# jiahuei/sparse-image-captioning

Hardware: AMD Instinct MI355X
Metric: captions/sec (higher is better)
Workload: dtype bf16; 1 GPU; configs[1]: ORT dense, 256 images x 5 captions, teacher-forcing XE fwd+bwd+clip+Adam; images_per_gpu=256, regions=36, captions_per_image=5, parallelism=single

## Files before the change

include/ortk.h:

```cpp
#ifndef ORTK_H
#define ORTK_H

#include <stddef.h>
#include <stdint.h>

#ifdef __cplusplus
extern "C" {
#endif

#define ORTK_VERSION 4
#define ORTK_EINVAL (-1)
#define ORTK_ENOSPC (-2)
#define ORTK_ENOSYS (-3)
#define ORTK_EEXCHANGE (-4)

typedef void* ortk_stream;

int ortk_version(void);
int ortk_device_ok(void);

struct ortk_sparse_plan;
typedef struct ortk_config {
    int32_t d_model, d_ff, n_layers, n_heads;
    int32_t vocab, feat, seq_len;
    int32_t pad_id, bos_id, eos_id, unk_id;
    int32_t box_trig;
    int32_t precision;
    float   drop_src, drop;
    int32_t share_enc[16], share_dec[16];
    int32_t share_att_enc, share_att_dec;
    int32_t no_box;
    const struct ortk_sparse_plan* sparse_fwd;
    const struct ortk_sparse_plan* sparse_bwd;
} ortk_config;

int64_t ortk_arena_numel(const ortk_config* cfg);
int64_t ortk_arena_numel_with_buffers(const ortk_config* cfg);
int32_t ortk_arena_entries(const ortk_config* cfg);
int ortk_arena_entry(const ortk_config* cfg, int32_t index, char* name_buf, int64_t* offset,
                     int64_t* numel, int32_t* ndim, int64_t* shape, int32_t* kind);

uint32_t ortk_dropout_site_seed(uint64_t seed, int32_t stack, int32_t layer, int32_t k);

typedef struct ortk_batch {
    const float*   att_feats;
    const float*   boxes;
    const float*   att_masks;
    const int64_t* seqs;
    int64_t        seq_stride;
    const float*   tok_weight;
    int32_t B, S, R, T;
    const int32_t* cap_off;
    const int32_t* row_pos;
    int32_t        Mc;
    int32_t        no_pad_keys;
} ortk_batch;

int ortk_valid_position_tables(const int64_t* counts, int32_t R, int32_t T, int32_t* cap_off, int32_t* row_pos, ortk_stream stream);
size_t ortk_train_workspace_bytes(const ortk_config* cfg, int32_t B, int32_t S, int32_t R, int32_t T);
int ortk_valid_positions_ok(const ortk_config* cfg, int32_t B, int32_t S, int32_t R, int32_t T);

int ortk_forward(const ortk_config* cfg, const float* params, const ortk_batch* batch, void* ws, size_t ws_bytes,
                 float* logp_out, int64_t ldv, int32_t train, uint64_t seed, ortk_stream stream);
int ortk_forward_phase(const ortk_config* cfg, const float* params, const ortk_batch* batch, void* ws, size_t ws_bytes,
                       float* logp_out, int64_t ldv, int32_t train, uint64_t seed, int32_t phase, ortk_stream stream);
void* ortk_train_workspace_memory(const ortk_config* cfg, int32_t B, int32_t S, int32_t R, int32_t T, void* ws, int32_t* dtype);

int ortk_loss(const ortk_config* cfg, const ortk_batch* batch, void* ws, size_t ws_bytes,
              const float* norm_dev, float* loss_dev, ortk_stream stream);

int ortk_loss_external(const ortk_config* cfg, const ortk_batch* batch, void* ws, size_t ws_bytes,
                       const float* logp, const float* dlogp, int64_t ldv, ortk_stream stream);

int ortk_backward(const ortk_config* cfg, const float* params, float* grads, const ortk_batch* batch,
                  void* ws, size_t ws_bytes, int32_t train, uint64_t seed, ortk_stream stream);
int ortk_backward_phase(const ortk_config* cfg, const float* params, float* grads, const ortk_batch* batch,
                        void* ws, size_t ws_bytes, int32_t train, uint64_t seed, int32_t phase, ortk_stream stream);
int64_t ortk_arena_decoder_offset(const ortk_config* cfg);

#define ORTK_SP_ELL32 0
#define ORTK_SP_ELL16 1
#define ORTK_SP_GU16  2
typedef struct ortk_sparse_block {
    int64_t src_offset;
    int64_t ld;
    int64_t stream_offset;
    int64_t capacity;
    int32_t N, K;
    int32_t chunk0;
    int32_t row0;
} ortk_sparse_block;

typedef struct ortk_sparse_plan {
    const ortk_sparse_block* blocks_host; const ortk_sparse_block* blocks_dev;
    int32_t nblocks, format;
    void* stream;
    int32_t* chunk_ptr;
    int32_t* chunk_len;
    int32_t* perm;
    int32_t* count_scratch;
    int32_t* overflow;
    int64_t total_rows;
} ortk_sparse_plan;

int ortk_sparse_build(const ortk_sparse_plan* plan, const void* dense, int32_t dtype, ortk_stream stream);

typedef struct ortk_spmm_args {
    const void* X; void* Y;
    int64_t ldx, ldy; int64_t M;
    int32_t x_dtype, y_dtype;
    const float* bias; const float* rowscale; const float* resid; int64_t ldr;
    const void* gate; int64_t ldg; int32_t gate_dtype; float gate_scale;
    int32_t relu; float drop_p; uint32_t drop_seed;
    const int32_t* drop_rows;
} ortk_spmm_args;
int ortk_spmm(const ortk_sparse_plan* plan, int32_t block, const ortk_spmm_args* a, ortk_stream stream);

typedef struct ortk_chain_unit { int64_t offset, ld; } ortk_chain_unit;
typedef struct ortk_chain_args {
    const void* w16; const ortk_chain_unit* units_dev; int32_t n_units;
    void* packed; size_t packed_bytes;
    int64_t M;
    const float* x_in;
    const void* a_in; const float* bias_r; float* x_mid; uint32_t seed_r;
    const float *g1, *b1; void* y1; float* st1;
    int32_t n1; const float* bias_s1; void* out1; int64_t ld1;
    int32_t NC; const float *bias_h, *bias_o; void* h; float* x_out; uint32_t seed_h, seed_o;
    const float *g2, *b2; void* y2; float* st2;
    int32_t n2; const float* bias_s2; void* out2; int64_t ld2;
    float drop_p, eps;
    int32_t* progress;
    const int32_t* drop_rows;
} ortk_chain_args;
size_t ortk_chain_packed_bytes(int32_t n_units);
int ortk_row_chain(const ortk_chain_args* a, ortk_stream stream);

typedef struct ortk_bchain_args {
    const void* w16t; const ortk_chain_unit* units_dev; int32_t n_units;
    void* packed; size_t packed_bytes;
    int64_t M;
    int32_t nin; const void* ain; int64_t ld_ain; const void* dz0;
    const float *xa, *sta, *ga, *dresa; float *dxa, *daa, *dba; void* dza; uint32_t seed_a; int32_t mask_a;
    int32_t NC; const void* hgate; void* gh; float gate_scale;
    const float *xb, *stb, *gb, *dresb; float *dxb, *dab, *dbb; void* dzb; uint32_t seed_b; int32_t mask_b;
    int32_t n2; void* out2;
    float drop_p, eps;
    const int32_t* drop_rows;
} ortk_bchain_args;
int ortk_row_bchain(const ortk_bchain_args* a, ortk_stream stream);
// ... 97 lines not shown
    int64_t rows;
    int32_t flags;
    void* ws; size_t ws_bytes;
} ortk_wgrad_group_args;
int ortk_wgrad_group(const ortk_wgrad_group_args* a, ortk_stream stream);
size_t ortk_wgrad_group_workspace_bytes(const ortk_wgrad_group_args* a);
int ortk_prof_enable(int32_t on);
int ortk_prof_collect(int32_t key, int64_t* launches, double* total_ms, double* total_flops);
int ortk_prof_collect_bytes(int32_t key, double* total_bytes);
int ortk_prof_collect_units(int32_t key, double* total_workgroups);

int ortk_layernorm_fwd(const float* x, const float* a, const float* b, void* y, int32_t y_dtype, float* stats,
                       int64_t rows, int32_t d, float eps, ortk_stream stream);
int ortk_layernorm_bwd(const float* dy, const float* x, const float* a, const float* stats, const float* dres,
                       float* dx, float* da, float* db, int64_t rows, int32_t d, float eps, ortk_stream stream);
int ortk_layernorm_bwd_drop(const float* dy, const float* x, const float* a, const float* stats, const float* dres,
                            float* dx, float* da, float* db, int64_t rows, int32_t d, float eps, void* dz, int32_t dz_dtype,
                            float drop_p, uint32_t drop_seed, ortk_stream stream);
int ortk_layernorm_bwd_drop_rows(const float* dy, const float* x, const float* a, const float* stats, const float* dres,
                                 float* dx, float* da, float* db, int64_t rows, int32_t d, float eps, void* dz, int32_t dz_dtype,
                                 float drop_p, uint32_t drop_seed, const int32_t* drop_rows, ortk_stream stream);
int ortk_layernorm_bwd_dt(const void* dy, int32_t dy_dtype, const float* x, const float* a, const float* stats, const float* dres,
                          float* dx, float* da, float* db, int64_t rows, int32_t d, float eps, void* dz, int32_t dz_dtype,
                          float drop_p, uint32_t drop_seed, const int32_t* drop_rows, ortk_stream stream);

int ortk_box_logbias_fwd(const float* boxes, const float* const* wg, const float* const* bg, const float* dim_mat,
                         float* out, int32_t L, int32_t B, int32_t S, int32_t H, ortk_stream stream);
int ortk_box_logbias_bwd(const float* boxes, const float* const* wg, const float* const* bg, const float* dim_mat,
                         const float* dscore, float* const* dwg, float* const* dbg,
                         int32_t L, int32_t B, int32_t S, int32_t H, ortk_stream stream);
int ortk_box_embedding(const float* boxes, const float* dim_mat, float* out, int32_t B, int32_t S, ortk_stream stream);

typedef struct ortk_attn_args {
    const float* q; const float* k; const float* v; void* o;
    int64_t ldq, ldk, ldv, ldo;
    const float* kmask; const float* bias; const int32_t* kv_index;
    int64_t kv_group_stride;
    float* p;
    int32_t nkv, H, Lq, Lk, dk, causal_period;
    float drop_p; uint32_t drop_seed;
    const float* d_o; void* dq; void* d_k; void* dv; float* dscore;
    int64_t lddo, lddq, lddk, lddv;
    int32_t o_dtype, dqkv_dtype;
    int32_t kv_dtype;
    const float* k_new; const float* v_new; int64_t ld_new;
    int32_t bwd_part;
    int32_t precision;
    int32_t qkv_dtype;
    const int32_t* q_off; int32_t q_off_stride; int32_t kv_ragged;
    int32_t drop_tf_T, drop_tf_t, drop_tf_lk;
    const int32_t* drop_rows;
} ortk_attn_args;
int ortk_attention_fwd(const ortk_attn_args* a, ortk_stream stream);
int ortk_attention_bwd(const ortk_attn_args* a, ortk_stream stream);

int ortk_embed_fwd(const int64_t* seq, int64_t seq_stride, const float* lut, const float* pe, float* out, float* keymask,
                   int64_t R, int32_t T, int32_t t0, int32_t d, int32_t pad_id, float drop_p, uint32_t seed, ortk_stream stream);
int ortk_embed_bwd(const int64_t* seq, int64_t seq_stride, const float* dout, float* dlut,
                   int64_t R, int32_t T, int32_t d, float drop_p, uint32_t seed, ortk_stream stream);

int ortk_log_softmax(float* x, int64_t rows, int32_t V, int64_t ld, float scale, ortk_stream stream);
int64_t ortk_xent_scratch_floats(int64_t rows);
int ortk_xent_fwd_bwd(const float* logits, const int64_t* targets, int64_t target_stride, int32_t T, const float* weight,
                      const float* norm_dev, float* loss_dev, float* row_loss, int64_t rows, int32_t V, int64_t ld,
                      void* dlogits, int32_t dl_dtype, int64_t ld_dl, ortk_stream stream);
int ortk_log_softmax_bwd(const float* logp, const float* dlogp, int64_t ld_in, void* dlogits, int32_t dl_dtype,
                         int64_t ld_out, int64_t rows, int32_t V, ortk_stream stream);

int ortk_colsum(const void* x, int32_t x_dtype, int64_t ld, float* out, int64_t M, int32_t N, ortk_stream stream);
int ortk_gate_apply(const float* x, const float* gate, void* y, int32_t y_dtype, int64_t n, float scale, ortk_stream stream);
int ortk_dropout_apply(const float* x, void* y, int32_t y_dtype, int64_t n, float p, uint32_t seed, ortk_stream stream);
int ortk_dropout_apply_rows(const float* x, void* y, int32_t y_dtype, int64_t rows, int32_t d, float p, uint32_t seed,
                            const int32_t* drop_rows, ortk_stream stream);
int ortk_cast_bf16(const float* x, void* y, int64_t n, ortk_stream stream);
int ortk_fill(float* x, int64_t n, float value, ortk_stream stream);
int ortk_axpy_cols(const void* x, void* y, int32_t dtype, int64_t ld, int64_t rows, int32_t cols, ortk_stream stream);
int64_t ortk_sum_scratch_floats(int64_t n);
int ortk_sum(const float* x, int64_t n, float* scratch, float* out_dev, ortk_stream stream);

int ortk_adam_clip(float* p, const float* g, float* m, float* v, int64_t n, float lr, float beta1, float beta2,
                   float eps, float clip, float bc1, float bc2, ortk_stream stream);
int ortk_adam_clip_zero(float* p, float* g, float* m, float* v, int64_t n, float lr, float beta1, float beta2,
                        float eps, float clip, float bc1, float bc2, ortk_stream stream);

int ortk_mask_apply(const float* w, const float* m, float* w_eff, int64_t n, int32_t mode, uint32_t seed, ortk_stream stream);
int ortk_mask_bwd(const float* dw_eff, const float* w, const float* m, float* dw, float* dm, int64_t n, int32_t mode,
                  uint32_t seed, const float* extra_coef_dev, ortk_stream stream);
typedef struct ortk_masked_adam_args {
    float *w, *g, *mw, *vw;
    float *ml, *mm, *mv;
    const float* draws;
    const float* active;
    const float* extra_coef;
    int64_t n, index0; int32_t mode; uint32_t seed;
    float lr_w, eps_w, lr_m, eps_m, beta1, beta2, clip, bc1, bc2;
} ortk_masked_adam_args;
int ortk_masked_adam_step(const ortk_masked_adam_args* a, ortk_stream stream);
int ortk_mask_apply_draws(const float* w, const float* m, const float* draws, float* w_eff, int64_t n, ortk_stream stream);
int ortk_mask_bwd_draws(const float* dw_eff, const float* w, const float* m, const float* draws, float* dw, float* dm, int64_t n,
                        const float* extra_coef_dev, ortk_stream stream);
int ortk_linear_block(const ortk_config* cfg, int32_t i, int64_t* offset, int32_t* N, int32_t* K);
int ortk_mask_count(const float* m, int64_t n, int32_t mode, float* count_dev, ortk_stream stream);

#ifdef __cplusplus
}
#endif
#endif
```

sparse-image-captioning_amd/_lib.py:

```python
import ctypes as C
import os

import torch

_HERE = os.path.dirname(os.path.abspath(__file__))
LIB_PATH = os.path.join(_HERE, "libortk.so")


class OrtkUnavailable(RuntimeError):
    pass


class OrtkError(RuntimeError):
    pass


class Config(C.Structure):
    _fields_ = [("d_model", C.c_int32), ("d_ff", C.c_int32), ("n_layers", C.c_int32), ("n_heads", C.c_int32),
                ("vocab", C.c_int32), ("feat", C.c_int32), ("seq_len", C.c_int32),
                ("pad_id", C.c_int32), ("bos_id", C.c_int32), ("eos_id", C.c_int32), ("unk_id", C.c_int32),
                ("box_trig", C.c_int32), ("precision", C.c_int32), ("drop_src", C.c_float), ("drop", C.c_float),
                ("share_enc", C.c_int32 * 16), ("share_dec", C.c_int32 * 16),
                ("share_att_enc", C.c_int32), ("share_att_dec", C.c_int32), ("no_box", C.c_int32),
                ("sparse_fwd", C.c_void_p), ("sparse_bwd", C.c_void_p)]


class Batch(C.Structure):
    _fields_ = [("att_feats", C.c_void_p), ("boxes", C.c_void_p), ("att_masks", C.c_void_p), ("seqs", C.c_void_p),
                ("seq_stride", C.c_int64), ("tok_weight", C.c_void_p),
                ("B", C.c_int32), ("S", C.c_int32), ("R", C.c_int32), ("T", C.c_int32),
                ("cap_off", C.c_void_p), ("row_pos", C.c_void_p), ("Mc", C.c_int32), ("no_pad_keys", C.c_int32)]


SP_ELL32, SP_ELL16, SP_GU16 = 0, 1, 2


class EllBlock(C.Structure):
    _fields_ = [("src_offset", C.c_int64), ("ld", C.c_int64), ("stream_offset", C.c_int64), ("capacity", C.c_int64),
                ("N", C.c_int32), ("K", C.c_int32), ("chunk0", C.c_int32), ("row0", C.c_int32)]


class EllPlanStruct(C.Structure):
    _fields_ = [("blocks_host", C.POINTER(EllBlock)), ("blocks_dev", C.c_void_p), ("nblocks", C.c_int32), ("format", C.c_int32),
                ("stream", C.c_void_p), ("chunk_ptr", C.c_void_p), ("chunk_len", C.c_void_p), ("perm", C.c_void_p),
                ("count_scratch", C.c_void_p), ("overflow", C.c_void_p), ("total_rows", C.c_int64)]


class SpmmArgs(C.Structure):
    _fields_ = [("X", C.c_void_p), ("Y", C.c_void_p), ("ldx", C.c_int64), ("ldy", C.c_int64), ("M", C.c_int64),
                ("x_dtype", C.c_int32), ("y_dtype", C.c_int32),
                ("bias", C.c_void_p), ("rowscale", C.c_void_p), ("resid", C.c_void_p), ("ldr", C.c_int64),
                ("gate", C.c_void_p), ("ldg", C.c_int64), ("gate_dtype", C.c_int32), ("gate_scale", C.c_float),
                ("relu", C.c_int32), ("drop_p", C.c_float), ("drop_seed", C.c_uint32), ("drop_rows", C.c_void_p)]


class ChainUnit(C.Structure):
    _fields_ = [("offset", C.c_int64), ("ld", C.c_int64)]


class ChainArgs(C.Structure):
    _fields_ = [("w16", C.c_void_p), ("units_dev", C.c_void_p), ("n_units", C.c_int32), ("packed", C.c_void_p), ("packed_bytes", C.c_size_t),
                ("M", C.c_int64), ("x_in", C.c_void_p),
                ("a_in", C.c_void_p), ("bias_r", C.c_void_p), ("x_mid", C.c_void_p), ("seed_r", C.c_uint32),
                ("g1", C.c_void_p), ("b1", C.c_void_p), ("y1", C.c_void_p), ("st1", C.c_void_p),
                ("n1", C.c_int32), ("bias_s1", C.c_void_p), ("out1", C.c_void_p), ("ld1", C.c_int64),
                ("NC", C.c_int32), ("bias_h", C.c_void_p), ("bias_o", C.c_void_p), ("h", C.c_void_p), ("x_out", C.c_void_p),
                ("seed_h", C.c_uint32), ("seed_o", C.c_uint32),
                ("g2", C.c_void_p), ("b2", C.c_void_p), ("y2", C.c_void_p), ("st2", C.c_void_p),
                ("n2", C.c_int32), ("bias_s2", C.c_void_p), ("out2", C.c_void_p), ("ld2", C.c_int64),
                ("drop_p", C.c_float), ("eps", C.c_float), ("progress", C.c_void_p), ("drop_rows", C.c_void_p)]


class BChainArgs(C.Structure):
    _fields_ = [("w16t", C.c_void_p), ("units_dev", C.c_void_p), ("n_units", C.c_int32), ("packed", C.c_void_p), ("packed_bytes", C.c_size_t),
                ("M", C.c_int64),
                ("nin", C.c_int32), ("ain", C.c_void_p), ("ld_ain", C.c_int64), ("dz0", C.c_void_p),
                ("xa", C.c_void_p), ("sta", C.c_void_p), ("ga", C.c_void_p), ("dresa", C.c_void_p), ("dxa", C.c_void_p), ("daa", C.c_void_p),
                ("dba", C.c_void_p), ("dza", C.c_void_p), ("seed_a", C.c_uint32), ("mask_a", C.c_int32),
                ("NC", C.c_int32), ("hgate", C.c_void_p), ("gh", C.c_void_p), ("gate_scale", C.c_float),
                ("xb", C.c_void_p), ("stb", C.c_void_p), ("gb", C.c_void_p), ("dresb", C.c_void_p), ("dxb", C.c_void_p), ("dab", C.c_void_p),
                ("dbb", C.c_void_p), ("dzb", C.c_void_p), ("seed_b", C.c_uint32), ("mask_b", C.c_int32),
                ("n2", C.c_int32), ("out2", C.c_void_p), ("drop_p", C.c_float), ("eps", C.c_float), ("drop_rows", C.c_void_p)]


class MaskedAdamArgs(C.Structure):
    _fields_ = [("w", C.c_void_p), ("g", C.c_void_p), ("mw", C.c_void_p), ("vw", C.c_void_p),
                ("ml", C.c_void_p), ("mm", C.c_void_p), ("mv", C.c_void_p),
                ("draws", C.c_void_p), ("active", C.c_void_p), ("extra_coef", C.c_void_p),
                ("n", C.c_int64), ("index0", C.c_int64), ("mode", C.c_int32), ("seed", C.c_uint32),
                ("lr_w", C.c_float), ("eps_w", C.c_float), ("lr_m", C.c_float), ("eps_m", C.c_float),
                ("beta1", C.c_float), ("beta2", C.c_float), ("clip", C.c_float), ("bc1", C.c_float), ("bc2", C.c_float)]


class Tuning(C.Structure):
    _fields_ = [("gemm_t64", C.c_int32), ("attn_impl", C.c_int32), ("attn16_min_lq", C.c_int32),
                ("side_stream", C.c_int32), ("row_chain", C.c_int32), ("chain_wide", C.c_int32), ("spmm_alias", C.c_int32), ("f32_split", C.c_int32), ("wgrad_wgs", C.c_int32),
                ("wgrad_group", C.c_int32), ("wgrad_group_splitk", C.c_int32), ("wgrad_group_wgs", C.c_int32), ("wgrad_group_tail", C.c_int32), ("feats_bf16", C.c_int32), ("ln_fuse", C.c_int32), ("samp_epilogue", C.c_int32), ("gemm_epilogue", C.c_int32)]


DEC_UNFUSED, DEC_STACK, DEC_SPARSE_STREAM, DEC_STACK_RB20, DEC_STACK_SPLIT, DEC_SPLIT_SMALL, DEC_SPARSE_GATHER = 1, 2, 4, 8, 16, 32, 64


class DecodeOpts(C.Structure):
    _fields_ = [("beam_size", C.c_int32), ("num_random_sample", C.c_int32), ("temperature", C.c_float),
                ("decoding_constraint", C.c_int32), ("length_penalty", C.c_int32), ("length_alpha", C.c_double),
                ("seed", C.c_uint64), ("sparse", C.POINTER(EllPlanStruct)), ("exec_flags", C.c_int32), ("with_greedy", C.c_int32), ("sample_row_offset", C.c_int64),
                ("train", C.c_int32), ("drop_seed", C.c_uint64), ("memory", C.c_void_p)]


class GemmArgs(C.Structure):
    _fields_ = [("A", C.c_void_p), ("B", C.c_void_p), ("C", C.c_void_p),
                ("lda", C.c_int64), ("ldb", C.c_int64), ("ldc", C.c_int64),
                ("M", C.c_int32), ("N", C.c_int32), ("K", C.c_int32), ("transA", C.c_int32), ("transB", C.c_int32),
                ("bias", C.c_void_p), ("rowscale", C.c_void_p), ("resid", C.c_void_p), ("ldr", C.c_int64),
                ("gate", C.c_void_p), ("ldg", C.c_int64), ("gate_scale", C.c_float),
                ("relu", C.c_int32), ("drop_p", C.c_float), ("drop_seed", C.c_uint32),
                ("accumulate", C.c_int32), ("splitk", C.c_int32), ("precision", C.c_int32),
                ("a_dtype", C.c_int32), ("b_dtype", C.c_int32), ("c_dtype", C.c_int32), ("gate_dtype", C.c_int32),
                ("colsum", C.c_void_p), ("drop_row_stride", C.c_int32), ("drop_row_off", C.c_int32),
                ("ln_mode", C.c_int32), ("ln_y_dtype", C.c_int32),
                ("ln_a", C.c_void_p), ("ln_b", C.c_void_p), ("ln_y", C.c_void_p), ("ln_stats", C.c_void_p), ("ln_eps", C.c_float),
                ("ln_x", C.c_void_p), ("ln_dres", C.c_void_p), ("ln_da", C.c_void_p), ("ln_db", C.c_void_p),
                ("tile_stats", C.c_void_p), ("stat_ncols", C.c_int32), ("drop_rows", C.c_void_p),
                ("tile_samp", C.c_void_p), ("samp_seq", C.c_void_p), ("samp_seed", C.c_uint64), ("samp_row_offset", C.c_int64),
                ("samp_L", C.c_int32), ("samp_t", C.c_int32), ("samp_greedy_stride", C.c_int32), ("samp_sample", C.c_int32),
                ("samp_fast", C.c_int32), ("samp_no_store", C.c_int32), ("samp_inv_temperature", C.c_float)]


class WgradItem(C.Structure):
    _fields_ = [("dY", C.c_void_p), ("lddy", C.c_int64), ("X", C.c_void_p), ("ldx", C.c_int64),
                ("dW", C.c_void_p), ("lddw", C.c_int64), ("db", C.c_void_p), ("Nout", C.c_int32), ("Kin", C.c_int32)]


WGRAD_MAX = 8


class WgradGroupArgs(C.Structure):
    _fields_ = [("item", WgradItem * WGRAD_MAX), ("n", C.c_int32), ("splitk", C.c_int32), ("rows", C.c_int64), ("flags", C.c_int32),
                ("ws", C.c_void_p), ("ws_bytes", C.c_size_t)]


class AttnArgs(C.Structure):
    _fields_ = [("q", C.c_void_p), ("k", C.c_void_p), ("v", C.c_void_p), ("o", C.c_void_p),
                ("ldq", C.c_int64), ("ldk", C.c_int64), ("ldv", C.c_int64), ("ldo", C.c_int64),
                ("kmask", C.c_void_p), ("bias", C.c_void_p), ("kv_index", C.c_void_p), ("kv_group_stride", C.c_int64),
                ("p", C.c_void_p),
                ("nkv", C.c_int32), ("H", C.c_int32), ("Lq", C.c_int32), ("Lk", C.c_int32), ("dk", C.c_int32),
                ("causal_period", C.c_int32), ("drop_p", C.c_float), ("drop_seed", C.c_uint32),
                ("d_o", C.c_void_p), ("dq", C.c_void_p), ("d_k", C.c_void_p), ("dv", C.c_void_p), ("dscore", C.c_void_p),
                ("lddo", C.c_int64), ("lddq", C.c_int64), ("lddk", C.c_int64), ("lddv", C.c_int64),
                ("o_dtype", C.c_int32), ("dqkv_dtype", C.c_int32), ("kv_dtype", C.c_int32),
                ("k_new", C.c_void_p), ("v_new", C.c_void_p), ("ld_new", C.c_int64), ("bwd_part", C.c_int32),
                ("precision", C.c_int32), ("qkv_dtype", C.c_int32),
                ("q_off", C.c_void_p), ("q_off_stride", C.c_int32), ("kv_ragged", C.c_int32),
                ("drop_tf_T", C.c_int32), ("drop_tf_t", C.c_int32), ("drop_tf_lk", C.c_int32), ("drop_rows", C.c_void_p)]


_P, _I32, _I64, _F, _U32, _U64, _SZ = C.c_void_p, C.c_int32, C.c_int64, C.c_float, C.c_uint32, C.c_uint64, C.c_size_t
_CFG = C.POINTER(Config)

SIGNATURES = {
    "ortk_version": (_I32, []),
    "ortk_device_ok": (_I32, []),
    "ortk_arena_numel": (_I64, [_CFG]),
    "ortk_arena_numel_with_buffers": (_I64, [_CFG]),
    "ortk_arena_entries": (_I32, [_CFG]),
    "ortk_arena_entry": (_I32, [_CFG, _I32, C.c_char_p, C.POINTER(_I64), C.POINTER(_I64), C.POINTER(_I32),
                               C.POINTER(_I64), C.POINTER(_I32)]),
    "ortk_train_workspace_bytes": (_SZ, [_CFG, _I32, _I32, _I32, _I32]),
    "ortk_valid_positions_ok": (_I32, [_CFG, _I32, _I32, _I32, _I32]),
    "ortk_forward": (_I32, [_CFG, _P, C.POINTER(Batch), _P, _SZ, _P, _I64, _I32, _U64, _P]),
    "ortk_forward_phase": (_I32, [_CFG, _P, C.POINTER(Batch), _P, _SZ, _P, _I64, _I32, _U64, _I32, _P]),
    "ortk_train_workspace_memory": (_P, [_CFG, _I32, _I32, _I32, _I32, _P, C.POINTER(C.c_int32)]),
    "ortk_loss": (_I32, [_CFG, C.POINTER(Batch), _P, _SZ, _P, _P, _P]),
    "ortk_loss_external": (_I32, [_CFG, C.POINTER(Batch), _P, _SZ, _P, _P, _I64, _P]),
    "ortk_backward": (_I32, [_CFG, _P, _P, C.POINTER(Batch), _P, _SZ, _I32, _U64, _P]),
    "ortk_backward_phase": (_I32, [_CFG, _P, _P, C.POINTER(Batch), _P, _SZ, _I32, _U64, _I32, _P]),
    "ortk_arena_decoder_offset": (_I64, [_CFG]),
    "ortk_decode_workspace_bytes": (_SZ, [_CFG, _I32, _I32, C.POINTER(DecodeOpts)]),
    "ortk_decode": (_I32, [_CFG, _P, _P, _P, _P, _I32, _I32, C.POINTER(DecodeOpts), _P, _SZ, _P, _P, _P, _P]),
    "ortk_decode_status": (_I32, [_P, _P]),
    "ortk_encode": (_I32, [_CFG, _P, _P, _P, _P, _I32, _I32, _P, _SZ, _P, _P]),
    "ortk_chain_packed_bytes": (_SZ, [_I32]),
    "ortk_row_chain": (_I32, [C.POINTER(ChainArgs), _P]),
    "ortk_row_bchain": (_I32, [C.POINTER(BChainArgs), _P]),
    "ortk_get_tuning": (None, [C.POINTER(Tuning)]),
    "ortk_set_tuning": (_I32, [C.POINTER(Tuning)]),
    "ortk_gemm": (_I32, [C.POINTER(GemmArgs), _P]),
    "ortk_wgrad_group": (_I32, [C.POINTER(WgradGroupArgs), _P]),
    "ortk_wgrad_group_workspace_bytes": (_SZ, [C.POINTER(WgradGroupArgs)]),
    "ortk_prof_enable": (_I32, [_I32]),
    "ortk_prof_collect": (_I32, [_I32, C.POINTER(_I64), C.POINTER(C.c_double), C.POINTER(C.c_double)]),
    "ortk_prof_collect_bytes": (_I32, [_I32, C.POINTER(C.c_double)]),
    "ortk_prof_collect_units": (_I32, [_I32, C.POINTER(C.c_double)]),
    "ortk_layernorm_fwd": (_I32, [_P, _P, _P, _P, _I32, _P, _I64, _I32, _F, _P]),
    "ortk_layernorm_bwd": (_I32, [_P, _P, _P, _P, _P, _P, _P, _P, _I64, _I32, _F, _P]),
    "ortk_layernorm_bwd_drop": (_I32, [_P, _P, _P, _P, _P, _P, _P, _P, _I64, _I32, _F, _P, _I32, _F, C.c_uint32, _P]),
    "ortk_layernorm_bwd_drop_rows": (_I32, [_P, _P, _P, _P, _P, _P, _P, _P, _I64, _I32, _F, _P, _I32, _F, C.c_uint32, _P, _P]),
    "ortk_layernorm_bwd_dt": (_I32, [_P, _I32, _P, _P, _P, _P, _P, _P, _P, _I64, _I32, _F, _P, _I32, _F, C.c_uint32, _P, _P]),
    "ortk_box_logbias_fwd": (_I32, [_P, C.POINTER(_P), C.POINTER(_P), C.POINTER(_F), _P, _I32, _I32, _I32, _I32, _P]),
    "ortk_box_logbias_bwd": (_I32, [_P, C.POINTER(_P), C.POINTER(_P), C.POINTER(_F), _P, C.POINTER(_P), C.POINTER(_P),
                                   _I32, _I32, _I32, _I32, _P]),
    "ortk_box_embedding": (_I32, [_P, C.POINTER(_F), _P, _I32, _I32, _P]),
    "ortk_attention_fwd": (_I32, [C.POINTER(AttnArgs), _P]),
    "ortk_attention_bwd": (_I32, [C.POINTER(AttnArgs), _P]),
    "ortk_valid_position_tables": (_I32, [_P, _I32, _I32, _P, _P, _P]),
    "ortk_embed_fwd": (_I32, [_P, _I64, _P, _P, _P, _P, _I64, _I32, _I32, _I32, _I32, _F, _U32, _P]),
    "ortk_embed_bwd": (_I32, [_P, _I64, _P, _P, _I64, _I32, _I32, _F, _U32, _P]),
    "ortk_log_softmax": (_I32, [_P, _I64, _I32, _I64, _F, _P]),
    "ortk_xent_scratch_floats": (_I64, [_I64]),
    "ortk_xent_fwd_bwd": (_I32, [_P, _P, _I64, _I32, _P, _P, _P, _P, _I64, _I32, _I64, _P, _I32, _I64, _P]),
    "ortk_log_softmax_bwd": (_I32, [_P, _P, _I64, _P, _I32, _I64, _I64, _I32, _P]),
    "ortk_colsum": (_I32, [_P, _I32, _I64, _P, _I64, _I32, _P]),
    "ortk_gate_apply": (_I32, [_P, _P, _P, _I32, _I64, _F, _P]),
    "ortk_dropout_apply": (_I32, [_P, _P, _I32, _I64, _F, _U32, _P]),
    "ortk_dropout_apply_rows": (_I32, [_P, _P, _I32, _I64, _I32, _F, _U32, _P, _P]),
    "ortk_dropout_site_seed": (_U32, [_U64, _I32, _I32, _I32]),
    "ortk_cast_bf16": (_I32, [_P, _P, _I64, _P]),
    "ortk_fill": (_I32, [_P, _I64, _F, _P]),
    "ortk_sum_scratch_floats": (_I64, [_I64]),
    "ortk_sum": (_I32, [_P, _I64, _P, _P, _P]),
    "ortk_adam_clip": (_I32, [_P, _P, _P, _P, _I64, _F, _F, _F, _F, _F, _F, _F, _P]),
    "ortk_adam_clip_zero": (_I32, [_P, _P, _P, _P, _I64, _F, _F, _F, _F, _F, _F, _F, _P]),
    "ortk_mask_apply": (_I32, [_P, _P, _P, _I64, _I32, _U32, _P]),
    "ortk_mask_bwd": (_I32, [_P, _P, _P, _P, _P, _I64, _I32, _U32, _P, _P]),
    "ortk_masked_adam_step": (_I32, [C.POINTER(MaskedAdamArgs), _P]),
    "ortk_mask_count": (_I32, [_P, _I64, _I32, _P, _P]),
    "ortk_mask_apply_draws": (_I32, [_P, _P, _P, _P, _I64, _P]),
    "ortk_mask_bwd_draws": (_I32, [_P, _P, _P, _P, _P, _P, _I64, _P, _P]),
    "ortk_decode_step_workspace_bytes": (_SZ, [_CFG, _I32]),
    "ortk_project_memory": (_I32, [_CFG, _P, _P, _I64, _P, _SZ, _P, _P]),
    "ortk_decode_step": (_I32, [_CFG, _P, _P, _I32, _I32, _I32, _I32, _P, _P, _P, _P, _I32, _P, _SZ, _P, _I64, _P]),
    "ortk_axpy_cols": (_I32, [_P, _P, _I32, _I64, _I64, _I32, _P]),
    "ortk_linear_block": (_I32, [_CFG, _I32, C.POINTER(C.c_int64), C.POINTER(C.c_int32), C.POINTER(C.c_int32)]),
    "ortk_sparse_build": (_I32, [C.POINTER(EllPlanStruct), _P, _I32, _P]),
    "ortk_spmm": (_I32, [C.POINTER(EllPlanStruct), _I32, C.POINTER(SpmmArgs), _P]),
}

_lib = None
ABI_VERSION = 4


def lib():
    global _lib
    if _lib is None:
        if not os.path.exists(LIB_PATH):
            raise OrtkUnavailable(
                f"{LIB_PATH} is missing: build it with `python -c 'import __graft_entry__ as g; g.build()'` "
                "(or `make -C sparse-image-captioning_amd/csrc`).  There is no CPU / PyTorch fallback.")
        h = C.CDLL(LIB_PATH)
        h.ortk_version.restype = C.c_int32
        if h.ortk_version() != ABI_VERSION:
            raise OrtkUnavailable(
                f"{LIB_PATH} is ABI version {h.ortk_version()}, these bindings were written for version {ABI_VERSION} (include/ortk.h: "
                "ORTK_VERSION): a stale build.  Rebuild it with `make -C sparse-image-captioning_amd/csrc`.")
        for name, (res, args) in SIGNATURES.items():
            fn = getattr(h, name)
            fn.restype = res
            fn.argtypes = args
        _lib = h
    return _lib


def set_tuning(**kw):
    t = Tuning()
    lib().ortk_get_tuning(C.byref(t))
    old = {f: getattr(t, f) for f, _ in Tuning._fields_}
    for k, v in kw.items():
        assert k in old, k
        setattr(t, k, int(v))
    check(lib().ortk_set_tuning(C.byref(t)), "ortk_set_tuning")
    return old


def require_gpu():
    if not torch.cuda.is_available():
        raise OrtkUnavailable("no HIP device visible: the ORT hot path runs only on MI355X (gfx950); no CPU fallback")
    if not lib().ortk_device_ok():
        raise OrtkUnavailable("the visible device is not gfx950; libortk.so carries gfx950 code objects only")


def stream_ptr():
    return C.c_void_p(torch.cuda.current_stream().cuda_stream)


def ptr(t):
    if t is None:
        return None
    assert t.is_cuda, "libortk takes device pointers only"
    return C.c_void_p(t.data_ptr())


def check(code, what):
    if code != 0:
        names = {-1: "ORTK_EINVAL (bad argument / unsupported shape)", -2: "ORTK_ENOSPC (workspace too small)",
                 -3: "ORTK_ENOSYS (option not implemented)",
                 -4: "ORTK_EEXCHANGE (column-split decode: an exchange group never met — the launch was not fully resident; "
                     "outputs are poisoned; set model.exclusive_gpu = False when the GPU is shared)"}
        raise OrtkError(f"{what} failed: {names.get(code, 'hipError ' + str(code))}")


def f32c(t):
    assert t.is_cuda
    if t.dtype != torch.float32:
        t = t.float()
    return t.contiguous()
```

sparse-image-captioning_amd/csrc/ortk_chain.hip:

```cpp
#include "ortk_internal.h"
#include <mutex>

namespace ortk {
namespace {

typedef __attribute__((ext_vector_type(2))) __bf16 bf16x2;

constexpr int CD = 512;
constexpr int CMT = 3;
constexpr int CRB = 16 * CMT;
constexpr int CSPD = 4;
constexpr int CFRAG = 64;
constexpr int CKSTEP = 4 * CFRAG;
constexpr int CUNIT = 16 * CKSTEP;
constexpr int CIMG = CRB * CD * 2;
constexpr int CKEY_BYTES = 512;
__device__ __forceinline__ void c_fill_keys(uint32_t* skey, const int32_t* __restrict__ drop_rows, int r0, int nrow, int tid) {
    if (tid < CKEY_BYTES / 4) {
        const int g = r0 + (tid < nrow ? tid : 0);
        skey[tid] = drop_rows ? (uint32_t)drop_rows[g] : (uint32_t)g;
    }
    __syncthreads();
}

// ... 729 lines not shown
        ln_bwd(acc, a.xa, a.sta, a.ga, a.dresa, a.dxa, a.daa, a.dba, a.dza, a.seed_a, a.mask_a != 0);
    } else {
        load_img(A0, a.dz0, CD, 0);
        __syncthreads();
    }
    if (a.NC > 0) {
        CH_FRESH_LANE();
        f32x4 acc2[CMT][4];
        c_zero(acc2);
        const int64_t ffn = (int64_t)a.NC * CD;
        for (int c = 0; c < a.NC; ++c) {
            char* Hc = (c & 1) ? H1 : H0;
            f32x4 acc[CMT][4];
            c_zero(acc);
            c_unit(acc, A0, wp, ring, lane);
#pragma unroll
            for (int mt = 0; mt < CMT; ++mt) {
                const int row = 16 * mt + (lane & 15);
                const bool live = row < nrow;
                const int64_t g = r0 + (live ? row : 0);
#pragma unroll
                for (int nt = 0; nt < 4; ++nt) {
                    const int col = 64 * wave + 16 * nt + 4 * (lane >> 4);
                    const uint2 hv = *reinterpret_cast<const uint2*>(a.hgate + g * ffn + c * CD + col);
                    const bool k0 = (hv.x & 0x7FFFu) != 0 && !(hv.x & 0x8000u), k1 = (hv.x & 0x7FFF0000u) != 0 && !(hv.x & 0x80000000u);
                    const bool k2 = (hv.y & 0x7FFFu) != 0 && !(hv.y & 0x8000u), k3 = (hv.y & 0x7FFF0000u) != 0 && !(hv.y & 0x80000000u);
                    const float v0 = k0 ? acc[mt][nt][0] * a.gate_scale : 0.f, v1 = k1 ? acc[mt][nt][1] * a.gate_scale : 0.f;
                    const float v2 = k2 ? acc[mt][nt][2] * a.gate_scale : 0.f, v3 = k3 ? acc[mt][nt][3] * a.gate_scale : 0.f;
                    const uint2 pk = make_uint2(c_pack2(v0, v1), c_pack2(v2, v3));
                    *reinterpret_cast<uint2*>(Hc + c_off(row, col >> 3) + ((col >> 2) & 1) * 8) = pk;
                    if (live) *reinterpret_cast<uint2*>(a.gh + g * ffn + c * CD + col) = pk;
                }
            }
            __syncthreads();
            c_unit(acc2, Hc, wp, ring, lane);
        }
        __syncthreads();
        ln_bwd(acc2, a.xb, a.stb, a.gb, a.dresb, a.dxb, a.dab, a.dbb, a.dzb, a.seed_b, a.mask_b != 0);
    }
    if (a.n2 > 0) {
        CH_FRESH_LANE();
        f32x4 acc[CMT][4];
        c_zero(acc);
        c_unit(acc, A0, wp, ring, lane);
#pragma unroll
        for (int mt = 0; mt < CMT; ++mt) {
            const int row = 16 * mt + (lane & 15);
            if (row < nrow) {
#pragma unroll
                for (int nt = 0; nt < 4; ++nt) {
                    const int col = 64 * wave + 16 * nt + 4 * (lane >> 4);
                    *reinterpret_cast<uint2*>(a.out2 + (int64_t)(r0 + row) * CD + col) =
                        make_uint2(c_pack2(acc[mt][nt][0], acc[mt][nt][1]), c_pack2(acc[mt][nt][2], acc[mt][nt][3]));
                }
            }
        }
    }
#undef CH_FRESH_LANE
}

struct PackUnit { int64_t offset, ld; };
__device__ __forceinline__ int64_t pack_src(int form, int w, int q, int64_t ld) {
    const int lane = q & 63;
    int nt, ks, col0;
    col0 = 64 * w;
    if (form != 2) { nt = (q >> 6) & 3; ks = q >> 8; }
    else { const int j = (q >> 6) & 3, g = q >> 8; ks = 2 * (g & 7) + (j >> 1); nt = 2 * (g >> 3) + (j & 1); }
    return (int64_t)(col0 + 16 * nt + (lane & 15)) * ld + 32 * ks + 8 * (lane >> 4);
}
__global__ __launch_bounds__(256) void chain_pack_kernel(const __bf16* __restrict__ w16, uint4* __restrict__ out, const PackUnit* __restrict__ units,
                                                         int n_units, int wide, int n_r, int n1, int NC) {
    const int64_t usz = CUNIT;
    const int64_t per_wave = (int64_t)(n_units + 1) * usz, total = 8 * per_wave;
    for (int64_t i = (int64_t)blockIdx.x * 256 + threadIdx.x; i < total; i += (int64_t)gridDim.x * 256) {
        const int w = (int)(i / per_wave);
        const int64_t rest = i - (int64_t)w * per_wave;
        const int u = (int)(rest / usz), q = (int)(rest % usz);
        if (u >= n_units) { out[i] = make_uint4(0, 0, 0, 0); continue; }
        const PackUnit pu = units[u];
        out[i] = *reinterpret_cast<const uint4*>(w16 + pu.offset + pack_src(chain_unit_form(wide != 0, u, n_r, n1, NC), w, q, pu.ld));
    }
}

__global__ __launch_bounds__(256) void chain_pack_all_kernel(const __bf16* __restrict__ w16, uint4* __restrict__ out, ChainPackTable t, int64_t total) {
    for (int64_t i = (int64_t)blockIdx.x * 256 + threadIdx.x; i < total; i += (int64_t)gridDim.x * 256) {
        int c = 0;
        int64_t rest = i;
        for (; c < t.n_chains; ++c) {
            const int64_t sz = (int64_t)8 * (t.first[c + 1] - t.first[c] + 1) * CUNIT;
            if (rest < sz) break;
            rest -= sz;
        }
        const int n = t.first[c + 1] - t.first[c];
        const int64_t usz = CUNIT;
        const int64_t per_wave = (int64_t)(n + 1) * usz;
        const int w = (int)(rest / per_wave);
        const int64_t r2 = rest - (int64_t)w * per_wave;
        const int u = (int)(r2 / usz), q = (int)(r2 % usz);
        uint4 v = make_uint4(0, 0, 0, 0);
        if (u < n) {
            const auto pu = t.u[t.first[c] + u];
            v = *reinterpret_cast<const uint4*>(w16 + (int64_t)pu.offset + pack_src(t.form[t.first[c] + u], w, q, pu.ld));
        }
        out[t.base[c] + rest] = v;
    }
}

constexpr size_t CHAIN_LDS = (size_t)3 * CIMG + 2 * CRB * 8 * sizeof(float) + CKEY_BYTES;

}

size_t chain_packed_bytes(int n_units) { return (size_t)8 * (n_units + 1) * CUNIT * sizeof(uint4); }

int chain_rows_per_block(int64_t M, int slots) {
    const int64_t blocks48 = ortk_cdiv(M, CRB), rounds = ortk_cdiv(blocks48, slots);
    const int64_t rb = ortk_cdiv(M, rounds * slots);
    return (int)std::min<int64_t>(CRB, std::max<int64_t>(rb, 1));
}

bool chain_wide(int64_t M) {
    if (!tuning().chain_wide) return false;
    if (tuning().chain_wide == 2) return ortk_cdiv(ortk_cdiv(M, (int64_t)WRB), 256) < ortk_cdiv(ortk_cdiv(M, (int64_t)CRB), 256);
    return ortk_cdiv(ortk_cdiv(M, (int64_t)WRB), 256) == 1 && ortk_cdiv(ortk_cdiv(M, (int64_t)CRB), 256) == 2;
}

int chain_pack(const void* w16, const ortk_chain_unit* units_dev, int n_units, void* packed, hipStream_t s, bool wide, int n_r, int n1, int NC) {
    if (!w16 || !units_dev || n_units < 1 || !packed) return ORTK_EINVAL;
    static_assert(sizeof(PackUnit) == sizeof(ortk_chain_unit), "unit descriptor");
    static_assert(WUNIT == CUNIT, "both streams take the same bytes per unit and wave");
    hipLaunchKernelGGL(chain_pack_kernel, dim3(1024), dim3(256), 0, s, reinterpret_cast<const __bf16*>(w16), reinterpret_cast<uint4*>(packed),
                       reinterpret_cast<const PackUnit*>(units_dev), n_units, wide ? 1 : 0, n_r, n1, NC);
    ORTK_CHECK_LAUNCH();
    return 0;
}

int chain_pack_all(const void* w16, void* packed, const ChainPackTable& t, hipStream_t s) {
    if (!w16 || !packed || t.n_chains < 1 || t.n_chains > CH_MAX_CHAINS) return ORTK_EINVAL;
    int64_t total = 0;
    for (int c = 0; c < t.n_chains; ++c) {
        if (t.base[c] != total || t.first[c + 1] <= t.first[c] || t.first[c + 1] > CH_MAX_UNITS) return ORTK_EINVAL;
        total += (int64_t)8 * (t.first[c + 1] - t.first[c] + 1) * CUNIT;
    }
    hipLaunchKernelGGL(chain_pack_all_kernel, dim3(2048), dim3(256), 0, s, reinterpret_cast<const __bf16*>(w16), reinterpret_cast<uint4*>(packed), t, total);
    ORTK_CHECK_LAUNCH();
    return 0;
}

int chain_run(const ortk_chain_args* p, const void* packed, hipStream_t s) {
    if (!p || !packed || !p->x_in || p->M < 1 || p->M > (int64_t)1 << 22) return ORTK_EINVAL;
    if (p->n1 < 0 || p->n1 > 3 || p->n2 < 0 || p->n2 > 3 || p->NC < 0 || p->NC > 8) return ORTK_EINVAL;
    if ((p->n1 > 0 && !p->g1) || (p->n2 > 0 && !p->g2)) return ORTK_EINVAL;
    if (p->a_in && (!p->bias_r || !p->x_mid)) return ORTK_EINVAL;
    if (p->n1 > 0 && (!p->bias_s1 || !p->out1 || p->ld1 < p->n1 * CD || p->ld1 % 4)) return ORTK_EINVAL;
    if (p->n2 > 0 && (!p->bias_s2 || !p->out2 || p->ld2 < p->n2 * CD || p->ld2 % 4)) return ORTK_EINVAL;
    if (p->NC > 0 && (!p->g1 || !p->bias_h || !p->bias_o || !p->x_out)) return ORTK_EINVAL;
    if (p->drop_p < 0.f || p->drop_p >= 1.f) return ORTK_EINVAL;
    const int n_units = (p->a_in ? 1 : 0) + p->n1 + 2 * p->NC + p->n2;
    if (n_units < 1 || n_units != p->n_units) return ORTK_EINVAL;
    if ((int64_t)p->M * std::max(p->NC, 1) * CD >= ((int64_t)1 << 32)) return ORTK_EINVAL;
    static std::mutex mu;
    static bool done[64] = {};
    int dev = 0;
    if (hipGetDevice(&dev) != hipSuccess || dev < 0 || dev >= 64) return ORTK_EINVAL;
    {
        std::lock_guard<std::mutex> g(mu);
        if (!done[dev]) {
            hipError_t e = hipFuncSetAttribute(reinterpret_cast<const void*>(row_chain_kernel), hipFuncAttributeMaxDynamicSharedMemorySize, (int)CHAIN_LDS);
            if (e == hipSuccess) e = hipFuncSetAttribute(reinterpret_cast<const void*>(row_chain_wide_kernel), hipFuncAttributeMaxDynamicSharedMemorySize, (int)WIDE_LDS);
            if (e != hipSuccess) return (int)e;
            done[dev] = true;
        }
    }
    const bool wide = !p->progress && chain_wide(p->M);
    ChainArgs a;
    a.wpk = reinterpret_cast<const uint4*>(packed); a.n_units = n_units;
    a.progress = p->progress; a.npf = p->progress ? 8 : 0; a.slots = 256 - a.npf;
    if (p->progress && hipMemsetAsync(p->progress, 0, 16 * sizeof(int32_t), s) != hipSuccess) return ORTK_EINVAL;
    a.M = (int)p->M; a.rb = chain_rows_per_block(p->M, a.slots);
    if (wide) a.rb = (int)std::min<int64_t>(WRB, ortk_cdiv(p->M, ortk_cdiv(ortk_cdiv(p->M, (int64_t)WRB), 256) * 256));
    a.x_in = p->x_in;
    a.a_in = reinterpret_cast<const __bf16*>(p->a_in); a.bias_r = p->bias_r; a.x_mid = p->x_mid; a.seed_r = p->seed_r;
    a.g1 = p->g1; a.b1 = p->b1; a.y1 = reinterpret_cast<__bf16*>(p->y1); a.st1 = p->st1;
    a.n1 = p->n1; a.bias_s1 = p->bias_s1; a.out1 = reinterpret_cast<__bf16*>(p->out1); a.ld1 = (int)p->ld1;
    a.NC = p->NC; a.bias_h = p->bias_h; a.bias_o = p->bias_o; a.h = reinterpret_cast<__bf16*>(p->h); a.x_out = p->x_out;
    a.seed_h = p->seed_h; a.seed_o = p->seed_o;
    a.g2 = p->g2; a.b2 = p->b2; a.y2 = reinterpret_cast<__bf16*>(p->y2); a.st2 = p->st2;
    a.n2 = p->n2; a.bias_s2 = p->bias_s2; a.out2 = reinterpret_cast<__bf16*>(p->out2); a.ld2 = (int)p->ld2;
    a.drop_p = p->drop_p; a.eps = p->eps; a.drop_rows = p->drop_rows;
    const unsigned grid = (unsigned)(ortk_cdiv(p->M, a.rb) + a.npf);
    ProfMark pm;
    if (ortk_prof_active()) {
        const double rowb = 2048.0 + (p->a_in ? 1024 + 2048 : 0) + (p->g1 ? (p->y1 ? 1024 : 0) + 8 : 0) + p->n1 * 1024.0 +
                            (p->NC ? (p->h ? p->NC * 1024.0 : 0.0) + 2048 + 2048 : 0) + (p->g2 ? (p->y2 ? 1024 : 0) + 8 : 0) + p->n2 * 1024.0;
        (void)prof_begin(PROF_KEY_CHAIN, 2.0 * p->M * n_units * CD * CD, (double)n_units * CD * CD * 2 + rowb * p->M, s, pm);
    } else pm.live = false;
    if (wide) hipLaunchKernelGGL(row_chain_wide_kernel, dim3(grid), dim3(512), WIDE_LDS, s, a);
    else hipLaunchKernelGGL(row_chain_kernel, dim3(grid), dim3(512), CHAIN_LDS, s, a);
    prof_end(pm, s);
    ORTK_CHECK_LAUNCH();
    return 0;
}

int bchain_run(const ortk_bchain_args* p, const void* packed, hipStream_t s) {
    if (!p || !packed || p->M < 1 || p->M > (int64_t)1 << 22) return ORTK_EINVAL;
    if ((p->nin != 0 && p->nin != 1 && p->nin != 3) || p->NC < 0 || p->NC > 8 || p->n2 < 0 || p->n2 > 1) return ORTK_EINVAL;
    if (p->nin > 0 && (!p->ain || p->ld_ain < p->nin * CD || p->ld_ain % 8 || !p->xa || !p->sta || !p->ga || !p->dxa || !p->daa || !p->dba)) return ORTK_EINVAL;
    if (p->nin == 0 && !p->dz0) return ORTK_EINVAL;
    if (p->NC > 0 && (!p->hgate || !p->gh || !p->xb || !p->stb || !p->gb || !p->dxb || !p->dab || !p->dbb)) return ORTK_EINVAL;
    if (p->n2 > 0 && !p->out2) return ORTK_EINVAL;
    if ((p->NC > 0 || p->n2 > 0) && p->nin > 0 && !p->mask_a) return ORTK_EINVAL;
    if (p->n2 > 0 && p->NC > 0 && !p->mask_b) return ORTK_EINVAL;
    if (p->drop_p < 0.f || p->drop_p >= 1.f) return ORTK_EINVAL;
    const int n_units = p->nin + 2 * p->NC + p->n2;
    if (n_units < 1 || n_units != p->n_units) return ORTK_EINVAL;
    if ((int64_t)p->M * CD >= ((int64_t)1 << 32)) return ORTK_EINVAL;
    static std::mutex mu;
    static bool done[64] = {};
    int dev = 0;
    if (hipGetDevice(&dev) != hipSuccess || dev < 0 || dev >= 64) return ORTK_EINVAL;
    {
        std::lock_guard<std::mutex> g(mu);
        if (!done[dev]) {
            const hipError_t e = hipFuncSetAttribute(reinterpret_cast<const void*>(row_bchain_kernel), hipFuncAttributeMaxDynamicSharedMemorySize, (int)CHAIN_LDS);
            if (e != hipSuccess) return (int)e;
            done[dev] = true;
        }
// ... 38 lines not shown
```

sparse-image-captioning_amd/csrc/ortk_embed_loss.hip:

```cpp
#include "ortk_internal.h"

namespace {

__global__ __launch_bounds__(128) void embed_fwd_kernel(const int64_t* __restrict__ seq, int64_t seq_stride,
                                                        const float* __restrict__ lut, const float* __restrict__ pe,
                                                        float* __restrict__ out, float* __restrict__ keymask, int T, int t0,
                                                        int d, int pad_id, float scale, float drop_p, uint32_t seed,
                                                        const int32_t* __restrict__ row_pos, int drop_rs, int drop_r0, int eval_stride) {
    const int64_t row = blockIdx.x;
    const int64_t prow = row_pos ? (int64_t)row_pos[row] : row;
    const int64_t r = prow / T;
    const int t = (int)(prow - r * T);
    const int64_t tok = seq[r * seq_stride + t];
    if (keymask && threadIdx.x == 0) keymask[row] = tok != pad_id ? 1.f : 0.f;
    const float* e = lut + tok * d;
    const float* p = pe + (int64_t)(t0 + t) * d;
    const float inv_keep = drop_p > 0.f ? 1.f / (1.f - drop_p) : 1.f;
    int64_t drow = prow;
    bool drop = drop_p > 0.f;
    if (eval_stride > 0) { const int64_t q = row / eval_stride, k = row - q * eval_stride; drop = drop && k != 0; drow = q * (eval_stride - 1) + k - 1; }
    for (int c = threadIdx.x; c < d; c += 128) {
        float v = e[c] * scale + p[c];
        if (drop) v = ortk_keep(seed, (uint64_t)(drow * drop_rs + drop_r0) * d + c, drop_p) ? v * inv_keep : 0.f;
        out[row * d + c] = v;
// ... 100 lines not shown
    if (FAST) {
#pragma unroll
        for (int u = 0; u < NPT; ++u) { z[u] = tid + 256 * u < V ? __expf(z[u] - mx) : 0.f; s += z[u]; }
    } else {
#pragma unroll
        for (int u = 0; u < NPT; ++u) if (tid + 256 * u < V) s += expf(z[u] - mx);
    }
    s = block_sum(s, sh);
    const float lse = logf(s);
    if (tid == 0) row_loss[r] = w != 0.f ? -((row[tgt] - mx) - lse) * w : 0.f;
    __syncthreads();
    const float ws_ = FAST ? w / s : 0.f;
#pragma unroll
    for (int u = 0; u < NPT; ++u) {
        const int c = tid + 256 * u;
        if (c < (int)ld_dl) {
            float g = 0.f;
            if (FAST) { if (c < V && w != 0.f) g = z[u] * ws_ - (c == tgt ? w : 0.f); }
            else if (c < V && w != 0.f) g = (expf((z[u] - mx) - lse) - (c == tgt ? 1.f : 0.f)) * w;
            st_elem(dlogits, r * ld_dl + c, dl_dt, g);
        }
    }
}

__global__ __launch_bounds__(256) void log_softmax_bwd_kernel(const float* __restrict__ logp, const float* __restrict__ dlogp,
                                                              int64_t ld_in, void* __restrict__ dlogits, int dl_dt, int64_t ld_out, int V) {
    __shared__ float sh[4];
    const int64_t r = blockIdx.x;
    const float* lp = logp + r * ld_in;
    const float* dl = dlogp + r * ld_in;
    float s = 0.f;
    for (int c = threadIdx.x; c < V; c += 256) s += dl[c];
    s = block_sum(s, sh);
    for (int c = threadIdx.x; c < (int)ld_out; c += 256) st_elem(dlogits, r * ld_out + c, dl_dt, c < V ? dl[c] - expf(lp[c]) * s : 0.f);
}

constexpr int CS_ROWS = 256;
__global__ __launch_bounds__(256) void colsum_kernel(const void* __restrict__ x, int x_dt, int64_t ld, float* __restrict__ out,
                                                     int64_t M, int N) {
    __shared__ float sh[4][64];
    const int lane = threadIdx.x & 63, wave = threadIdx.x >> 6;
    const int c = blockIdx.x * 64 + lane;
    const int64_t r0 = (int64_t)blockIdx.y * CS_ROWS;
    float acc = 0.f;
    if (c < N)
        for (int64_t r = r0 + wave; r < min(M, r0 + CS_ROWS); r += 4) acc += ld_elem(x, r * ld + c, x_dt);
    sh[wave][lane] = acc;
    __syncthreads();
    if (wave == 0 && c < N) atomicAdd(&out[c], sh[0][lane] + sh[1][lane] + sh[2][lane] + sh[3][lane]);
}

__global__ __launch_bounds__(256) void dropout_apply_kernel(const float* __restrict__ x, void* __restrict__ y, int y_dt, int64_t n,
                                                            float p, uint32_t seed) {
    const float inv_keep = 1.f / (1.f - p);
    for (int64_t i = (int64_t)blockIdx.x * 256 + threadIdx.x; i < n; i += (int64_t)gridDim.x * 256)
        st_elem(y, i, y_dt, (p > 0.f && !ortk_keep(seed, (uint64_t)i, p)) ? 0.f : x[i] * inv_keep);
}

__global__ __launch_bounds__(256) void dropout_apply_rows_kernel(const float* __restrict__ x, void* __restrict__ y, int y_dt, int64_t rows, int d,
                                                                 float p, uint32_t seed, const int32_t* __restrict__ drop_rows) {
    const float inv_keep = 1.f / (1.f - p);
    const int64_t n = rows * d;
    for (int64_t i = (int64_t)blockIdx.x * 256 + threadIdx.x; i < n; i += (int64_t)gridDim.x * 256) {
        const int64_t r = i / d; const int c = (int)(i - r * d);
        st_elem(y, i, y_dt, (p > 0.f && !ortk_keep(seed, (uint64_t)drop_rows[r] * (uint64_t)d + (uint64_t)c, p)) ? 0.f : x[i] * inv_keep);
    }
}

__global__ __launch_bounds__(256) void gate_apply_kernel(const float* __restrict__ x, const float* __restrict__ gate,
                                                         void* __restrict__ y, int y_dt, int64_t n, float scale) {
    for (int64_t i = (int64_t)blockIdx.x * 256 + threadIdx.x; i < n; i += (int64_t)gridDim.x * 256)
        st_elem(y, i, y_dt, gate[i] > 0.f ? x[i] * scale : 0.f);
}

__global__ __launch_bounds__(256) void cast_bf16_kernel(const float* __restrict__ x, __bf16* __restrict__ y, int64_t n) {
    const int64_t n4 = n >> 2;
    for (int64_t i = (int64_t)blockIdx.x * 256 + threadIdx.x; i < n4; i += (int64_t)gridDim.x * 256) {
        const float4 v = reinterpret_cast<const float4*>(x)[i];
        reinterpret_cast<bf16x4*>(y)[i] = (bf16x4){(__bf16)v.x, (__bf16)v.y, (__bf16)v.z, (__bf16)v.w};
    }
    for (int64_t i = (n4 << 2) + (int64_t)blockIdx.x * 256 + threadIdx.x; i < n; i += (int64_t)gridDim.x * 256) y[i] = (__bf16)x[i];
}

__global__ __launch_bounds__(256) void cast_bf16_t_kernel(const float* __restrict__ x, __bf16* __restrict__ yt, ortk::WBlockTable tab) {
    __shared__ float tile[64][65];
    int bi = 0;
    {
        int lo = 0, hi = tab.n - 1;
        while (lo < hi) { const int mid = (lo + hi + 1) >> 1; if (tab.b[mid].tile0 <= (int)blockIdx.x) lo = mid; else hi = mid - 1; }
        bi = lo;
    }
    const ortk::WBlock wb = tab.b[bi];
    const int tk = (wb.K + 63) >> 6;
    const int t = (int)blockIdx.x - wb.tile0, n0 = (t / tk) * 64, k0 = (t % tk) * 64;
    const float* src = x + wb.off;
    __bf16* dst = yt + wb.off;
    const int tid = threadIdx.x;
    const bool vec = (wb.K & 3) == 0 && (wb.off & 3) == 0;
#pragma unroll
    for (int i = 0; i < 4; ++i) {
        const int r = (tid >> 4) + 16 * i, c = (tid & 15) * 4;
        const int n = n0 + r, k = k0 + c;
        float4 v = make_float4(0.f, 0.f, 0.f, 0.f);
        if (n < wb.N) {
            if (vec && k + 3 < wb.K) v = *reinterpret_cast<const float4*>(src + (int64_t)n * wb.K + k);
            else { float* q = &v.x; for (int e = 0; e < 4; ++e) if (k + e < wb.K) q[e] = src[(int64_t)n * wb.K + k + e]; }
        }
        tile[r][c] = v.x; tile[r][c + 1] = v.y; tile[r][c + 2] = v.z; tile[r][c + 3] = v.w;
    }
    __syncthreads();
    const bool vec_o = (wb.N & 7) == 0 && (wb.off & 7) == 0;
#pragma unroll
    for (int i = 0; i < 2; ++i) {
        const int kr = (tid >> 3) + 32 * i, c = (tid & 7) * 8;
        const int k = k0 + kr, n = n0 + c;
        if (k >= wb.K) continue;
        if (vec_o && n + 7 < wb.N) {
            bf16x8 o;
#pragma unroll
            for (int e = 0; e < 8; ++e) o[e] = (__bf16)tile[c + e][kr];
            *reinterpret_cast<bf16x8*>(dst + (int64_t)k * wb.N + n) = o;
        } else {
            for (int e = 0; e < 8; ++e) if (n + e < wb.N) dst[(int64_t)k * wb.N + n + e] = (__bf16)tile[c + e][kr];
        }
    }
}

__global__ __launch_bounds__(256) void add_cols_kernel(const void* __restrict__ x, void* __restrict__ y, int dt, int64_t ld, int64_t rows, int cols) {
    const int64_t n = rows * cols;
    for (int64_t i = (int64_t)blockIdx.x * 256 + threadIdx.x; i < n; i += (int64_t)gridDim.x * 256) {
        const int64_t r = i / cols; const int c = (int)(i - r * cols);
        st_elem(y, r * ld + c, dt, ld_elem(y, r * ld + c, dt) + ld_elem(x, r * ld + c, dt));
    }
}

__global__ __launch_bounds__(256) void fill_kernel(float* __restrict__ x, int64_t n, float v) {
    for (int64_t i = (int64_t)blockIdx.x * 256 + threadIdx.x; i < n; i += (int64_t)gridDim.x * 256) x[i] = v;
}

constexpr int SUM_THREADS = 1024;
constexpr int64_t SUM_CHUNK = 64 * 1024;
__device__ __forceinline__ float fixed_order_block_sum(const float* __restrict__ x, int64_t n, float* sh) {
    float s = 0.f;
    for (int64_t i = threadIdx.x; i < n; i += SUM_THREADS) s += x[i];
    sh[threadIdx.x] = s;
    __syncthreads();
#pragma unroll
    for (int k = SUM_THREADS / 2; k >= 1; k >>= 1) {
        if ((int)threadIdx.x < k) sh[threadIdx.x] += sh[threadIdx.x + k];
        __syncthreads();
    }
    return sh[0];
}
__global__ __launch_bounds__(SUM_THREADS) void sum_fixed_kernel(const float* __restrict__ x, int64_t n, float* __restrict__ out) {
    __shared__ float sh[SUM_THREADS];
    const int64_t i0 = (int64_t)blockIdx.x * SUM_CHUNK;
    const float s = fixed_order_block_sum(x + i0, n - i0 < SUM_CHUNK ? n - i0 : SUM_CHUNK, sh);
    if (threadIdx.x == 0) out[blockIdx.x] = s;
}

__global__ __launch_bounds__(1024) void valid_rows_scan_kernel(const int64_t* __restrict__ n, int R, int32_t* __restrict__ cap_off) {
    __shared__ int part[1024];
    const int tid = threadIdx.x;
    const int per = (R + 1023) / 1024, r0 = tid * per, r1 = min(R, r0 + per);
    int s = 0;
    for (int r = r0; r < r1; ++r) s += (int)n[r];
    part[tid] = s;
    __syncthreads();
    for (int k = 1; k < 1024; k <<= 1) {
        const int v = tid >= k ? part[tid - k] : 0;
        __syncthreads();
        part[tid] += v;
        __syncthreads();
    }
    int acc = tid ? part[tid - 1] : 0;
    if (tid == 0) cap_off[0] = 0;
    for (int r = r0; r < r1; ++r) { acc += (int)n[r]; cap_off[r + 1] = acc; }
}
__global__ __launch_bounds__(256) void valid_rows_fill_kernel(const int32_t* __restrict__ cap_off, int R, int T, int32_t* __restrict__ row_pos) {
    const int r = blockIdx.x * 4 + (threadIdx.x >> 6), lane = threadIdx.x & 63;
    if (r >= R) return;
    const int o = cap_off[r], cnt = cap_off[r + 1] - o;
    for (int t = lane; t < cnt; t += 64) row_pos[o + t] = r * T + t;
}

inline unsigned ew_grid(int64_t n) { return (unsigned)std::min<int64_t>(ortk_cdiv(n, 256), 2048); }

}

namespace ortk {
int embed_fwd_rows(const int64_t* seq, int64_t seq_stride, const float* lut, const float* pe, float* out, float* keymask, int64_t nrows,
// ... 61 lines not shown
              int64_t ld_dl, hipStream_t s) {
    if (!logits || !targets || !weight || !norm_dev || !loss_dev || !row_loss || !dlogits || rows < 0 || V < 1 || ld < V || ld_dl < V || T < 1)
        return ORTK_EINVAL;
    if (dl_dtype != ORTK_F32 && dl_dtype != ORTK_BF16) return ORTK_EINVAL;
    if (rows == 0) return ortk_fill(loss_dev, 1, 0.f, (ortk_stream)s);
    if (V <= 256 * 40 && ld_dl <= 256 * 40 && V > 256 * 8 && dl_dtype == ORTK_BF16)
        hipLaunchKernelGGL((xent_reg_kernel<40, true>), dim3((unsigned)rows), dim3(256), 0, s, logits, targets, target_stride, T,
                           weight, norm_dev, row_loss, V, ld, dlogits, (int)dl_dtype, ld_dl, row_pos);
    else if (V <= 256 * 40 && ld_dl <= 256 * 40 && V > 256 * 8)
        hipLaunchKernelGGL((xent_reg_kernel<40, false>), dim3((unsigned)rows), dim3(256), 0, s, logits, targets, target_stride, T,
                           weight, norm_dev, row_loss, V, ld, dlogits, (int)dl_dtype, ld_dl, row_pos);
    else
        hipLaunchKernelGGL(xent_kernel, dim3((unsigned)rows), dim3(256), 0, s, logits, targets, target_stride, T, weight,
                           norm_dev, row_loss, V, ld, dlogits, (int)dl_dtype, ld_dl, row_pos);
    ORTK_CHECK_LAUNCH();
    return sum_fixed(row_loss, rows, row_loss + rows, loss_dev, s);
}
}

extern "C" int64_t ortk_xent_scratch_floats(int64_t rows) { return ortk::xent_scratch_floats(rows); }
extern "C" int ortk_xent_fwd_bwd(const float* logits, const int64_t* targets, int64_t target_stride, int32_t T, const float* weight,
                                 const float* norm_dev, float* loss_dev, float* row_loss, int64_t rows, int32_t V, int64_t ld, void* dlogits,
                                 int32_t dl_dtype, int64_t ld_dl, ortk_stream stream) {
    return ortk::xent_rows(logits, targets, target_stride, T, weight, norm_dev, loss_dev, row_loss, rows, nullptr, V, ld, dlogits, dl_dtype,
                           ld_dl, ortk_s(stream));
}

extern "C" int ortk_log_softmax_bwd(const float* logp, const float* dlogp, int64_t ld_in, void* dlogits, int32_t dl_dtype,
                                    int64_t ld_out, int64_t rows, int32_t V, ortk_stream stream) {
    if (!logp || !dlogp || !dlogits || rows < 0 || V < 1 || ld_in < V || ld_out < V) return ORTK_EINVAL;
    if (dl_dtype != ORTK_F32 && dl_dtype != ORTK_BF16) return ORTK_EINVAL;
    if (rows == 0) return 0;
    hipLaunchKernelGGL(log_softmax_bwd_kernel, dim3((unsigned)rows), dim3(256), 0, ortk_s(stream), logp, dlogp, ld_in, dlogits,
                       (int)dl_dtype, ld_out, V);
    ORTK_CHECK_LAUNCH();
    return 0;
}

extern "C" int ortk_colsum(const void* x, int32_t x_dtype, int64_t ld, float* out, int64_t M, int32_t N, ortk_stream stream) {
    if (!x || !out || M < 0 || N < 0 || (x_dtype != ORTK_F32 && x_dtype != ORTK_BF16)) return ORTK_EINVAL;
    if (M == 0 || N == 0) return 0;
    hipLaunchKernelGGL(colsum_kernel, dim3((unsigned)ortk_cdiv(N, 64), (unsigned)ortk_cdiv(M, CS_ROWS)), dim3(256), 0,
                       ortk_s(stream), x, (int)x_dtype, ld, out, M, N);
    ORTK_CHECK_LAUNCH();
    return 0;
}

extern "C" int ortk_dropout_apply(const float* x, void* y, int32_t y_dtype, int64_t n, float p, uint32_t seed, ortk_stream stream) {
    if (!x || !y || n < 0 || p < 0.f || p >= 1.f || (y_dtype != ORTK_F32 && y_dtype != ORTK_BF16)) return ORTK_EINVAL;
    if (n == 0) return 0;
    hipLaunchKernelGGL(dropout_apply_kernel, dim3(ew_grid(n)), dim3(256), 0, ortk_s(stream), x, y, (int)y_dtype, n, p, seed);
    ORTK_CHECK_LAUNCH();
    return 0;
}

extern "C" int ortk_dropout_apply_rows(const float* x, void* y, int32_t y_dtype, int64_t rows, int32_t d, float p, uint32_t seed,
                                       const int32_t* drop_rows, ortk_stream stream) {
    if (rows < 0 || d < 1) return ORTK_EINVAL;
    if (!drop_rows) return ortk_dropout_apply(x, y, y_dtype, rows * d, p, seed, stream);
    if (!x || !y || p < 0.f || p >= 1.f || (y_dtype != ORTK_F32 && y_dtype != ORTK_BF16)) return ORTK_EINVAL;
    if (rows == 0) return 0;
    hipLaunchKernelGGL(dropout_apply_rows_kernel, dim3(ew_grid(rows * d)), dim3(256), 0, ortk_s(stream), x, y, (int)y_dtype, rows, (int)d, p, seed, drop_rows);
    ORTK_CHECK_LAUNCH();
    return 0;
}

extern "C" int ortk_gate_apply(const float* x, const float* gate, void* y, int32_t y_dtype, int64_t n, float scale, ortk_stream stream) {
    if (!x || !gate || !y || n < 0 || (y_dtype != ORTK_F32 && y_dtype != ORTK_BF16)) return ORTK_EINVAL;
    if (n == 0) return 0;
    hipLaunchKernelGGL(gate_apply_kernel, dim3(ew_grid(n)), dim3(256), 0, ortk_s(stream), x, gate, y, (int)y_dtype, n, scale);
    ORTK_CHECK_LAUNCH();
    return 0;
}

extern "C" int ortk_cast_bf16(const float* x, void* y, int64_t n, ortk_stream stream) {
    if (!x || !y || n < 0 || (reinterpret_cast<uintptr_t>(x) & 15) || (reinterpret_cast<uintptr_t>(y) & 7)) return ORTK_EINVAL;
    if (n == 0) return 0;
    hipLaunchKernelGGL(cast_bf16_kernel, dim3(ew_grid(n / 4 + 1)), dim3(256), 0, ortk_s(stream), x, reinterpret_cast<__bf16*>(y), n);
    ORTK_CHECK_LAUNCH();
    return 0;
}

namespace ortk {
int cast_bf16_transposed(const float* x, void* yt, const WBlockTable& t, hipStream_t s) {
    if (!x || !yt || t.n < 0 || t.n > MAX_WBLOCKS) return ORTK_EINVAL;
    if (t.n == 0 || t.tiles == 0) return 0;
    hipLaunchKernelGGL(cast_bf16_t_kernel, dim3((unsigned)t.tiles), dim3(256), 0, s, x, reinterpret_cast<__bf16*>(yt), t);
    ORTK_CHECK_LAUNCH();
    return 0;
}
}

extern "C" int ortk_axpy_cols(const void* x, void* y, int32_t dtype, int64_t ld, int64_t rows, int32_t cols, ortk_stream stream) {
    if (!x || !y || rows < 0 || cols < 0 || ld < cols || (dtype != ORTK_F32 && dtype != ORTK_BF16)) return ORTK_EINVAL;
    if (rows == 0 || cols == 0) return 0;
    hipLaunchKernelGGL(add_cols_kernel, dim3(ew_grid(rows * cols)), dim3(256), 0, ortk_s(stream), x, y, (int)dtype, ld, rows, cols);
    ORTK_CHECK_LAUNCH();
    return 0;
}

extern "C" int ortk_valid_position_tables(const int64_t* counts, int32_t R, int32_t T, int32_t* cap_off, int32_t* row_pos, ortk_stream stream) {
    if (!counts || !cap_off || !row_pos || R < 1 || R > 1024 * 64 || T < 1) return ORTK_EINVAL;
    hipLaunchKernelGGL(valid_rows_scan_kernel, dim3(1), dim3(1024), 0, ortk_s(stream), counts, (int)R, cap_off);
    ORTK_CHECK_LAUNCH();
    hipLaunchKernelGGL(valid_rows_fill_kernel, dim3((unsigned)ortk_cdiv(R, 4)), dim3(256), 0, ortk_s(stream), cap_off, (int)R, (int)T, row_pos);
    ORTK_CHECK_LAUNCH();
    return 0;
}

extern "C" int ortk_fill(float* x, int64_t n, float value, ortk_stream stream) {
    if (!x || n < 0) return ORTK_EINVAL;
    if (n == 0) return 0;
    hipLaunchKernelGGL(fill_kernel, dim3(ew_grid(n)), dim3(256), 0, ortk_s(stream), x, n, value);
    ORTK_CHECK_LAUNCH();
    return 0;
}

extern "C" int64_t ortk_sum_scratch_floats(int64_t n) { return n < 0 ? -1 : ortk::sum_partials(n); }
extern "C" int ortk_sum(const float* x, int64_t n, float* scratch, float* out_dev, ortk_stream stream) {
    return ortk::sum_fixed(x, n, scratch, out_dev, ortk_s(stream));
}
```

sparse-image-captioning_amd/csrc/ortk_internal.h:

```cpp
#pragma once
#include "ortk_common.h"

namespace ortk {

const ortk_tuning& tuning();
int lds_attr(const void* fn, size_t bytes);

bool ortk_prof_active();
bool ortk_prof_serial();
constexpr int PROF_KEY_DECSTACK = 16;
constexpr int PROF_KEY_CHAIN = 17;
constexpr int PROF_KEY_WGRAD_GROUP = 18;
struct ProfMark { hipEvent_t a, b; int key; double flops, bytes; bool live; int slot = -1; double per_count = 0.0; double units = 0.0 ; };
bool prof_begin(int key, double flops, double bytes, hipStream_t s, ProfMark& m);
void prof_end(const ProfMark& m, hipStream_t s);
unsigned long long* prof_slot(int* index);

int kv_append(const float* qkv, void* cache_k, void* cache_v, int32_t kv_dtype, int64_t rows, int32_t d, int32_t row_mult, int32_t tmax,
              int32_t t, hipStream_t s);

bool attn16_shape_ok(int Lq, int Lk, int dk);
bool attn16_ok(const ortk_attn_args* a, bool bwd);
int attn16_fwd(const ortk_attn_args* a, hipStream_t s);
int attn16_bwd(const ortk_attn_args* a, hipStream_t s);

struct WBlock { int32_t off, N, K, tile0; };
constexpr int MAX_WBLOCKS = 200;
struct WBlockTable { int32_t n, tiles; WBlock b[MAX_WBLOCKS]; };
int cast_bf16_transposed(const float* x, void* yt, const WBlockTable& t, hipStream_t s);

struct BeamState {
    int32_t B, b, L, V, eos;
    int64_t ldv;
    int32_t* seq[2];
    float* tok_lp[2];
    float* cum;
    int64_t* it;
    int32_t* kvidx[2];
    int32_t* done_seq;
    float* done_lp;
    double* done_p;
    int32_t* done_len;
    int32_t* done_cnt;
    int32_t decoding_constraint, length_penalty;
    double length_alpha;
    int32_t tmax;
    const float* gstats; int32_t nblk;
    unsigned long long* uniq = nullptr;
};
int beam_step(const BeamState& st, const float* logp, int32_t t, hipStream_t s, bool fused = false, float scale = 1.f, bool fast_exp = false);
int beam_finalize(const BeamState& st, int64_t* seq_out, float* lp_out, float* score_out, hipStream_t s);

struct SampleState {
    int32_t rows, L, V, eos;
    int64_t ldv;
    int64_t* it;
    int64_t* seq;
    float* lp;
    int32_t* unfinished;
    int32_t* last_step;
    int32_t decoding_constraint, sample;
    float temperature;
    uint64_t seed;
    int32_t greedy_stride;
    int64_t row_offset;
};
int sample_init(const SampleState& st, int32_t bos, hipStream_t s);
int sample_step(const SampleState& st, const float* logp, int32_t t, hipStream_t s, bool fused = false, bool fast_exp = false);
int sample_combine(const SampleState& st, const float* gstats, const float* gsamp, int32_t nblk, int32_t t, hipStream_t s, bool fast_exp);
int sample_finalize(const SampleState& st, hipStream_t s);

constexpr int STACK_MAXL = 8;
struct StackLayer {
    const float *n0a, *n0b, *bqkv, *bo, *n1a, *n1b, *cqb, *cob, *n2a, *n2b, *b1, *b2;
    __bf16 *ck, *cv;
    const __bf16 *xk, *xv;
    const __bf16 *xkg, *xvg;
};
struct StackArgs {
    StackLayer layer[STACK_MAXL];
    const uint4* wpk;
    const uint2* sstream;
    int32_t gather;
    const int32_t* snst;
    const int64_t* sstart;
    const float* x_io;
    const int64_t* tok; const float* lut; const float* pe_t; float emb_scale;
    __bf16* y_out;
    const float *fa, *fb;
    const float* att_masks;
    const int32_t* kvidx;
    int64_t ldx;
    int32_t rows, per_img, S, T, t, L, NC;
    float eps;
    int32_t nblocks;
    int32_t* progress;
    int32_t uniq_slot;
    int32_t debug;
    int32_t rb;
    int32_t tp;
    const uint4* tp_wpk;
    char* tp_xbuf;
    int32_t* tp_flag;
    int32_t* tp_status;
    int32_t tp_groups;
    int32_t tp_launch;
    int64_t tp_xtile;
    float drop_p;
    int32_t greedy_stride;
    uint32_t drop_seed[STACK_MAXL][6];
};
constexpr int TP_FLAG_STRIDE = 128;
// ... 53 lines not shown
```

sparse-image-captioning_amd/csrc/ortk_model.hip:

```cpp
#include <string>
#include <vector>
#include <mutex>
#include <utility>
#include <cstring>
#include <cstdio>
#include <cstdlib>
#include "ortk_internal.h"

namespace ortk {

constexpr int MAXLAYERS = 16;

struct EncOff { int64_t wqkv, bqkv, wo, bo, wg, bg, w1, b1, w2, b2, n0a, n0b, n1a, n1b; };
struct DecOff { int64_t wqkv, bqkv, wo, bo, cqw, cqb, cow, cob, w1, b1, w2, b2, n0a, n0b, n1a, n1b, n2a, n2b; };
struct Offsets {
    int64_t att_w, att_b;
    EncOff enc[MAXLAYERS];
    int64_t enc_na, enc_nb;
    DecOff dec[MAXLAYERS];
    int64_t dec_na, dec_nb;
    int64_t ckv_w, ckv_b;
    int ckv_slot[MAXLAYERS];
    int ckv_slots;
    int64_t cw;
// ... 661 lines not shown
    const int d = cfg.d_model, ff = cfg.d_ff, H = cfg.n_heads, L = cfg.n_layers, dk = d / H, A = c.adt;
    const int64_t Me = (int64_t)B * S;
    const bool plain = cfg.no_box != 0;
    hipEvent_t box_done = nullptr;
    if (plain) {
    } else if (box_queued) {
        box_done = *box_queued;
    } else {
        TRY(queue_box_bias(c, o, boxes, logbias, B, S, &box_done));
    }
    if (feats16) {
        TRY(c.wait_ev(feats16_done));
        TRY(fwd_gemm(c, feats16, ORTK_BF16, cfg.feat, o.att_w, P + o.att_b, x0, ORTK_F32, d, Me, d, cfg.feat, true, c.p_src(), c.sub(OP_SRC),
                     nullptr, 0, plain ? nullptr : masks));
    } else {
        TRY(fwd_gemm(c, feats, ORTK_F32, cfg.feat, o.att_w, P + o.att_b, x0, ORTK_F32, d, Me, d, cfg.feat, true, c.p_src(), c.sub(OP_SRC),
                     nullptr, 0, plain ? nullptr : masks));
    }
    TRY(c.wait_ev(pack_done));
    const float* x = x0;
    const AttMode am = att_mode(cfg.share_att_enc);
    const bool chains = cs && cs->on && cs->e0 >= 0 && chain_pk && qdt == ORTK_BF16 && mem_dt == ORTK_BF16 && A == ORTK_BF16;
    if (chains) {
        ortk_chain_args ca; std::memset(&ca, 0, sizeof(ca));
        ca.n_units = cs->units(cs->e0); ca.M = Me; ca.x_in = x0;
        ca.g1 = P + o.enc[0].n0a; ca.b1 = P + o.enc[0].n0b; ca.y1 = keep ? bufs[0].y1 : nullptr; ca.st1 = keep ? bufs[0].st1 : nullptr;
        ca.n1 = 3; ca.bias_s1 = P + o.enc[0].bqkv; ca.out1 = bufs[0].qkv; ca.ld1 = 3 * d;
        ca.eps = 1e-6f;
        TRY(chain_run(&ca, cs->stream_of(chain_pk, cs->e0), c.s));
    }
    for (int l = 0; l < L; ++l) {
        const EncOff& e = o.enc[l]; const EncPtrs& b = bufs[l];
        if (chains) {
            ortk_attn_args a; std::memset(&a, 0, sizeof(a)); a.precision = c.prec; a.qkv_dtype = qdt;
            a.q = (const float*)b.qkv; a.k = (const float*)off_elems(b.qkv, am.k * d, qdt); a.v = (const float*)off_elems(b.qkv, am.v * d, qdt);
            a.ldq = a.ldk = a.ldv = 3 * d; a.o = b.o; a.o_dtype = A; a.ldo = d;
            a.kmask = masks; a.bias = plain ? nullptr : logbias + (int64_t)l * B * H * S * S; a.p = b.P;
            a.nkv = B; a.H = H; a.Lq = S; a.Lk = S; a.dk = dk; a.drop_p = c.p_drop(); a.drop_seed = c.sub(eop(l, 0));
            if (l == 0) TRY(c.wait_ev(box_done));
            TRY(ortk_attention_fwd(&a, (ortk_stream)c.s));
            ortk_chain_args ca; std::memset(&ca, 0, sizeof(ca));
            ca.n_units = cs->units(cs->eb[l]); ca.M = Me; ca.x_in = x;
            ca.a_in = b.o; ca.bias_r = P + e.bo; ca.x_mid = b.xm; ca.seed_r = c.sub(eop(l, 1));
            ca.g1 = P + e.n1a; ca.b1 = P + e.n1b; ca.y1 = keep ? b.y2 : nullptr; ca.st1 = keep ? b.st2 : nullptr;
            ca.NC = ff / 512; ca.bias_h = P + e.b1; ca.bias_o = P + e.b2; ca.h = keep ? b.h : nullptr; ca.x_out = b.xout;
            ca.seed_h = c.sub(eop(l, 2)); ca.seed_o = c.sub(eop(l, 3));
            if (l + 1 < L) {
                ca.g2 = P + o.enc[l + 1].n0a; ca.b2 = P + o.enc[l + 1].n0b; ca.y2 = keep ? bufs[l + 1].y1 : nullptr; ca.st2 = keep ? bufs[l + 1].st1 : nullptr;
                ca.n2 = 3; ca.bias_s2 = P + o.enc[l + 1].bqkv; ca.out2 = bufs[l + 1].qkv; ca.ld2 = 3 * d;
            } else {
                ca.g2 = P + o.enc_na; ca.b2 = P + o.enc_nb; ca.y2 = mem; ca.st2 = keep ? st_mem : nullptr;
            }
            ca.drop_p = c.p_drop(); ca.eps = 1e-6f;
            TRY(chain_run(&ca, cs->stream_of(chain_pk, cs->eb[l]), c.s));
            x = b.xout;
            continue;
        }
        TRY(ln_fwd(c, x, e.n0a, e.n0b, b.y1, A, b.st1, Me));
        TRY(fwd_gemm(c, b.y1, A, d, e.wqkv, P + e.bqkv, b.qkv, qdt, 3 * d, Me, am.n * d, d));
        ortk_attn_args a; std::memset(&a, 0, sizeof(a)); a.precision = c.prec; a.qkv_dtype = qdt;
        a.q = (const float*)b.qkv; a.k = (const float*)off_elems(b.qkv, am.k * d, qdt); a.v = (const float*)off_elems(b.qkv, am.v * d, qdt);
        a.ldq = a.ldk = a.ldv = 3 * d; a.o = b.o; a.o_dtype = A; a.ldo = d;
        a.kmask = masks; a.bias = plain ? nullptr : logbias + (int64_t)l * B * H * S * S; a.p = b.P;
        a.nkv = B; a.H = H; a.Lq = S; a.Lk = S; a.dk = dk; a.drop_p = c.p_drop(); a.drop_seed = c.sub(eop(l, 0));
        if (l == 0) TRY(c.wait_ev(box_done));
        TRY(ortk_attention_fwd(&a, (ortk_stream)c.s));
        TRY(fwd_gemm(c, b.o, A, d, e.wo, P + e.bo, b.xm, ORTK_F32, d, Me, d, d, false, c.p_drop(), c.sub(eop(l, 1)), x, d));
        TRY(ln_fwd(c, b.xm, e.n1a, e.n1b, b.y2, A, b.st2, Me));
        TRY(fwd_gemm(c, b.y2, A, d, e.w1, P + e.b1, b.h, A, ff, Me, ff, d, true, c.p_drop(), c.sub(eop(l, 2))));
        TRY(fwd_gemm(c, b.h, A, ff, e.w2, P + e.b2, b.xout, ORTK_F32, d, Me, d, ff, false, c.p_drop(), c.sub(eop(l, 3)), b.xm, d));
        x = b.xout;
    }
    if (!chains) TRY(ln_fwd(c, x, o.enc_na, o.enc_nb, mem, mem_dt, st_mem, Me));
    return 0;
}

static void enc_ptrs_from_ws(const TrainWS& w, int L, EncPtrs* out) {
    for (int l = 0; l < L; ++l) {
        const EncBuf& e = w.enc[l];
        out[l] = EncPtrs{e.y1, e.qkv, e.P, e.o, e.xm, e.y2, e.h, e.xout, e.st1, e.st2};
    }
}

static int make_w16t(const ortk_config* cfg, const Offsets& o, const float* params, void* w16t, ortk_stream stream);
static int make_w16(const ortk_config* cfg, const Offsets& o, const float* params, void* w16, ortk_stream stream) {
    if (!cfg->precision) return 0;
    return ortk_cast_bf16(params, w16, o.total, stream);
}

}

using namespace ortk;

extern "C" int ortk_version(void) { return ORTK_VERSION; }

extern "C" int ortk_device_ok(void) {
    int n = 0;
    if (hipGetDeviceCount(&n) != hipSuccess || n <= 0) return 0;
    hipDeviceProp_t prop;
    if (hipGetDeviceProperties(&prop, 0) != hipSuccess) return 0;
    return std::strstr(prop.gcnArchName, "gfx950") != nullptr ? 1 : 0;
}

extern "C" int64_t ortk_arena_numel(const ortk_config* cfg) {
    if (check_cfg(cfg)) return -1;
    Offsets o; build_layout(*cfg, o, nullptr);
    return o.total;
}
extern "C" int64_t ortk_arena_numel_with_buffers(const ortk_config* cfg) {
    if (check_cfg(cfg)) return -1;
    Offsets o; build_layout(*cfg, o, nullptr);
    return o.total_all;
}
extern "C" int32_t ortk_arena_entries(const ortk_config* cfg) {
    if (check_cfg(cfg)) return -1;
    Offsets o; std::vector<Entry> v; build_layout(*cfg, o, &v);
    return (int32_t)v.size();
}
extern "C" int ortk_arena_entry(const ortk_config* cfg, int32_t index, char* name_buf, int64_t* offset, int64_t* numel,
                                int32_t* ndim, int64_t* shape, int32_t* kind) {
    if (int e = check_cfg(cfg)) return e;
    Offsets o; std::vector<Entry> v; build_layout(*cfg, o, &v);
    if (index < 0 || index >= (int32_t)v.size() || !name_buf) return ORTK_EINVAL;
    const Entry& e = v[index];
    std::snprintf(name_buf, 128, "%s", e.name.c_str());
    if (offset) *offset = e.offset;
    if (numel) *numel = e.numel;
    if (ndim) *ndim = e.ndim;
    if (shape) for (int i = 0; i < 4; ++i) shape[i] = e.shape[i];
    if (kind) *kind = e.kind;
    return 0;
}

static int check_batch(const ortk_config* cfg, const ortk_batch* b, bool need_seq) {
    if (!b || !b->att_feats || (!b->boxes && !cfg->no_box) || !b->att_masks) return ORTK_EINVAL;
    if (b->B < 1 || b->S < 1 || b->S > 128) return ORTK_EINVAL;
    if (need_seq) {
        if (!b->seqs || b->R < 1 || b->T < 1 || b->R % b->B || b->seq_stride < b->T + 1) return ORTK_EINVAL;
        if (b->T > 64 || (int64_t)(b->R / b->B) * b->T > 4096) return ORTK_EINVAL;
        if (b->T > cfg->seq_len) return ORTK_EINVAL;
        if (b->cap_off || b->row_pos || b->Mc) {
            if (!b->cap_off || !b->row_pos || b->Mc < b->R || (int64_t)b->Mc > (int64_t)b->R * b->T || cfg->precision != 1) return ORTK_EINVAL;
        }
    }
    return 0;
}
static inline bool batch_compact(const ortk_batch* b) { return b->row_pos != nullptr; }

extern "C" int ortk_valid_positions_ok(const ortk_config* cfg, int32_t B, int32_t S, int32_t R, int32_t T) {
    if (check_cfg(cfg) || B < 1 || S < 1 || R < 1 || T < 1 || R % B) return 0;
    TrainWS w; carve_train(*cfg, B, S, R, T, nullptr, w);
    return cfg->precision == 1 && w.qdt_self && w.qdt_cross ? 1 : 0;
}

extern "C" size_t ortk_train_workspace_bytes(const ortk_config* cfg, int32_t B, int32_t S, int32_t R, int32_t T) {
    if (check_cfg(cfg) || B < 1 || S < 1 || R < 1 || T < 1) return 0;
    TrainWS w; carve_train(*cfg, B, S, R, T, nullptr, w);
    return w.bytes;
}

extern "C" int ortk_forward(const ortk_config* cfg, const float* params, const ortk_batch* bt, void* ws, size_t ws_bytes,
                            float* logp_out, int64_t ldv_out, int32_t train, uint64_t seed, ortk_stream stream) {
    return ortk_forward_phase(cfg, params, bt, ws, ws_bytes, logp_out, ldv_out, train, seed, 0, stream);
}

extern "C" void* ortk_train_workspace_memory(const ortk_config* cfg, int32_t B, int32_t S, int32_t R, int32_t T, void* ws, int32_t* dtype) {
    if (check_cfg(cfg) || B < 1 || S < 1 || R < 1 || T < 1 || !ws) return nullptr;
    TrainWS w; carve_train(*cfg, B, S, R, T, ws, w);
    if (dtype) *dtype = w.adt;
    return w.mem;
}

extern "C" int ortk_forward_phase(const ortk_config* cfg, const float* params, const ortk_batch* bt, void* ws, size_t ws_bytes,
                                  float* logp_out, int64_t ldv_out, int32_t train, uint64_t seed, int32_t phase, ortk_stream stream) {
    if (phase < 0 || phase > 2) return ORTK_EINVAL;
    if (int e = check_cfg(cfg)) return e;
    if (int e = check_batch(cfg, bt, phase != 1)) return e;
    if (phase == 1 && (bt->R < 1 || bt->T < 1 || bt->R % bt->B || bt->T > cfg->seq_len)) return ORTK_EINVAL;
    if (!params || !ws) return ORTK_EINVAL;
    Offsets o; build_layout(*cfg, o, nullptr);
    TrainWS w; carve_train(*cfg, bt->B, bt->S, bt->R, bt->T, ws, w);
    if (w.bytes > ws_bytes) return ORTK_ENOSPC;
    if (logp_out && (ldv_out < cfg->vocab)) return ORTK_EINVAL;
    Ctx c{cfg, ortk_s(stream), cfg->precision, seed, train != 0, params, w.w16, w.adt};
    c.side = (c.adt == ORTK_BF16 && !ortk_prof_serial()) ? side_for(c.s) : nullptr;
    c.use_side = c.side != nullptr;
    hipEvent_t box_done = nullptr;
    const bool box_early = c.use_side && !cfg->no_box && phase != 2;
    hipEvent_t feats16_done = nullptr;
    const bool f16 = c.use_side && w.feats16 && phase != 2 && (cfg->feat % 64) == 0 && tuning().feats_bf16;
    if (phase != 2) {
        if (f16) {
            TRY(ortk_cast_bf16(bt->att_feats, w.feats16, w.Me * cfg->feat, (ortk_stream)c.side->s));
            TRY(c.side_mark(&feats16_done));
        }
        if (box_early) TRY(queue_box_bias(c, o, bt->boxes, w.logbias, bt->B, bt->S, &box_done));
        TRY(make_w16(cfg, o, params, w.w16, stream));
        if (c.use_side) {
            if (!box_early) TRY(c.fork());
            TRY(make_w16t(cfg, o, params, w.w16t, (ortk_stream)c.side->s));
            TRY(c.side_mark(nullptr));
        } else {
            TRY(make_w16t(cfg, o, params, w.w16t, stream));
        }
    }
    c.ell_f = cfg->sparse_fwd;
    const float* P = params;
    const int d = cfg->d_model, ff = cfg->d_ff, H = cfg->n_heads, L = cfg->n_layers, dk = d / H, V = cfg->vocab, A = w.adt;
    const int B = bt->B, S = bt->S, R = bt->R, T = bt->T, spi = R / B;
    const bool compact = batch_compact(bt);
    if (compact && (logp_out || !w.qdt_self || !w.qdt_cross)) return ORTK_EINVAL;
    ChainSet cs; chain_layout(*cfg, o, true, true, cs, w.Me, batch_compact(bt) ? bt->Mc : w.Md);
    if (cs.on && (!w.chain_pk || plan_hits_chain(c.ell_f, cs))) cs.on = false;
    const bool dchains = cs.on && w.qdt_self == ORTK_BF16 && w.qdt_cross == ORTK_BF16 && A == ORTK_BF16;
    hipEvent_t fplan_done = nullptr;
    if (cfg->sparse_fwd && phase != 2) {
        const void* src = cfg->precision ? (const void*)w.w16 : (const void*)params;
        const int sdt = cfg->precision ? ORTK_BF16 : ORTK_F32;
        if (cs.on && c.use_side && Ctx::ell_block(c.ell_f, o.att_w, cfg->d_model, cfg->feat) < 0) {
            TRY(c.fork());
            TRY(ortk_sparse_build(cfg->sparse_fwd, src, sdt, (ortk_stream)c.side->s));
            TRY(c.side_mark(&fplan_done));
        } else {
            TRY(ortk_sparse_build(cfg->sparse_fwd, src, sdt, stream));
        }
    }
    const int64_t Me = w.Me, Md = compact ? bt->Mc : w.Md;
    const bool repack2 = phase == 2 && cs.on && chain_wide(w.Md) != chain_wide(Md);
    hipEvent_t pack_done = nullptr;
    if (cs.on && (phase != 2 || repack2)) {
        if (c.use_side && phase != 2 && tuning().feats_bf16) {
            hipEvent_t w16_ready = c.side->take();
            pack_done = c.side->take();
            if (hipEventRecord(w16_ready, c.s) != hipSuccess || hipStreamWaitEvent(c.side->s2, w16_ready, 0) != hipSuccess) return ORTK_EINVAL;
            TRY(chain_pack_all(w.w16, w.chain_pk, cs.t, c.side->s2));
            if (hipEventRecord(pack_done, c.side->s2) != hipSuccess) return ORTK_EINVAL;
        } else {
            TRY(chain_pack_all(w.w16, w.chain_pk, cs.t, c.s));
        }
    }
    EncPtrs ep[MAXLAYERS]; enc_ptrs_from_ws(w, L, ep);
    const AttMode am = att_mode(cfg->share_att_dec);
    const int64_t cw = o.cw, cv = o.cv;
    auto self_part = [&](const Ctx& cx, int l, const float* x) -> int {
        const DecOff& e = o.dec[l]; const DecBuf& b = w.dec[l];
        if (dchains) {
            if (l == 0) {
                ortk_chain_args ca; std::memset(&ca, 0, sizeof(ca));
                ca.n_units = cs.units(cs.d0); ca.M = Md; ca.x_in = x;
                ca.g1 = P + e.n0a; ca.b1 = P + e.n0b; ca.y1 = b.y1; ca.st1 = b.st1;
                ca.n1 = 3; ca.bias_s1 = P + e.bqkv; ca.out1 = b.qkv; ca.ld1 = 3 * d; ca.eps = 1e-6f;
                TRY(chain_run(&ca, cs.stream_of(w.chain_pk, cs.d0), cx.s));
            }
        } else {
            TRY(ln_fwd(cx, x, e.n0a, e.n0b, b.y1, A, b.st1, Md));
            TRY(fwd_gemm(cx, b.y1, A, d, e.wqkv, P + e.bqkv, b.qkv, w.qdt_self, 3 * d, Md, am.n * d, d));
        }
        ortk_attn_args a; std::memset(&a, 0, sizeof(a)); a.precision = cx.prec; a.qkv_dtype = w.qdt_self;
        a.q = (const float*)b.qkv; a.k = (const float*)off_elems(b.qkv, am.k * d, w.qdt_self); a.v = (const float*)off_elems(b.qkv, am.v * d, w.qdt_self);
        a.ldq = a.ldk = a.ldv = 3 * d; a.o = b.o1; a.o_dtype = A; a.ldo = d;
        a.kmask = w.keymask; a.p = b.Ps; a.nkv = R; a.H = H; a.Lq = T; a.Lk = T; a.dk = dk; a.causal_period = T;
        a.drop_p = cx.p_drop(); a.drop_seed = cx.sub(dop(l, 0));
        if (compact) { a.q_off = bt->cap_off; a.q_off_stride = 1; a.kv_ragged = 1; }
        TRY(ortk_attention_fwd(&a, (ortk_stream)cx.s));
        if (dchains) {
            ortk_chain_args ca; std::memset(&ca, 0, sizeof(ca));
            ca.n_units = cs.units(cs.db[l]); ca.M = Md; ca.x_in = x;
            ca.a_in = b.o1; ca.bias_r = P + e.bo; ca.x_mid = b.xm1; ca.seed_r = cx.sub(dop(l, 1));
            ca.g1 = P + e.n1a; ca.b1 = P + e.n1b; ca.y1 = b.y2; ca.st1 = b.st2;
            ca.n1 = 1; ca.bias_s1 = P + e.cqb; ca.out1 = b.qc; ca.ld1 = d;
            ca.drop_p = cx.p_drop(); ca.eps = 1e-6f; ca.drop_rows = cx.drop_rows;
            return chain_run(&ca, cs.stream_of(w.chain_pk, cs.db[l]), cx.s);
        }
        TRY(fwd_gemm(cx, b.o1, A, d, e.wo, P + e.bo, b.xm1, ORTK_F32, d, Md, d, d, false, cx.p_drop(), cx.sub(dop(l, 1)), x, d));
        TRY(ln_fwd(cx, b.xm1, e.n1a, e.n1b, b.y2, A, b.st2, Md));
        TRY(fwd_gemm(cx, b.y2, A, d, e.cqw, P + e.cqb, b.qc, w.qdt_cross, d, Md, d, d));
        return 0;
    };
    hipEvent_t prefix_done = nullptr;
    const bool prefix_side = c.use_side && phase == 0;
    if (prefix_side) {
        TRY(c.fork());
        if (pack_done && hipStreamWaitEvent(c.side->s, pack_done, 0) != hipSuccess) return ORTK_EINVAL;
    }
    if (phase != 2)
        TRY(encoder_forward(c, o, bt->att_feats, bt->boxes, bt->att_masks, B, S, w.x0, w.logbias, ep, w.mem, A, w.st_mem, w.qdt_enc,
                            box_early ? &box_done : nullptr, &cs, w.chain_pk, true, f16 ? w.feats16 : nullptr, feats16_done, pack_done));
    else TRY(c.wait_ev(pack_done));
    c.drop_rows = compact ? bt->row_pos : nullptr;
    if (phase == 1) {
        if (cfg->sparse_bwd) bwd_plan_forget(cfg->sparse_bwd);
        return c.join();
    }
    TRY(c.wait_ev(fplan_done));
    {
        const Ctx cx = prefix_side ? c.on_side() : c;
        TRY(embed_fwd_rows(bt->seqs, bt->seq_stride, P + o.lut, P + o.pe, w.dx0, w.keymask, Md, compact ? bt->row_pos : nullptr, T, 0, d,
                           bt->no_pad_keys ? -1 : cfg->pad_id, c.p_drop(), c.sub(OP_EMB), cx.s));
        if (prefix_side) { TRY(self_part(cx, 0, w.dx0)); TRY(c.side_mark(&prefix_done)); }
    }
    hipEvent_t bplan_done = nullptr;
    if (cfg->precision && cfg->sparse_bwd && w.w16t) {
        if (c.use_side) {
            TRY(ortk_sparse_build(cfg->sparse_bwd, w.w16t, ORTK_BF16, (ortk_stream)c.side->s));
            TRY(c.side_mark(&bplan_done));
        } else {
            TRY(ortk_sparse_build(cfg->sparse_bwd, w.w16t, ORTK_BF16, stream));
        }
        bwd_plan_built_by(cfg->sparse_bwd, ws, seed, train != 0);
    }
    const int U = o.ckv_slots;
    TRY(fwd_gemm(c, w.mem, A, d, o.ckv_w, P + o.ckv_b, w.ckv, w.qdt_cross, U * cw, Me, (int)(U * cw), d));
    const float* x = w.dx0;
    for (int l = 0; l < L; ++l) {
        const DecOff& e = o.dec[l]; const DecBuf& b = w.dec[l];
        if (l == 0 && prefix_side) TRY(c.wait_ev(prefix_done)); else TRY(self_part(c, l, x));
        ortk_attn_args a; std::memset(&a, 0, sizeof(a)); a.precision = c.prec;
// ... 379 lines not shown
    for (int l = L - 1; l >= 0; --l) {
        const EncOff& e = o.enc[l]; const EncBuf& b = w.enc[l];
        const float* xin = l == 0 ? w.x0 : w.enc[l - 1].xout;
        const void* dt; int dtt;
        void* const ghl = gh_of(l); void* const gql = gq_of(l);
        c.grp_on = grp_layers;
        TRY(drop_bwd(c, dx, gt_cur, Me * d, eop(l, 3), &dt, &dtt, true));
        TRY(wgrad_gemm(c, dt, dtt, d, b.h, A, ff, G + e.w2, G + e.b2, Me, d, ff));
        TRY(dgrad_gemm(c, dt, dtt, d, e.w2, ghl, A, ff, Me, d, ff, b.h, A, ff, inv_keep));
        TRY(wgrad_gemm(c, ghl, A, ff, b.y2, A, d, G + e.w1, G + e.b1, Me, ff, d));
        TRY(dgrad_ln_bwd(c, ghl, A, ff, e.w1, Me, ff, d, w.gy, b.xm, G, e.n1a, e.n1b, b.st2, dx, dx2, gt_new(), eop(l, 1)));
        TRY(drop_bwd(c, dx2, gt_cur, Me * d, eop(l, 1), &dt, &dtt, true));
        TRY(wgrad_gemm(c, dt, dtt, d, b.o, A, d, G + e.wo, G + e.bo, Me, d, d));
        if (l == 0 && tail_group) TRY(flush_wgrads(c));
        void* dOe = w.qdt_enc ? w.gdo : (void*)w.gy;
        TRY(dgrad_gemm(c, dt, dtt, d, e.wo, dOe, w.qdt_enc, d, Me, d, d));
        ortk_attn_args a; std::memset(&a, 0, sizeof(a)); a.precision = c.prec;
        a.qkv_dtype = w.qdt_enc; a.q = (const float*)b.qkv; a.k = (const float*)off_elems(b.qkv, ame.k * d, w.qdt_enc);
        a.v = (const float*)off_elems(b.qkv, ame.v * d, w.qdt_enc); a.ldq = a.ldk = a.ldv = 3 * d;
        a.p = b.P; a.nkv = B; a.H = H; a.Lq = S; a.Lk = S; a.dk = dk; a.drop_p = c.p_drop(); a.drop_seed = c.sub(eop(l, 0));
        a.d_o = (const float*)dOe; a.lddo = d; a.dqkv_dtype = A;
        a.dq = gql; a.d_k = off_elems(gql, ame.gk * d, A); a.dv = off_elems(gql, ame.gv * d, A); a.lddq = a.lddk = a.lddv = 3 * d;
        a.dscore = cfg->no_box ? nullptr : w.dscore + (int64_t)l * B * H * S * S;
        TRY(c.before_write(gql));
        TRY(ortk_attention_bwd(&a, stream));
        if (l == 1 && box_split) TRY(box_grad(1, L - 1));
        if (l == 0 && tail_group && !cfg->no_box) TRY(box_grad(0, box_split ? 1 : L));
        TRY(fold(ame, Me, gql));
        TRY(wgrad_gemm(c, gql, A, 3 * d, b.y1, A, d, G + e.wqkv, G + e.bqkv, Me, ame.n * d, d));
        if (l > 0 || !tail_group) TRY(flush_wgrads(c, l == 0));
        c.grp_on = false;
        TRY(dgrad_ln_bwd(c, gql, A, 3 * d, e.wqkv, Me, ame.n * d, d, w.gy, xin, G, e.n0a, e.n0b, b.st1, dx2, dx, gt_new(), l > 0 ? (int)eop(l - 1, 3) : -1));
    }
    if (!cfg->no_box && !tail_group) TRY(box_grad(0, box_split ? 1 : L));
    TRY(c.before_write(gt_new()));
    TRY(ortk_gate_apply(dx, w.x0, gt_cur, A, Me * d, c.p_src() > 0.f ? 1.f / (1.f - c.p_src()) : 1.f, stream));
    if (tail_group) {
        c.grp_on = true;
        TRY(wgrad_gemm(c, gt_cur, A, d, w.feats16, ORTK_BF16, cfg->feat, G + o.att_w, G + o.att_b, Me, d, cfg->feat));
        TRY(flush_wgrads(c, true));
        c.grp_on = false;
    } else {
        const bool us = c.use_side;
        c.use_side = false;
        TRY(wgrad_gemm(c, gt_cur, A, d, bt->att_feats, ORTK_F32, cfg->feat, G + o.att_w, G + o.att_b, Me, d, cfg->feat));
        c.use_side = us;
    }
    TRY(c.wait_ev(box_done_ev));
    return c.join();
}

static int encode_impl(const ortk_config*, const float*, const float*, const float*, const float*, int32_t, int32_t, void*,
                       size_t, float*, ortk_stream);

extern "C" int ortk_encode(const ortk_config* cfg, const float* params, const float* att_feats, const float* boxes,
                           const float* att_masks, int32_t B, int32_t S, void* ws, size_t ws_bytes, float* memory_out,
                           ortk_stream stream) {
    if (int e = check_cfg(cfg)) return e;
    if (!params || !att_feats || (!boxes && !cfg->no_box) || !att_masks || !ws || !memory_out || B < 1 || S < 1 || S > 128) return ORTK_EINVAL;
    return encode_impl(cfg, params, att_feats, boxes, att_masks, B, S, ws, ws_bytes, memory_out, stream);
}

namespace ortk {
struct Blk { int64_t off; int N, K; };
static std::vector<Blk> linear_blocks(const ortk_config* cfg, const Offsets& o) {
    const int d = cfg->d_model, ff = cfg->d_ff, L = cfg->n_layers;
    const int ne = att_mode(cfg->share_att_enc).n, nd = att_mode(cfg->share_att_dec).n;
    std::vector<Blk> v;
    v.push_back({o.att_w, d, cfg->feat});
    for (int l = 0; l < L; ++l) {
        const EncOff& e = o.enc[l];
        v.push_back({e.wqkv, ne * d, d}); v.push_back({e.wo, d, d}); v.push_back({e.w1, ff, d}); v.push_back({e.w2, d, ff});
    }
    for (int l = 0; l < L; ++l) {
        const DecOff& e = o.dec[l];
        v.push_back({e.wqkv, nd * d, d}); v.push_back({e.wo, d, d}); v.push_back({e.cow, d, d});
        if (cfg->share_att_dec != 2) v.push_back({e.cqw, d, d});
        v.push_back({e.w1, ff, d}); v.push_back({e.w2, d, ff});
    }
    v.push_back({o.ckv_w, (int)(o.ckv_slots * o.cw), d});
    v.push_back({o.gen_w, (int)ortk_align(cfg->vocab, 128), d});
    return v;
}
static int make_w16t(const ortk_config* cfg, const Offsets& o, const float* params, void* w16t, ortk_stream stream) {
    if (!cfg->precision || !w16t) return 0;
    const std::vector<Blk> v = linear_blocks(cfg, o);
    WBlockTable t; t.n = 0; t.tiles = 0;
    for (size_t i = 1; i < v.size(); ++i) {
        bool dup = false;
        for (int j = 0; j < t.n; ++j) dup |= t.b[j].off == (int32_t)v[i].off;
        if (dup) continue;
        if (t.n >= MAX_WBLOCKS || v[i].off > 0x7FFFFFFF) return ORTK_EINVAL;
        t.b[t.n] = WBlock{(int32_t)v[i].off, v[i].N, v[i].K, t.tiles};
        t.tiles += (int32_t)(ortk_cdiv(v[i].N, 64) * ortk_cdiv(v[i].K, 64));
        ++t.n;
    }
    return cast_bf16_transposed(params, w16t, t, ortk_s(stream));
}
}

extern "C" int ortk_linear_block(const ortk_config* cfg, int32_t i, int64_t* offset, int32_t* N, int32_t* K) {
    if (int e = check_cfg(cfg)) return e;
    Offsets o; build_layout(*cfg, o, nullptr);
    const std::vector<Blk> v = linear_blocks(cfg, o);
    if (i < 0) return (int)v.size();
    if (i >= (int)v.size() || !offset || !N || !K) return ORTK_EINVAL;
    *offset = v[i].off; *N = v[i].N; *K = v[i].K;
    return 0;
}

namespace ortk {
struct DecodeWS {
    int64_t ldv; int adt;
    void* w16;
    float *x0, *logbias; void* mem ; float* st; void* ckv ;
    EncPtrs enc;
    float *xa, *xb; void* y ; float* qkv; void* o ; void* q ; void* h ; float* logits;
    float* gstats = nullptr;
    float* gsamp = nullptr;
    int ckvdt, xq16;
    void *cache_k[MAXLAYERS], *cache_v[MAXLAYERS]; int kvdt;
    int64_t* it; int32_t *unfinished, *last_step;
    int32_t *bseq[2], *kvidx[2], *done_seq, *done_len, *done_cnt; float *blp[2], *cum, *done_lp; double* done_p;
    void* wpk = nullptr;
    int32_t* progress = nullptr;
    SStackBufs ss{};
    int tp = 0;
    void* tp_wpk = nullptr; char* tp_xbuf = nullptr; int32_t* tp_flag = nullptr;
    void* chain_pk = nullptr;
    int32_t* status = nullptr;
    void* ckv_g = nullptr;
    size_t bytes;
};

static bool stack_ok(const ortk_config& c, int64_t rows, int32_t flags) {
    if (flags & ORTK_DEC_UNFUSED) return false;
    const bool small_split = (flags & ORTK_DEC_SPLIT_SMALL) && !(flags & ORTK_DEC_SPARSE_STREAM) && stack_tp_degree(rows) >= 4;
    if (!(flags & (ORTK_DEC_STACK | ORTK_DEC_SPARSE_STREAM | ORTK_DEC_STACK_SPLIT)) && !small_split && rows < 1600) return false;
    return c.precision == 1 && c.d_model == 512 && c.n_heads == 8 && c.d_ff % 512 == 0 && c.d_ff / 512 <= 8 &&
           c.share_att_dec == 0 && c.n_layers <= STACK_MAXL && c.seq_len <= 64;
}

static int split_degree(bool dense_stack, int32_t flags, int64_t rows) {
    if (!dense_stack) return 0;
    const int G = stack_tp_degree(rows);
    if (flags & ORTK_DEC_STACK_SPLIT) return G;
    return ((flags & ORTK_DEC_SPLIT_SMALL) && !(flags & ORTK_DEC_STACK) && G >= 4) ? G : 0;
}
static void carve_decode(const ortk_config& c, int B, int S, int K, bool beam, void* base, DecodeWS& w, bool stack = false, bool sstream = false,
                         bool train = false, int tp = 0, bool greedy_rows = false) {
    const int64_t d = c.d_model, ff = c.d_ff, H = c.n_heads, L = c.n_layers, T = c.seq_len;
    w.kvdt = (c.precision && H == 8 && d == 512 && S > 8 && S <= 48 && T <= 32 && K <= 16) ? ORTK_BF16 : ORTK_F32;
    w.xq16 = (c.precision && w.kvdt == ORTK_F32 && S > 48 && attn16_shape_ok(K, S, (int)(d / H))) ? 1 : 0;
    w.ckvdt = w.xq16 ? ORTK_BF16 : w.kvdt;
    if (stack) { w.kvdt = w.ckvdt = ORTK_BF16; w.xq16 = 0; }
    if (train && !stack) { w.kvdt = w.ckvdt = ORTK_F32; w.xq16 = 0; }
    const size_t kves = ortk_esize(w.kvdt);
    const int64_t Me = (int64_t)B * S, rows = (int64_t)B * K;
    w.ldv = ortk_align(c.vocab, 128);
    w.adt = c.precision ? ORTK_BF16 : ORTK_F32;
    const size_t es = ortk_esize(w.adt);
    Bump b{reinterpret_cast<char*>(base), 0};
    auto act = [&](int64_t n) { return b.take_bytes((size_t)n * es); };
    Offsets o; build_layout(c, o, nullptr);
    w.status = b.take<int32_t>(64);
    w.w16 = c.precision ? b.take_bytes((size_t)o.total * 2) : nullptr;
    w.x0 = b.take<float>(Me * d); w.logbias = b.take<float>(L * B * H * S * S);
    w.enc.y1 = act(Me * d); w.enc.qkv = b.take<float>(Me * 3 * d); w.enc.P = nullptr; w.enc.o = act(Me * d);
    w.enc.xm = b.take<float>(Me * d); w.enc.y2 = act(Me * d); w.enc.h = act(Me * ff);
    w.enc.xout = w.x0; w.enc.st1 = b.take<float>(Me * 2); w.enc.st2 = w.enc.st1;
    w.mem = b.take_bytes((size_t)Me * d * 4); w.st = b.take<float>(std::max(Me, rows) * 2);
    w.ckv = b.take_bytes((size_t)(Me * L * 2 * d) * ortk_esize(w.ckvdt));
    if (train && stack && greedy_rows) w.ckv_g = b.take_bytes((size_t)(Me * L * 2 * d) * ortk_esize(w.ckvdt));
    w.xa = b.take<float>(rows * d); w.xb = b.take<float>(rows * d); w.y = act(rows * d);
    w.qkv = b.take<float>(rows * 3 * d); w.o = act(rows * d); w.q = b.take<float>(rows * d);
    w.h = act(rows * ff); w.logits = b.take<float>(rows * w.ldv);
    if (c.precision) w.gstats = b.take<float>(rows * (w.ldv / 64) * 2);
    if (!beam && c.precision) w.gsamp = b.take<float>(rows * (w.ldv / 64) * 4);
    for (int l = 0; l < L; ++l) { w.cache_k[l] = b.take_bytes((size_t)(rows * T * d) * kves); w.cache_v[l] = b.take_bytes((size_t)(rows * T * d) * kves); }
    w.it = b.take<int64_t>(rows);
// ... 404 lines not shown
```

sparse-image-captioning_amd/csrc/ortk_optim.hip:

```cpp
#include "ortk_common.h"

namespace {

template <bool ZERO>
__global__ __launch_bounds__(256) void adam_clip_kernel(float* __restrict__ p, float* __restrict__ g, float* __restrict__ m,
                                                        float* __restrict__ v, int64_t n, float step_size, float b1, float b2,
                                                        float eps, float clip, float sqrt_bc2) {
    const int64_t stride = (int64_t)gridDim.x * 256;
    const int64_t n4 = n >> 2;
    for (int64_t i = (int64_t)blockIdx.x * 256 + threadIdx.x; i < n4; i += stride) {
        float4 pp = reinterpret_cast<float4*>(p)[i], gg = reinterpret_cast<const float4*>(g)[i];
        float4 mm = reinterpret_cast<float4*>(m)[i], vv = reinterpret_cast<float4*>(v)[i];
        float* P = &pp.x; float* G = &gg.x; float* M = &mm.x; float* V = &vv.x;
#pragma unroll
        for (int u = 0; u < 4; ++u) {
            const float gc = fminf(fmaxf(G[u], -clip), clip);
            M[u] = M[u] + (gc - M[u]) * (1.f - b1);
            V[u] = V[u] * b2 + gc * gc * (1.f - b2);
            const float denom = sqrtf(V[u]) / sqrt_bc2 + eps;
            P[u] = P[u] - step_size * (M[u] / denom);
        }
        reinterpret_cast<float4*>(p)[i] = pp;
        reinterpret_cast<float4*>(m)[i] = mm;
        reinterpret_cast<float4*>(v)[i] = vv;
        if (ZERO) reinterpret_cast<float4*>(g)[i] = make_float4(0.f, 0.f, 0.f, 0.f);
    }
    for (int64_t i = (n4 << 2) + (int64_t)blockIdx.x * 256 + threadIdx.x; i < n; i += stride) {
        const float gc = fminf(fmaxf(g[i], -clip), clip);
        const float mi = m[i] + (gc - m[i]) * (1.f - b1);
        const float vi = v[i] * b2 + gc * gc * (1.f - b2);
        m[i] = mi; v[i] = vi;
        p[i] = p[i] - step_size * (mi / (sqrtf(vi) / sqrt_bc2 + eps));
        if (ZERO) g[i] = 0.f;
    }
}

__device__ __forceinline__ float sigmoidf_(float x) { return 1.f / (1.f + expf(-x)); }

__device__ __forceinline__ float mask_sample(float m, int mode, uint32_t seed, uint64_t i, const float* __restrict__ draws) {
    if (mode == 2) return m;
    const float pr = sigmoidf_(m);
    if (mode == 0) return rintf(pr);
    if (draws) return draws[i] < pr ? 1.f : 0.f;
    const uint32_t h = ortk_mix32((uint32_t)i * 0x9E3779B1u + (uint32_t)(i >> 32) * 0x85EBCA77u + seed);
    return ortk_u01(h) < pr ? 1.f : 0.f;
}

__global__ __launch_bounds__(256) void mask_apply_kernel(const float* __restrict__ w, const float* __restrict__ m,
                                                         float* __restrict__ we, int64_t n, int mode, uint32_t seed,
                                                         const float* __restrict__ draws) {
    for (int64_t i = (int64_t)blockIdx.x * 256 + threadIdx.x; i < n; i += (int64_t)gridDim.x * 256)
        we[i] = mask_sample(m[i], mode, seed, (uint64_t)i, draws) * w[i];
}

__global__ __launch_bounds__(256) void mask_bwd_kernel(const float* __restrict__ dwe, const float* __restrict__ w,
                                                       const float* __restrict__ m, float* __restrict__ dw, float* __restrict__ dm,
                                                       int64_t n, int mode, uint32_t seed,
                                                       const float* __restrict__ extra_coef, const float* __restrict__ draws, int64_t index0) {
    const float ec = extra_coef ? extra_coef[0] : 0.f;
    for (int64_t i = (int64_t)blockIdx.x * 256 + threadIdx.x; i < n; i += (int64_t)gridDim.x * 256) {
        const float g = dwe[i], mi = m[i];
        const float s = mask_sample(mi, mode, seed, (uint64_t)(index0 + i), draws ? draws - index0 : nullptr);
        if (dm) {
            float ds = g * w[i] + ec;
            if (mode != 2) { const float pr = sigmoidf_(mi); ds *= pr * (1.f - pr); }
            dm[i] += ds;
        }
        dw[i] = g * s;
    }
}

__global__ __launch_bounds__(256) void mask_count_kernel(const float* __restrict__ m, int64_t n, int mode, float* __restrict__ out) {
    __shared__ float sh[4];
    float c = 0.f;
    for (int64_t i = (int64_t)blockIdx.x * 256 + threadIdx.x; i < n; i += (int64_t)gridDim.x * 256)
        c += mode == 2 ? (m[i] != 0.f ? 1.f : 0.f) : rintf(sigmoidf_(m[i]));
    c = wave_sum(c);
    if ((threadIdx.x & 63) == 0) sh[threadIdx.x >> 6] = c;
    __syncthreads();
    if (threadIdx.x == 0) atomicAdd(out, sh[0] + sh[1] + sh[2] + sh[3]);
}

__device__ __forceinline__ void adam1(float& p, float g, float& m, float& v, float step_size, float b1, float b2, float eps, float clip, float sqrt_bc2) {
    const float gc = fminf(fmaxf(g, -clip), clip);
    m = m + (gc - m) * (1.f - b1);
    v = v * b2 + gc * gc * (1.f - b2);
    p = p - step_size * (m / (sqrtf(v) / sqrt_bc2 + eps));
}
__global__ __launch_bounds__(256) void masked_adam_kernel(ortk_masked_adam_args a, float step_w, float step_m, float sqrt_bc2) {
    const float ec = a.extra_coef ? a.extra_coef[0] : 0.f;
    const bool tm = a.mm != nullptr;
    const int64_t stride = (int64_t)gridDim.x * 256;
    auto one = [&](int64_t i, float g, float& w, float& ml, float& mw, float& vw, float& mm, float& mv, float act) {
        const float s = mask_sample(ml, a.mode, a.seed, (uint64_t)(a.index0 + i), a.draws);
        float ds = g * w + ec;
        if (a.mode != 2) { const float pr = sigmoidf_(ml); ds *= pr * (1.f - pr); }
        ds *= act;
        adam1(w, g * s, mw, vw, step_w, a.beta1, a.beta2, a.eps_w, a.clip, sqrt_bc2);
        if (tm) adam1(ml, ds, mm, mv, step_m, a.beta1, a.beta2, a.eps_m, a.clip, sqrt_bc2);
    };
    const int64_t n4 = a.n >> 2;
    for (int64_t i = (int64_t)blockIdx.x * 256 + threadIdx.x; i < n4; i += stride) {
        float4 g4 = reinterpret_cast<const float4*>(a.g)[i], w4 = reinterpret_cast<float4*>(a.w)[i], l4 = reinterpret_cast<float4*>(a.ml)[i];
        float4 mw4 = reinterpret_cast<float4*>(a.mw)[i], vw4 = reinterpret_cast<float4*>(a.vw)[i];
        float4 mm4 = make_float4(0.f, 0.f, 0.f, 0.f), mv4 = mm4, ac4 = make_float4(1.f, 1.f, 1.f, 1.f);
        if (tm) { mm4 = reinterpret_cast<float4*>(a.mm)[i]; mv4 = reinterpret_cast<float4*>(a.mv)[i]; }
        if (a.active) ac4 = reinterpret_cast<const float4*>(a.active)[i];
        float* G = &g4.x; float* W = &w4.x; float* Lg = &l4.x; float* MW = &mw4.x; float* VW = &vw4.x; float* MM = &mm4.x; float* MV = &mv4.x; float* AC = &ac4.x;
#pragma unroll
        for (int u = 0; u < 4; ++u) one(4 * i + u, G[u], W[u], Lg[u], MW[u], VW[u], MM[u], MV[u], AC[u]);
        reinterpret_cast<float4*>(a.w)[i] = w4; reinterpret_cast<float4*>(a.mw)[i] = mw4; reinterpret_cast<float4*>(a.vw)[i] = vw4;
        if (tm) { reinterpret_cast<float4*>(a.ml)[i] = l4; reinterpret_cast<float4*>(a.mm)[i] = mm4; reinterpret_cast<float4*>(a.mv)[i] = mv4; }
        reinterpret_cast<float4*>(a.g)[i] = make_float4(0.f, 0.f, 0.f, 0.f);
    }
    for (int64_t i = (n4 << 2) + (int64_t)blockIdx.x * 256 + threadIdx.x; i < a.n; i += stride) {
        float w = a.w[i], ml = a.ml[i], mw = a.mw[i], vw = a.vw[i], mm = tm ? a.mm[i] : 0.f, mv = tm ? a.mv[i] : 0.f;
        one(i, a.g[i], w, ml, mw, vw, mm, mv, a.active ? a.active[i] : 1.f);
        a.w[i] = w; a.mw[i] = mw; a.vw[i] = vw;
        if (tm) { a.ml[i] = ml; a.mm[i] = mm; a.mv[i] = mv; }
        a.g[i] = 0.f;
    }
}

inline unsigned ew_grid(int64_t n) { return (unsigned)std::min<int64_t>(ortk_cdiv(n, 256), 4096); }

}

extern "C" int ortk_masked_adam_step(const ortk_masked_adam_args* a, ortk_stream stream) {
    if (!a || !a->w || !a->g || !a->mw || !a->vw || !a->ml || a->n < 0 || a->index0 < 0 || a->mode < 0 || a->mode > 2) return ORTK_EINVAL;
    if ((a->mm == nullptr) != (a->mv == nullptr) || a->bc1 <= 0.f || a->bc2 <= 0.f) return ORTK_EINVAL;
    if (a->n == 0) return 0;
    auto al = [](const void* q) { return q == nullptr || (reinterpret_cast<uintptr_t>(q) & 15) == 0; };
    if (!(al(a->w) && al(a->g) && al(a->mw) && al(a->vw) && al(a->ml) && al(a->mm) && al(a->mv) && al(a->active))) return ORTK_EINVAL;
    ortk_masked_adam_args k = *a;
    if (k.draws) { k.draws -= k.index0; }
    hipLaunchKernelGGL(masked_adam_kernel, dim3(ew_grid(a->n / 4 + 1)), dim3(256), 0, ortk_s(stream), k, a->lr_w / a->bc1, a->lr_m / a->bc1,
                       (float)sqrt((double)a->bc2));
    ORTK_CHECK_LAUNCH();
    return 0;
}

static int adam_clip_launch(float* p, float* g, float* m, float* v, int64_t n, float lr, float beta1, float beta2, float eps, float clip,
                            float bc1, float bc2, bool zero, ortk_stream stream) {
    if (!p || !g || !m || !v || n < 0 || bc1 <= 0.f || bc2 <= 0.f) return ORTK_EINVAL;
    if (n == 0) return 0;
    auto al = [](const void* q) { return (reinterpret_cast<uintptr_t>(q) & 15) == 0; };
    if (!(al(p) && al(g) && al(m) && al(v))) return ORTK_EINVAL;
    const float step_size = lr / bc1;
    const float sqrt_bc2 = (float)sqrt((double)bc2);
    if (zero) hipLaunchKernelGGL(adam_clip_kernel<true>, dim3(ew_grid(n / 4 + 1)), dim3(256), 0, ortk_s(stream), p, g, m, v, n, step_size,
                                 beta1, beta2, eps, clip, sqrt_bc2);
    else      hipLaunchKernelGGL(adam_clip_kernel<false>, dim3(ew_grid(n / 4 + 1)), dim3(256), 0, ortk_s(stream), p, g, m, v, n, step_size,
                                 beta1, beta2, eps, clip, sqrt_bc2);
    ORTK_CHECK_LAUNCH();
    return 0;
}
extern "C" int ortk_adam_clip(float* p, const float* g, float* m, float* v, int64_t n, float lr, float beta1, float beta2,
                              float eps, float clip, float bc1, float bc2, ortk_stream stream) {
    return adam_clip_launch(p, const_cast<float*>(g), m, v, n, lr, beta1, beta2, eps, clip, bc1, bc2, false, stream);
}
extern "C" int ortk_adam_clip_zero(float* p, float* g, float* m, float* v, int64_t n, float lr, float beta1, float beta2,
                                   float eps, float clip, float bc1, float bc2, ortk_stream stream) {
    return adam_clip_launch(p, g, m, v, n, lr, beta1, beta2, eps, clip, bc1, bc2, true, stream);
}

extern "C" int ortk_mask_apply(const float* w, const float* m, float* w_eff, int64_t n, int32_t mode, uint32_t seed,
                               ortk_stream stream) {
    if (!w || !m || !w_eff || n < 0 || mode < 0 || mode > 2) return ORTK_EINVAL;
    if (n == 0) return 0;
    hipLaunchKernelGGL(mask_apply_kernel, dim3(ew_grid(n)), dim3(256), 0, ortk_s(stream), w, m, w_eff, n, mode, seed, (const float*)nullptr);
    ORTK_CHECK_LAUNCH();
    return 0;
}

extern "C" int ortk_mask_apply_draws(const float* w, const float* m, const float* draws, float* w_eff, int64_t n, ortk_stream stream) {
    if (!w || !m || !draws || !w_eff || n < 0) return ORTK_EINVAL;
    if (n == 0) return 0;
    hipLaunchKernelGGL(mask_apply_kernel, dim3(ew_grid(n)), dim3(256), 0, ortk_s(stream), w, m, w_eff, n, 1, 0u, draws);
    ORTK_CHECK_LAUNCH();
    return 0;
}

extern "C" int ortk_mask_bwd(const float* dw_eff, const float* w, const float* m, float* dw, float* dm, int64_t n, int32_t mode,
                             uint32_t seed, const float* extra_coef_dev, ortk_stream stream) {
    if (!dw_eff || !w || !m || !dw || n < 0 || mode < 0 || mode > 2) return ORTK_EINVAL;
    if (n == 0) return 0;
    hipLaunchKernelGGL(mask_bwd_kernel, dim3(ew_grid(n)), dim3(256), 0, ortk_s(stream), dw_eff, w, m, dw, dm, n, mode, seed, extra_coef_dev,
                       (const float*)nullptr, (int64_t)0);
    ORTK_CHECK_LAUNCH();
    return 0;
}

extern "C" int ortk_mask_bwd_draws(const float* dw_eff, const float* w, const float* m, const float* draws, float* dw, float* dm,
                                   int64_t n, const float* extra_coef_dev, ortk_stream stream) {
    if (!dw_eff || !w || !m || !draws || !dw || n < 0) return ORTK_EINVAL;
    if (n == 0) return 0;
    hipLaunchKernelGGL(mask_bwd_kernel, dim3(ew_grid(n)), dim3(256), 0, ortk_s(stream), dw_eff, w, m, dw, dm, n, 1, 0u, extra_coef_dev, draws, (int64_t)0);
    ORTK_CHECK_LAUNCH();
    return 0;
}

extern "C" int ortk_mask_count(const float* m, int64_t n, int32_t mode, float* count_dev, ortk_stream stream) {
    if (!m || !count_dev || n < 0 || mode < 0 || mode > 2) return ORTK_EINVAL;
    if (n == 0) return 0;
    hipLaunchKernelGGL(mask_count_kernel, dim3((unsigned)std::min<int64_t>(ortk_cdiv(n, 256), 1024)), dim3(256), 0,
                       ortk_s(stream), m, n, mode, count_dev);
    ORTK_CHECK_LAUNCH();
    return 0;
}
```

sparse-image-captioning_amd/models/relation_transformer.py:

```python
import ctypes as C
import os
import math
import weakref

import torch
import torch.nn as nn

from . import register_model
from .. import _lib as L
from ..data.collate import ObjectRelationCollate


class _Node(nn.Module):

    def forward(self, *a, **k):
        raise RuntimeError("structural node: compute happens in RelationTransformerModel")


def parse_share_layer(value, n_layers, what):
    if value is None or value == "" or value == ():
        return [0] * n_layers
    if isinstance(value, str):
        value = [int(v) for v in value.replace("(", "").replace(")", "").replace("[", "").replace("]", "").split(",") if v.strip()]
    if not isinstance(value, (tuple, list)):
# ... 33 lines not shown
    c.vocab, c.feat, c.seq_len = int(config.vocab_size), int(config.att_feat_size), int(config.max_seq_length)
    c.pad_id, c.bos_id, c.eos_id, c.unk_id = (int(config.pad_token_id), int(config.bos_token_id),
                                              int(config.eos_token_id), int(config.unk_token_id))
    c.box_trig = 0 if get("no_box_trigonometric_embedding", False) else 1
    c.precision = int(precision)
    c.drop_src = float(config.drop_prob_src if train_drop_src is None else train_drop_src)
    c.drop = float(drop)
    return c


def arena_entries(ccfg):
    lib = L.lib()
    n = lib.ortk_arena_entries(C.byref(ccfg))
    if n < 0:
        raise L.OrtkError("unsupported model geometry (see ortk_model.hip: check_cfg)")
    out = []
    name = C.create_string_buffer(128)
    off, numel, ndim, kind = C.c_int64(), C.c_int64(), C.c_int32(), C.c_int32()
    shape = (C.c_int64 * 4)()
    for i in range(n):
        L.check(lib.ortk_arena_entry(C.byref(ccfg), i, name, C.byref(off), C.byref(numel), C.byref(ndim), shape,
                                     C.byref(kind)), "ortk_arena_entry")
        out.append(dict(name=name.value.decode(), offset=off.value, numel=numel.value,
                        shape=tuple(shape[j] for j in range(ndim.value)), kind=kind.value))
    return out


class _ForwardFn(torch.autograd.Function):

    @staticmethod
    def forward(ctx, model, batch, train, seed, *params):
        logp, ws = model._run_forward(batch, train, seed, want_logp=True, cache_ws=False)
        ctx.model_ref = weakref.ref(model)
        ctx.batch, ctx.ws, ctx.train, ctx.seed = batch, ws, train, seed
        ctx.save_for_backward(logp)
        return logp

    @staticmethod
    def backward(ctx, dlogp):
        model = ctx.model_ref()
        (logp,) = ctx.saved_tensors
        grads = model._run_backward_external(ctx.batch, ctx.ws, logp, dlogp.contiguous(), ctx.train, ctx.seed)
        ctx.ws = None
        return (None, None, None, None) + tuple(grads)


class CaptionModelBase(nn.Module):

    def forward(self, *args, **kwargs):
        mode = kwargs.pop("mode", "forward")
        return getattr(self, "_" + mode)(*args, **kwargs)


@register_model("relation_transformer")
class RelationTransformerModel(CaptionModelBase):
    COLLATE_FN = ObjectRelationCollate
    DROPOUT = 0.1
    MASKED = False
    NO_BOX = False

    def __init__(self, config, precision=None):
        super().__init__()
        self.config = config
        self.d_model, self.dim_feedforward = config.d_model, config.dim_feedforward
        self.num_layers, self.num_heads = config.num_layers, config.num_heads
        self.drop_prob_src = config.drop_prob_src
        self.seq_length = config.max_seq_length
        self.att_feat_size, self.vocab_size = config.att_feat_size, config.vocab_size
        self.eos_idx, self.bos_idx = config.eos_token_id, config.bos_token_id
        self.unk_idx, self.pad_idx = config.unk_token_id, config.pad_token_id
        self.box_trigonometric_embedding = not (config.get("no_box_trigonometric_embedding", False) if hasattr(config, "get")
                                                else getattr(config, "no_box_trigonometric_embedding", False))
        assert self.num_layers > 0, "num_layers should be greater than 0"
        if precision is None:
            precision = config.get("ortk_precision", 0) if hasattr(config, "get") else 0
        self.precision = {"fp32": 0, "f32": 0, "bf16": 1}.get(precision, precision)
        self._ccfg = make_ccfg(config, self.precision, self.DROPOUT, no_box=self.NO_BOX)
        self._entries = arena_entries(self._ccfg)
        lib = L.lib()
        self._n_train = lib.ortk_arena_numel(C.byref(self._ccfg))
        self._n_all = lib.ortk_arena_numel_with_buffers(C.byref(self._ccfg))
        self._flat = torch.zeros(self._n_all)
        self._params = {}
        self._build_tree()
        self._bind()
        self.reset_parameters()
        self._ws_cache = {}
        self._vr_stage = {}
        self._seed_counter = 0
        self.done_beams = None

    def _extra_param_specs(self, entry):
        return []

    def _build_tree(self):
        for e in self._entries:
            parts = e["name"].split(".")
            node = self
            for p in parts[:-1]:
                if p not in node._modules:
                    node.add_module(p, _Node())
                node = node._modules[p]
            if e["kind"] == 2:
                node.register_buffer(parts[-1], torch.empty(0))
                self._params[e["name"]] = (node, parts[-1], None)
            else:
                par = nn.Parameter(torch.empty(0))
                node.register_parameter(parts[-1], par)
                self._params[e["name"]] = (node, parts[-1], par)
                for suffix, _ in self._extra_param_specs(e):
                    mp = nn.Parameter(torch.empty(0))
                    node.register_parameter(parts[-1] + suffix, mp)
                    self._params[e["name"] + suffix] = (node, parts[-1] + suffix, mp)

        for stack, share in (("encoder", self._ccfg.share_enc), ("decoder", self._ccfg.share_dec)):
            layers = self._modules["core" if self.NO_BOX else "model"]._modules[stack]._modules["layers"]
            for l in range(self.num_layers):
                if share[l] > 0:
                    layers.add_module(str(l), layers._modules[str(share[l] - 1)])

    def _arenas(self):
        return {"": "_flat"}

    def _bind(self):
        for e in self._entries:
            node, leaf, par = self._params[e["name"]]
            view = self._flat[e["offset"]:e["offset"] + e["numel"]].view(e["shape"])
            if par is None:
                node._buffers[leaf] = view
            else:
                par.data = view
                for suffix, attr in self._extra_param_specs(e):
                    arena = getattr(self, attr, None)
                    if arena is None:
                        continue
                    self._params[e["name"] + suffix][2].data = arena[e["offset"]:e["offset"] + e["numel"]].view(e["shape"])

    def _apply(self, fn, recurse=True):
        for attr in self._arenas().values():
            if getattr(self, attr, None) is None:
                continue
            t = fn(getattr(self, attr))
            if t.dtype != torch.float32:
                raise TypeError("the ORT arena is fp32; choose bf16 MFMA with precision='bf16', not .half()/.bfloat16()")
            setattr(self, attr, t)
        self._bind()
        self._ws_cache = {}
        self._vr_stage = {}
        self._plans = None
        self._ccfg.sparse_fwd = None
        self._ccfg.sparse_bwd = None
        for par in self.parameters():
            if par.grad is not None:
                par.grad = fn(par.grad)
        return self

    def named_weight_entries(self):
        return [e for e in self._entries if e["kind"] != 2]

    @torch.no_grad()
    def reset_parameters(self):
        for e in self._entries:
            node, leaf, par = self._params[e["name"]]
            name, shape = e["name"], e["shape"]
            t = node._buffers[leaf] if par is None else par.data
            if e["kind"] == 2:
                d = shape[-1]
                position = torch.arange(0, shape[1]).unsqueeze(1).float()
                div_term = torch.exp(torch.arange(0, d, 2).float() * -(math.log(10000.0) / d))
                t[0, :, 0::2] = torch.sin(position * div_term)
                t[0, :, 1::2] = torch.cos(position * div_term)
            elif name.endswith(".a_2"):
                t.fill_(1.0)
            elif name.endswith(".b_2"):
                t.zero_()
            elif len(shape) >= 2:
                if name.startswith(("model.", "core.")):
                    nn.init.xavier_uniform_(t)
                else:
                    nn.init.kaiming_uniform_(t, a=math.sqrt(5))
            else:
                wshape = self._shape_of(name[:-len("bias")] + "weight")
                bound = 1.0 / math.sqrt(wshape[1]) if wshape is not None and wshape[1] > 0 else 0.0
                t.uniform_(-bound, bound)

    def _shape_of(self, name):
        for e in self._entries:
            if e["name"] == name:
                return e["shape"]
        return None

    def load_state_dict(self, state_dict, strict=True, **kw):
        from ..utils.model_utils import densify_state_dict
        sd = {k: (v.float() if isinstance(v, torch.Tensor) and v.is_floating_point() and v.dtype != torch.float32 else v)
              for k, v in densify_state_dict(state_dict).items()}
        out = super().load_state_dict(sd, strict=strict, **kw)
        self._plans = None
        return out

    def _eff_params_ptr(self, train, seed):
        return L.ptr(self._flat)

    def _eff_params_tensor(self):
        return self._flat

    def enable_sparse_kernels(self, min_sparsity=0.9, train=False, fmt=None):
        self._sparse_min = min_sparsity
        self._sparse_fmt = {None: None, "ell16": L.SP_ELL16, "gu16": L.SP_GU16, "ell32": L.SP_ELL32}[fmt]
        self._sparse_train = bool(train) and min_sparsity is not None
        self._plans = None
        self._ccfg.sparse_fwd = None
        self._ccfg.sparse_bwd = None
        if min_sparsity is not None and self._flat.is_cuda:
            self._sparse_plans()

    def enable_sparse_stream(self, on=True):
        gather = on == "gather"
        if on == "auto":
            self._eff_params_ptr(False, 0)
            eff = self._eff_params_tensor()
            dec = [e for e in self._entries if ".decoder.layers." in e["name"] and len(e["shape"]) >= 2]
            nz = sum(int(torch.count_nonzero(eff[e["offset"]:e["offset"] + e["numel"]])) for e in dec)
            tot = sum(e["numel"] for e in dec)
            on, gather = nz <= 0.2 * tot, nz <= 0.015 * tot
        self._sparse_stream = bool(on)
        self._sparse_gather = bool(on) and gather
        return self._sparse_stream

    def _sparse_plans(self):
        if getattr(self, "_sparse_min", None) is None:
            return None, None
        if getattr(self, "_plans", None) is None:
            from ..sparse import make_plans
            L.require_gpu()
            self._eff_params_ptr(False, 0)
            eff = self._eff_params_tensor()
            pf, pb = make_plans(self._ccfg, eff, self._sparse_min, self.precision, backward=self._sparse_train,
                                fmt=getattr(self, "_sparse_fmt", None), density_of=self._train_density if self._sparse_train else None)
            if pf is not None:
                pf.build(eff[:self._n_train].bfloat16() if self.precision else eff)
                pf.check_overflow()
            self._plans = (pf, pb)
            if self._sparse_train:
                self._ccfg.sparse_fwd = C.cast(pf.ref(), C.c_void_p) if pf is not None else None
                self._ccfg.sparse_bwd = C.cast(pb.ref(), C.c_void_p) if pb is not None else None
        return self._plans

    def _train_density(self, offset, N, K):
        return 0.0

    def check_sparse_overflow(self):
        for pl in self._sparse_plans():
            if pl is not None:
                pl.check_overflow()

    def _next_seed(self):
        self._seed_counter += 1
        return (torch.initial_seed() * 1000003 + self._seed_counter) & 0xFFFFFFFFFFFFFFFF or 1

    def _workspace(self, key, nbytes, cache):
        if not cache:
            return torch.empty(int(nbytes), dtype=torch.uint8, device=self._flat.device)
        slot = (key[0], key[5] if key[0] == "decode" and len(key) > 5 else 0)
        ws = self._ws_cache.get(slot)
        if ws is None or ws.numel() < nbytes:
            ws = None
            self._ws_cache.pop(slot, None)
            ws = torch.empty(int(nbytes), dtype=torch.uint8, device=self._flat.device)
            self._ws_cache[slot] = ws
        return ws

    @staticmethod
    def clip_att(att_feats, att_masks, boxes, max_len=None):
        if att_masks is not None:
            if max_len is None:
                max_len = int(att_masks.long().sum(1).max())
            if max_len < att_masks.size(1):
                att_feats, att_masks = att_feats[:, :max_len], att_masks[:, :max_len]
                boxes = boxes[:, :max_len] if boxes is not None else boxes
# ... 356 lines not shown
```

sparse-image-captioning_amd/training.py:

```python
import ctypes as C
import math

import torch
import torch.distributed as dist

from . import _lib as L
from . import parallel
from .pruning import prune


def noam_rate(step, d_model, factor, warmup):
    return factor * (d_model ** (-0.5) * min(step ** (-0.5), step * warmup ** (-1.5)))


class NativeTrainer:
    def __init__(self, model, noamopt_factor=1.0, noamopt_warmup=20000, grad_clip=0.1, betas=(0.9, 0.98), eps=1e-9,
                 prune_supermask_lr=100.0, mask_eps=1e-2, sparsity_target=None, sparsity_weight=None, max_train_step=1,
                 overlap_allreduce=None, keep_grads=False, allreduce_dtype=None):
        L.require_gpu()
        self.model = model
        self.dev = model._flat.device
        assert self.dev.type == "cuda", "move the model to the GPU first"
        self.factor, self.warmup, self.clip, self.betas, self.eps = noamopt_factor, noamopt_warmup, grad_clip, betas, eps
        n = model._n_train
        self.grads = torch.zeros(n, device=self.dev)
        self.m = torch.zeros(n, device=self.dev)
        self.v = torch.zeros(n, device=self.dev)
        self.step_count = 0
        self.loss_dev = torch.zeros(1, device=self.dev)
        self.norm_dev = torch.zeros(1, device=self.dev)
        self._sum_scratch = None
        self.masked = getattr(model, "MASKED", False)
        if self.masked:
            self.train_masks = model._supermask
            self.mask_lr, self.mask_eps = prune_supermask_lr, mask_eps
            if self.train_masks:
                self.dm = torch.zeros(n, device=self.dev)
                self.mm = torch.zeros(n, device=self.dev)
                self.mv = torch.zeros(n, device=self.dev)
                self.mask_active = None
                if model.mask_freeze_scope is not None:
                    act = torch.zeros(n, device=self.dev)
                    names = {k for k, _ in model.active_pruning_masks()}
                    for e in model.named_weight_entries():
                        if e["kind"] == 1 and (e["name"] + "_pruning_mask") in names:
                            act[e["offset"]:e["offset"] + e["numel"]] = 1.0
                    self.mask_active = act
            self.sparsity_target = sparsity_target
            self.sparsity_weight = sparsity_weight if (sparsity_weight is not None and sparsity_weight >= 0) else (
                max(5.0, 1.5 / (1.0 - sparsity_target)) if sparsity_target is not None else 0.0)
            self.max_train_step = max_train_step
        assert allreduce_dtype in (None, "fp32", "bf16"), allreduce_dtype
        self.allreduce_dtype = "bf16" if allreduce_dtype == "bf16" else None
        self.world = parallel.world()
        self.overlap = (self.world > 1 if overlap_allreduce is None else bool(overlap_allreduce)) and not self.masked
        self.valid_positions = True
        self._dec_off = int(L.lib().ortk_arena_decoder_offset(C.byref(model._ccfg)))
        self._pending = None
        self.early_adam = (self.world == 1 and not self.masked and not self.overlap and self._dec_off % 4 == 0
                           and 0 < self._dec_off < self.grads.numel())
        self.fused_masked_tail = True
        self._opt_stream = None
        self._grads_clean = False
        self.keep_grads = bool(keep_grads)
        self.overflow_check_every = 50
        self.check_rollout_status = False

    def _batch(self, data, tok_weight, rollouts=False):
        m = self.model
        feats, boxes, masks = m._prepare(data["att_feats"], data.get("boxes"), data.get("att_masks"), data.get("att_max_len"))
        return m._make_batch(feats, boxes, masks, data["seqs"], tok_weight, m.valid_position_tables(data) if self.valid_positions else None,
                             rollouts=rollouts)

    def encode_for_update(self, data, rows, train=False, seed=0, positions=None):
        m, lib = self.model, L.lib()
        feats, boxes, masks = m._prepare(data["att_feats"], data.get("boxes"), data.get("att_masks"), data.get("att_max_len"))
        b = m._make_batch(feats, boxes, masks, None, None, None)
        b.R, b.T = int(rows), int(m.seq_length if positions is None else positions)
        m._sparse_plans()
        nbytes = lib.ortk_train_workspace_bytes(C.byref(m._ccfg), b.B, b.S, b.R, b.T)
        ws = m._workspace(("train", b.B, b.S, b.R, b.T), nbytes, True)
        pptr = m._eff_params_ptr(train, seed)
        L.check(lib.ortk_forward_phase(C.byref(m._ccfg), pptr, C.byref(b), L.ptr(ws), ws.numel(), None, 0, int(train), seed, 1,
                                       L.stream_ptr()), "ortk_forward_phase(1)")
        dt = C.c_int32(0)
        mem = lib.ortk_train_workspace_memory(C.byref(m._ccfg), b.B, b.S, b.R, b.T, L.ptr(ws), C.byref(dt))
        if not mem:
            raise L.OrtkError("ortk_train_workspace_memory")
        self._enc_keep = (feats, boxes, masks, ws)
        self._enc_geom = (b.B, b.S, b.R, b.T, bool(train), int(seed))
        return int(mem)

    def _fwd_bwd(self, batch, norm, train=True, seed=None, after_decoder_half=None, encoded=False):
        m, lib = self.model, L.lib()
        if seed is None:
            seed = m._next_seed() if train else 0
        m._sparse_plans()
        if encoded:
            geom = (batch.B, batch.S, batch.R, batch.T, bool(train), int(seed))
            if getattr(self, "_enc_geom", None) != geom:
                raise ValueError(f"encoded=True: encode_for_update() prepared {getattr(self, '_enc_geom', None)}, the update asks for "
                                 f"{geom} (images, regions, caption rows, positions, train, seed)")
            self._enc_geom = None
        nbytes = lib.ortk_train_workspace_bytes(C.byref(m._ccfg), batch.B, batch.S, batch.R, batch.T)
        ws = m._workspace(("train", batch.B, batch.S, batch.R, batch.T), nbytes, True)
        pptr = m._eff_params_ptr(train, seed)
        L.check(lib.ortk_forward_phase(C.byref(m._ccfg), pptr, C.byref(batch), L.ptr(ws), ws.numel(), None, 0, int(train), seed,
                                       2 if encoded else 0, L.stream_ptr()), "ortk_forward")
        L.check(lib.ortk_loss(C.byref(m._ccfg), C.byref(batch), L.ptr(ws), ws.numel(), L.ptr(norm), L.ptr(self.loss_dev),
                              L.stream_ptr()), "ortk_loss")
        if self.overlap or after_decoder_half is not None:
            for phase in (1, 2):
                L.check(lib.ortk_backward_phase(C.byref(m._ccfg), pptr, L.ptr(self.grads), C.byref(batch), L.ptr(ws), ws.numel(),
                                                int(train), seed, phase, L.stream_ptr()), "ortk_backward_phase")
                if phase == 1 and self.overlap:
                    self._pending = parallel.allreduce_async(self.grads[self._dec_off:], dtype=self.allreduce_dtype)
                if phase == 1 and after_decoder_half is not None:
                    after_decoder_half()
        else:
            L.check(lib.ortk_backward(C.byref(m._ccfg), pptr, L.ptr(self.grads), C.byref(batch), L.ptr(ws), ws.numel(), int(train),
                                      seed, L.stream_ptr()), "ortk_backward")
        return seed

    def _allreduce(self):
        if self.overlap:
            parallel.allreduce_arena(self.grads[:self._dec_off], dtype=self.allreduce_dtype)
            if self._pending is not None:
                self._pending.wait()
                self._pending = None
            return
        parallel.allreduce_arena(self.grads, self.dm if (self.masked and self.train_masks) else None, dtype=self.allreduce_dtype)

    def _adam(self, p, g, m, v, lr, eps, zero=False):
        t = self.step_count
        b1, b2 = self.betas
        fn = L.lib().ortk_adam_clip_zero if zero else L.lib().ortk_adam_clip
        L.check(fn(L.ptr(p), L.ptr(g), L.ptr(m), L.ptr(v), p.numel(), lr, b1, b2, eps, self.clip,
                   1.0 - b1 ** t, 1.0 - b2 ** t, L.stream_ptr()), "ortk_adam_clip")

    def rate(self):
        return noam_rate(max(self.step_count, 1), self.model.d_model, self.factor, self.warmup)

    def xe_step(self, data, train=True):
        tok_w = data["masks"][:, 1:].contiguous().float()
        return self._step(data, tok_w, tok_w, train)

    def scst_step(self, data, reward_fn, num_samples=5, baseline="greedy", train=True, sample="random", update_dropout=False,
                  sample_dropout=None, rollout_opt=None):
        m = self.model
        extra = dict(rollout_opt or {})
        was_training = m.training
        greedy = None
        B = data["att_feats"].size(0)
        kw = dict(att_feats=data["att_feats"], boxes=data.get("boxes"), att_masks=data.get("att_masks"), mode="sample",
                  att_max_len=data.get("att_max_len"))
        if sample_dropout is None:
            sample_dropout = bool(train) and sample == "random"
        drop_seed = None
        sparse_stream = getattr(m, "_sparse_stream", False)
        share_encoder = False
        with torch.no_grad():
            if sample_dropout and train:
                assert sample == "random", "train-mode sampling: multinomial rollouts"
                drop_seed = m._next_seed()
                opt = dict(extra, num_random_sample=num_samples, beam_size=0, train_mode=True, drop_seed=drop_seed)
                share_encoder = not self.masked and not sparse_stream
                if share_encoder:
                    m.train()
                    opt["memory"] = self.encode_for_update(data, B * num_samples, train=True, seed=drop_seed)
                fused = dict(opt, with_greedy=True, sample_row_offset=parallel.sample_row_offset(B, num_samples + 1))
                if baseline == "greedy" and share_encoder and m.decode_supported(B, data["att_feats"].size(1), fused, data.get("att_max_len")):
                    seq, _ = m(**kw, opt=fused)
                    greedy, seq = seq[:, :1].contiguous(), seq[:, 1:].contiguous()
                else:
                    if baseline == "greedy":
                        m.eval()
                        greedy, _ = m(**kw, opt=dict(beam_size=1, check_status=True))
                    seq, _ = m(**kw, opt=dict(opt, sample_row_offset=parallel.sample_row_offset(B, num_samples)))
            else:
                share_encoder = not (train and update_dropout) and not sparse_stream
                mem_opt = {}
                if share_encoder:
                    m.eval()
                    mem_opt = {"memory": self.encode_for_update(data, B * num_samples)}
                if sample == "beam_search":
                    assert num_samples > 1, "beam search needs more than one beam"
                    if baseline == "greedy":
                        greedy, _ = m(**kw, opt=dict(beam_size=1, check_status=True, **mem_opt))
                    seq, _ = m(**kw, opt=dict(extra, beam_size=num_samples, **mem_opt))
                else:
                    assert sample == "random", sample
                    seq, _ = m(**kw, opt={**extra, "num_random_sample": num_samples, "beam_size": 0, "with_greedy": baseline == "greedy",
                                          "sample_row_offset": parallel.sample_row_offset(B, num_samples + (baseline == "greedy")), **mem_opt})
                    if baseline == "greedy":
                        greedy, seq = seq[:, :1].contiguous(), seq[:, 1:].contiguous()
        m.train(was_training)
        reward = reward_fn(seq, greedy)
        host_reward = not reward.is_cuda
        if host_reward or self.check_rollout_status:
            m.check_decode_status()
        reward = reward.to(self.dev).float().reshape(-1)
        rows = seq.reshape(-1, seq.size(-1))
        mask = (rows != m.pad_idx).float()
        tf = dict(data)
        tf.pop("cap_len", None); tf.pop("_valid_rows", None)
        if host_reward and self.valid_positions:
            pos = torch.arange(1, mask.size(1) + 1, device=mask.device, dtype=mask.dtype)
            tf["cap_len"] = (mask * pos).amax(1).clamp_(min=1).to(torch.int64).cpu()
        tf["seqs"] = torch.cat([rows.new_full((rows.size(0), 1), m.bos_idx), rows], 1)
        if drop_seed is not None:
            loss = self._step(tf, mask * reward[:, None], mask, True, seed=drop_seed, encoded=share_encoder, rollouts=True)
        else:
            loss = self._step(tf, mask * reward[:, None], mask, train and update_dropout, encoded=share_encoder, rollouts=True)
        return loss, reward, seq, greedy

    def _masked_tail(self, a, b, train, seed, coef, lr):
        m, lib = self.model, L.lib()
        draws = m._draws(train)
        k = L.MaskedAdamArgs()
        k.w, k.g, k.mw, k.vw = m._flat[a:b].data_ptr(), self.grads[a:b].data_ptr(), self.m[a:b].data_ptr(), self.v[a:b].data_ptr()
        k.ml = m._mask_flat[a:b].data_ptr()
        if self.train_masks:
            k.mm, k.mv = self.mm[a:b].data_ptr(), self.mv[a:b].data_ptr()
            if self.mask_active is not None:
                k.active = self.mask_active[a:b].data_ptr()
        if draws is not None:
            k.draws = draws[a:b].data_ptr()
        if coef is not None:
            k.extra_coef = coef.data_ptr()
        k.n, k.index0, k.mode, k.seed = b - a, a, (1 if draws is not None else m._mode(train)), m._mask_seed(seed)
        t, (b1, b2) = self.step_count, self.betas
        k.lr_w, k.eps_w = lr, self.eps
        k.lr_m, k.eps_m = (self.mask_lr, self.mask_eps) if self.train_masks else (0.0, 1.0)
        k.beta1, k.beta2, k.clip, k.bc1, k.bc2 = b1, b2, self.clip, 1.0 - b1 ** t, 1.0 - b2 ** t
        L.check(lib.ortk_masked_adam_step(C.byref(k), L.stream_ptr()), "ortk_masked_adam_step")

    @staticmethod
    def scorer_reward_fn(scorer, refs, eos_idx=3, pad_idx=0, decode=None, device=False, vocab_size=None):
        if device:
            from .scst.scorers import MAX_DEVICE_VOCAB
            if decode is not None:
                raise ValueError("scorer_reward_fn(device=True): no string path on the device, `decode` does not apply")
            if vocab_size is None or int(vocab_size) > MAX_DEVICE_VOCAB:
                raise ValueError(f"scorer_reward_fn(device=True) needs the model's vocab_size, at most {MAX_DEVICE_VOCAB} (got {vocab_size})")
            cooked = {}

            def dev_fn(seq, greedy):
                items = seq.size(1) + (greedy is not None)
                key = (items, str(seq.device))
                if key not in cooked:
                    from .scst.scorers import RefPack
                    on_dev = isinstance(refs, RefPack) and torch.is_tensor(refs.pack)
                    cooked[key] = refs if on_dev else scorer.device_refs(refs, items, seq.device, vocab_size=vocab_size)
                return scorer.score_device(cooked[key], seq, greedy, eos_idx=eos_idx, pad_idx=pad_idx)[0]
            return dev_fn

        def fn(seq, greedy):
            sc_sample, sc_baseline = scorer.score_sequences(refs, seq, greedy, eos_idx=eos_idx, pad_idx=pad_idx, decode=decode)
            return torch.from_numpy(sc_sample - sc_baseline).float()
        return fn

    def _step(self, data, tok_weight, norm_mask, train, seed=None, encoded=False, rollouts=False):
        m = self.model
        self.step_count += 1
        if not self._grads_clean:
            self.grads.zero_()
        self._grads_clean = False
        n_norm = norm_mask.numel()
        ns = L.lib().ortk_sum_scratch_floats(n_norm)
        if ns > 0 and (self._sum_scratch is None or self._sum_scratch.numel() < ns):
            self._sum_scratch = torch.empty(ns, device=self.dev)
        L.check(L.lib().ortk_sum(L.ptr(norm_mask.contiguous()), n_norm, L.ptr(self._sum_scratch) if ns > 0 else None,
                                 L.ptr(self.norm_dev), L.stream_ptr()), "ortk_sum")
        parallel.reduce_scalar_sum(self.norm_dev)
        batch = self._batch(data, tok_weight, rollouts)
        lr = self.rate()
        early = None
        if self.early_adam:
            if self._opt_stream is None:
                self._opt_stream = torch.cuda.Stream()
            d0 = self._dec_off

            def early():
                cur = torch.cuda.current_stream()
                self._opt_stream.wait_stream(cur)
                with torch.cuda.stream(self._opt_stream):
                    self._adam(m._flat[d0:m._n_train], self.grads[d0:], self.m[d0:], self.v[d0:], lr, self.eps, zero=not self.keep_grads)
        try:
            seed = self._fwd_bwd(batch, self.norm_dev, train, seed, after_decoder_half=early, encoded=encoded)
        except BaseException:
            if self._opt_stream is not None:
                torch.cuda.current_stream().wait_stream(self._opt_stream)
            raise
        loss = self.loss_dev.clone()
        parallel.reduce_scalar_sum(loss)
        if early is not None:
            self._adam(m._flat[:d0], self.grads[:d0], self.m[:d0], self.v[:d0], lr, self.eps, zero=not self.keep_grads)
            torch.cuda.current_stream().wait_stream(self._opt_stream)
            self._grads_clean = not self.keep_grads
            return loss
        if getattr(m, "_sparse_train", False) and (self.step_count == 1 or self.step_count % self.overflow_check_every == 0):
            m.check_sparse_overflow()
        if self.masked:
            coef = None
            one_pass = self.world == 1 and self.fused_masked_tail and not self.keep_grads
            if self.train_masks:
                if not one_pass:
                    self.dm.zero_()
                if self.sparsity_target is not None:
                    sl = m.compute_sparsity_loss(self.sparsity_target, self.sparsity_weight, self.step_count - 1,
                                                 self.max_train_step)
                    loss = loss + sl
                    coef, m._sparsity_coef = m._sparsity_coef, None
                    if self.world > 1:
                        coef = coef / self.world
            if one_pass:
                self._masked_tail(0, m._n_train, train, seed, coef, lr)
                self._grads_clean = True
                return loss
            draws = m._draws(train)
            if draws is not None:
                L.check(L.lib().ortk_mask_bwd_draws(L.ptr(self.grads), L.ptr(m._flat), L.ptr(m._mask_flat), L.ptr(draws), L.ptr(self.grads),
                                                    L.ptr(self.dm) if self.train_masks else None, m._n_train, L.ptr(coef),
                                                    L.stream_ptr()), "ortk_mask_bwd_draws")
            else:
                L.check(L.lib().ortk_mask_bwd(L.ptr(self.grads), L.ptr(m._flat), L.ptr(m._mask_flat), L.ptr(self.grads),
                                              L.ptr(self.dm) if self.train_masks else None, m._n_train, m._mode(train),
                                              m._mask_seed(seed), L.ptr(coef), L.stream_ptr()), "ortk_mask_bwd")
            if self.train_masks and self.mask_active is not None:
                self.dm.mul_(self.mask_active)
        self._allreduce()
        self._adam(m._flat[:m._n_train], self.grads, self.m, self.v, lr, self.eps, zero=not self.keep_grads)
        self._grads_clean = not self.keep_grads
        if self.masked and self.train_masks:
            self._adam(m._mask_flat, self.dm, self.mm, self.mv, self.mask_lr, self.mask_eps)
        return loss
```

Before: 126,700 captions/sec.

## Fuse bf16 weight image write into Adam and skip recast on next forward

The Adam step now also writes the bf16 copy of the updated parameters into the workspace. The next forward skips the full fp32-to-bf16 cast when a version token shows the parameters are unchanged, and builds the transposed bf16 weights from that bf16 image instead of from fp32. The chain pack kernel is also restructured so each workgroup handles whole slots with four fragments per lane, and the per-element chain search is removed. This saves a full pass over the parameter arena each step, but adds cross-call state tracking that could go stale if parameters are modified outside the tracked paths.

```diff
diff --git a/include/ortk.h b/include/ortk.h
--- a/include/ortk.h
+++ b/include/ortk.h
@@ -8,7 +8,7 @@
 extern "C" {
 #endif
 
-#define ORTK_VERSION 4
+#define ORTK_VERSION 5
 #define ORTK_EINVAL (-1)
 #define ORTK_ENOSPC (-2)
 #define ORTK_ENOSYS (-3)
@@ -54,7 +54,9 @@
     const int32_t* row_pos;
     int32_t        Mc;
     int32_t        no_pad_keys;
+    int32_t        images_valid;
 } ortk_batch;
+#define ORTK_IMAGE_W16 1
 
 int ortk_valid_position_tables(const int64_t* counts, int32_t R, int32_t T, int32_t* cap_off, int32_t* row_pos, ortk_stream stream);
 size_t ortk_train_workspace_bytes(const ortk_config* cfg, int32_t B, int32_t S, int32_t R, int32_t T);
@@ -65,6 +67,7 @@
 int ortk_forward_phase(const ortk_config* cfg, const float* params, const ortk_batch* batch, void* ws, size_t ws_bytes,
                        float* logp_out, int64_t ldv, int32_t train, uint64_t seed, int32_t phase, ortk_stream stream);
 void* ortk_train_workspace_memory(const ortk_config* cfg, int32_t B, int32_t S, int32_t R, int32_t T, void* ws, int32_t* dtype);
+void* ortk_train_workspace_image(const ortk_config* cfg, int32_t B, int32_t S, int32_t R, int32_t T, void* ws, int32_t which, size_t* bytes);
 
 int ortk_loss(const ortk_config* cfg, const ortk_batch* batch, void* ws, size_t ws_bytes,
               const float* norm_dev, float* loss_dev, ortk_stream stream);
@@ -328,6 +331,8 @@
                    float eps, float clip, float bc1, float bc2, ortk_stream stream);
 int ortk_adam_clip_zero(float* p, float* g, float* m, float* v, int64_t n, float lr, float beta1, float beta2,
                         float eps, float clip, float bc1, float bc2, ortk_stream stream);
+int ortk_adam_clip_w16(float* p, float* g, float* m, float* v, void* w16, int64_t n, float lr, float beta1, float beta2,
+                       float eps, float clip, float bc1, float bc2, int32_t zero, ortk_stream stream);
 
 int ortk_mask_apply(const float* w, const float* m, float* w_eff, int64_t n, int32_t mode, uint32_t seed, ortk_stream stream);
 int ortk_mask_bwd(const float* dw_eff, const float* w, const float* m, float* dw, float* dm, int64_t n, int32_t mode,
diff --git a/sparse-image-captioning_amd/_lib.py b/sparse-image-captioning_amd/_lib.py
--- a/sparse-image-captioning_amd/_lib.py
+++ b/sparse-image-captioning_amd/_lib.py
@@ -29,9 +29,11 @@
     _fields_ = [("att_feats", C.c_void_p), ("boxes", C.c_void_p), ("att_masks", C.c_void_p), ("seqs", C.c_void_p),
                 ("seq_stride", C.c_int64), ("tok_weight", C.c_void_p),
                 ("B", C.c_int32), ("S", C.c_int32), ("R", C.c_int32), ("T", C.c_int32),
-                ("cap_off", C.c_void_p), ("row_pos", C.c_void_p), ("Mc", C.c_int32), ("no_pad_keys", C.c_int32)]
-
-
+                ("cap_off", C.c_void_p), ("row_pos", C.c_void_p), ("Mc", C.c_int32), ("no_pad_keys", C.c_int32),
+                ("images_valid", C.c_int32)]
+
+
+IMAGE_W16 = 1
 SP_ELL32, SP_ELL16, SP_GU16 = 0, 1, 2
 
 
@@ -172,6 +174,7 @@
     "ortk_forward": (_I32, [_CFG, _P, C.POINTER(Batch), _P, _SZ, _P, _I64, _I32, _U64, _P]),
     "ortk_forward_phase": (_I32, [_CFG, _P, C.POINTER(Batch), _P, _SZ, _P, _I64, _I32, _U64, _I32, _P]),
     "ortk_train_workspace_memory": (_P, [_CFG, _I32, _I32, _I32, _I32, _P, C.POINTER(C.c_int32)]),
+    "ortk_train_workspace_image": (_P, [_CFG, _I32, _I32, _I32, _I32, _P, _I32, C.POINTER(_SZ)]),
     "ortk_loss": (_I32, [_CFG, C.POINTER(Batch), _P, _SZ, _P, _P, _P]),
     "ortk_loss_external": (_I32, [_CFG, C.POINTER(Batch), _P, _SZ, _P, _P, _I64, _P]),
     "ortk_backward": (_I32, [_CFG, _P, _P, C.POINTER(Batch), _P, _SZ, _I32, _U64, _P]),
@@ -222,6 +225,7 @@
     "ortk_sum": (_I32, [_P, _I64, _P, _P, _P]),
     "ortk_adam_clip": (_I32, [_P, _P, _P, _P, _I64, _F, _F, _F, _F, _F, _F, _F, _P]),
     "ortk_adam_clip_zero": (_I32, [_P, _P, _P, _P, _I64, _F, _F, _F, _F, _F, _F, _F, _P]),
+    "ortk_adam_clip_w16": (_I32, [_P, _P, _P, _P, _P, _I64, _F, _F, _F, _F, _F, _F, _F, _I32, _P]),
     "ortk_mask_apply": (_I32, [_P, _P, _P, _I64, _I32, _U32, _P]),
     "ortk_mask_bwd": (_I32, [_P, _P, _P, _P, _P, _I64, _I32, _U32, _P, _P]),
     "ortk_masked_adam_step": (_I32, [C.POINTER(MaskedAdamArgs), _P]),
@@ -238,7 +242,7 @@
 }
 
 _lib = None
-ABI_VERSION = 4
+ABI_VERSION = 5
 
 
 def lib():
diff --git a/sparse-image-captioning_amd/csrc/ortk_chain.hip b/sparse-image-captioning_amd/csrc/ortk_chain.hip
--- a/sparse-image-captioning_amd/csrc/ortk_chain.hip
+++ b/sparse-image-captioning_amd/csrc/ortk_chain.hip
@@ -835,28 +835,33 @@
     }
 }
 
-__global__ __launch_bounds__(256) void chain_pack_all_kernel(const __bf16* __restrict__ w16, uint4* __restrict__ out, ChainPackTable t, int64_t total) {
-    for (int64_t i = (int64_t)blockIdx.x * 256 + threadIdx.x; i < total; i += (int64_t)gridDim.x * 256) {
-        int c = 0;
-        int64_t rest = i;
-        for (; c < t.n_chains; ++c) {
-            const int64_t sz = (int64_t)8 * (t.first[c + 1] - t.first[c] + 1) * CUNIT;
-            if (rest < sz) break;
-            rest -= sz;
-        }
-        const int n = t.first[c + 1] - t.first[c];
-        const int64_t usz = CUNIT;
-        const int64_t per_wave = (int64_t)(n + 1) * usz;
-        const int w = (int)(rest / per_wave);
-        const int64_t r2 = rest - (int64_t)w * per_wave;
-        const int u = (int)(r2 / usz), q = (int)(r2 % usz);
-        uint4 v = make_uint4(0, 0, 0, 0);
-        if (u < n) {
-            const auto pu = t.u[t.first[c] + u];
-            v = *reinterpret_cast<const uint4*>(w16 + (int64_t)pu.offset + pack_src(t.form[t.first[c] + u], w, q, pu.ld));
-        }
-        out[t.base[c] + rest] = v;
-    }
+constexpr int PACK_Q = 1024;
+static_assert(CUNIT % PACK_Q == 0 && PACK_Q == 4 * 256, "a slot is a whole number of workgroups of four fragments per lane");
+__global__ __launch_bounds__(256) void chain_pack_all_kernel(const __bf16* __restrict__ w16, uint4* __restrict__ out, ChainPackTable t) {
+    constexpr int PER_SLOT = CUNIT / PACK_Q;
+    int slot = (int)blockIdx.x / PER_SLOT;
+    const int q0 = ((int)blockIdx.x % PER_SLOT) * PACK_Q + (int)threadIdx.x;
+    int c = 0;
+    for (; c < t.n_chains - 1; ++c) {
+        const int slots = 8 * (t.first[c + 1] - t.first[c] + 1);
+        if (slot < slots) break;
+        slot -= slots;
+    }
+    const int n = t.first[c + 1] - t.first[c];
+    const int w = slot / (n + 1), u = slot - w * (n + 1);
+    uint4* dst = out + t.base[c] + (int64_t)slot * CUNIT + q0;
+    uint4 v[4];
+#pragma unroll
+    for (int j = 0; j < 4; ++j) v[j] = make_uint4(0, 0, 0, 0);
+    if (u < n) {
+        const auto pu = t.u[t.first[c] + u];
+        const int form = t.form[t.first[c] + u];
+        const __bf16* src = w16 + (int64_t)pu.offset;
+#pragma unroll
+        for (int j = 0; j < 4; ++j) v[j] = *reinterpret_cast<const uint4*>(src + pack_src(form, w, q0 + 256 * j, pu.ld));
+    }
+#pragma unroll
+    for (int j = 0; j < 4; ++j) dst[256 * j] = v[j];
 }
 
 constexpr size_t CHAIN_LDS = (size_t)3 * CIMG + 2 * CRB * 8 * sizeof(float) + CKEY_BYTES;
@@ -894,7 +899,8 @@
         if (t.base[c] != total || t.first[c + 1] <= t.first[c] || t.first[c + 1] > CH_MAX_UNITS) return ORTK_EINVAL;
         total += (int64_t)8 * (t.first[c + 1] - t.first[c] + 1) * CUNIT;
     }
-    hipLaunchKernelGGL(chain_pack_all_kernel, dim3(2048), dim3(256), 0, s, reinterpret_cast<const __bf16*>(w16), reinterpret_cast<uint4*>(packed), t, total);
+    if (total / PACK_Q > 0x7FFFFFFF) return ORTK_EINVAL;
+    hipLaunchKernelGGL(chain_pack_all_kernel, dim3((unsigned)(total / PACK_Q)), dim3(256), 0, s, reinterpret_cast<const __bf16*>(w16), reinterpret_cast<uint4*>(packed), t);
     ORTK_CHECK_LAUNCH();
     return 0;
 }
diff --git a/sparse-image-captioning_amd/csrc/ortk_embed_loss.hip b/sparse-image-captioning_amd/csrc/ortk_embed_loss.hip
--- a/sparse-image-captioning_amd/csrc/ortk_embed_loss.hip
+++ b/sparse-image-captioning_amd/csrc/ortk_embed_loss.hip
@@ -206,7 +206,8 @@
     for (int64_t i = (n4 << 2) + (int64_t)blockIdx.x * 256 + threadIdx.x; i < n; i += (int64_t)gridDim.x * 256) y[i] = (__bf16)x[i];
 }
 
-__global__ __launch_bounds__(256) void cast_bf16_t_kernel(const float* __restrict__ x, __bf16* __restrict__ yt, ortk::WBlockTable tab) {
+template <bool SRC16>
+__global__ __launch_bounds__(256) void cast_bf16_t_kernel(const void* __restrict__ xv, __bf16* __restrict__ yt, ortk::WBlockTable tab) {
     __shared__ float tile[64][65];
     int bi = 0;
     {
@@ -217,20 +218,39 @@
     const ortk::WBlock wb = tab.b[bi];
     const int tk = (wb.K + 63) >> 6;
     const int t = (int)blockIdx.x - wb.tile0, n0 = (t / tk) * 64, k0 = (t % tk) * 64;
-    const float* src = x + wb.off;
     __bf16* dst = yt + wb.off;
     const int tid = threadIdx.x;
-    const bool vec = (wb.K & 3) == 0 && (wb.off & 3) == 0;
-#pragma unroll
-    for (int i = 0; i < 4; ++i) {
-        const int r = (tid >> 4) + 16 * i, c = (tid & 15) * 4;
-        const int n = n0 + r, k = k0 + c;
-        float4 v = make_float4(0.f, 0.f, 0.f, 0.f);
-        if (n < wb.N) {
-            if (vec && k + 3 < wb.K) v = *reinterpret_cast<const float4*>(src + (int64_t)n * wb.K + k);
-            else { float* q = &v.x; for (int e = 0; e < 4; ++e) if (k + e < wb.K) q[e] = src[(int64_t)n * wb.K + k + e]; }
+    if constexpr (SRC16) {
+        const __bf16* src = reinterpret_cast<const __bf16*>(xv) + wb.off;
+        const bool vec = (wb.K & 7) == 0 && (wb.off & 7) == 0;
+#pragma unroll
+        for (int i = 0; i < 2; ++i) {
+            const int r = (tid >> 3) + 32 * i, c = (tid & 7) * 8;
+            const int n = n0 + r, k = k0 + c;
+            bf16x8 v;
+#pragma unroll
+            for (int e = 0; e < 8; ++e) v[e] = (__bf16)0.f;
+            if (n < wb.N) {
+                if (vec && k + 7 < wb.K) v = *reinterpret_cast<const bf16x8*>(src + (int64_t)n * wb.K + k);
+                else { for (int e = 0; e < 8; ++e) if (k + e < wb.K) v[e] = src[(int64_t)n * wb.K + k + e]; }
+            }
+#pragma unroll
+            for (int e = 0; e < 8; ++e) tile[r][c + e] = (float)v[e];
         }
-        tile[r][c] = v.x; tile[r][c + 1] = v.y; tile[r][c + 2] = v.z; tile[r][c + 3] = v.w;
+    } else {
+        const float* src = reinterpret_cast<const float*>(xv) + wb.off;
+        const bool vec = (wb.K & 3) == 0 && (wb.off & 3) == 0;
+#pragma unroll
+        for (int i = 0; i < 4; ++i) {
+            const int r = (tid >> 4) + 16 * i, c = (tid & 15) * 4;
+            const int n = n0 + r, k = k0 + c;
+            float4 v = make_float4(0.f, 0.f, 0.f, 0.f);
+            if (n < wb.N) {
+                if (vec && k + 3 < wb.K) v = *reinterpret_cast<const float4*>(src + (int64_t)n * wb.K + k);
+                else { float* q = &v.x; for (int e = 0; e < 4; ++e) if (k + e < wb.K) q[e] = src[(int64_t)n * wb.K + k + e]; }
+            }
+            tile[r][c] = v.x; tile[r][c + 1] = v.y; tile[r][c + 2] = v.z; tile[r][c + 3] = v.w;
+        }
     }
     __syncthreads();
     const bool vec_o = (wb.N & 7) == 0 && (wb.off & 7) == 0;
@@ -458,10 +478,11 @@
 }
 
 namespace ortk {
-int cast_bf16_transposed(const float* x, void* yt, const WBlockTable& t, hipStream_t s) {
-    if (!x || !yt || t.n < 0 || t.n > MAX_WBLOCKS) return ORTK_EINVAL;
+int cast_bf16_transposed(const void* x, int x_dtype, void* yt, const WBlockTable& t, hipStream_t s) {
+    if (!x || !yt || t.n < 0 || t.n > MAX_WBLOCKS || (x_dtype != ORTK_F32 && x_dtype != ORTK_BF16)) return ORTK_EINVAL;
     if (t.n == 0 || t.tiles == 0) return 0;
-    hipLaunchKernelGGL(cast_bf16_t_kernel, dim3((unsigned)t.tiles), dim3(256), 0, s, x, reinterpret_cast<__bf16*>(yt), t);
+    if (x_dtype == ORTK_BF16) hipLaunchKernelGGL(cast_bf16_t_kernel<true>, dim3((unsigned)t.tiles), dim3(256), 0, s, x, reinterpret_cast<__bf16*>(yt), t);
+    else hipLaunchKernelGGL(cast_bf16_t_kernel<false>, dim3((unsigned)t.tiles), dim3(256), 0, s, x, reinterpret_cast<__bf16*>(yt), t);
     ORTK_CHECK_LAUNCH();
     return 0;
 }
diff --git a/sparse-image-captioning_amd/csrc/ortk_internal.h b/sparse-image-captioning_amd/csrc/ortk_internal.h
--- a/sparse-image-captioning_amd/csrc/ortk_internal.h
+++ b/sparse-image-captioning_amd/csrc/ortk_internal.h
@@ -27,7 +27,7 @@
 struct WBlock { int32_t off, N, K, tile0; };
 constexpr int MAX_WBLOCKS = 200;
 struct WBlockTable { int32_t n, tiles; WBlock b[MAX_WBLOCKS]; };
-int cast_bf16_transposed(const float* x, void* yt, const WBlockTable& t, hipStream_t s);
+int cast_bf16_transposed(const void* x, int x_dtype, void* yt, const WBlockTable& t, hipStream_t s);
 
 struct BeamState {
     int32_t B, b, L, V, eos;
diff --git a/sparse-image-captioning_amd/csrc/ortk_model.hip b/sparse-image-captioning_amd/csrc/ortk_model.hip
--- a/sparse-image-captioning_amd/csrc/ortk_model.hip
+++ b/sparse-image-captioning_amd/csrc/ortk_model.hip
@@ -767,7 +767,7 @@
     }
 }
 
-static int make_w16t(const ortk_config* cfg, const Offsets& o, const float* params, void* w16t, ortk_stream stream);
+static int make_w16t(const ortk_config* cfg, const Offsets& o, const float* params, const void* w16, void* w16t, ortk_stream stream);
 static int make_w16(const ortk_config* cfg, const Offsets& o, const float* params, void* w16, ortk_stream stream) {
     if (!cfg->precision) return 0;
     return ortk_cast_bf16(params, w16, o.total, stream);
@@ -847,6 +847,16 @@
 extern "C" int ortk_forward(const ortk_config* cfg, const float* params, const ortk_batch* bt, void* ws, size_t ws_bytes,
                             float* logp_out, int64_t ldv_out, int32_t train, uint64_t seed, ortk_stream stream) {
     return ortk_forward_phase(cfg, params, bt, ws, ws_bytes, logp_out, ldv_out, train, seed, 0, stream);
+}
+
+extern "C" void* ortk_train_workspace_image(const ortk_config* cfg, int32_t B, int32_t S, int32_t R, int32_t T, void* ws, int32_t which, size_t* bytes) {
+    if (check_cfg(cfg) || B < 1 || S < 1 || R < 1 || T < 1 || !ws || which < 0 || which > 2 || !cfg->precision) return nullptr;
+    TrainWS w; carve_train(*cfg, B, S, R, T, ws, w);
+    Offsets o; build_layout(*cfg, o, nullptr);
+    size_t n = (size_t)o.total * 2;
+    if (which == 2) { ChainSet cs; chain_layout(*cfg, o, true, true, cs, 0, 0, true); n = w.chain_pk ? cs.bytes : 0; }
+    if (bytes) *bytes = n;
+    return which == 0 ? w.w16 : which == 1 ? w.w16t : w.chain_pk;
 }
 
 extern "C" void* ortk_train_workspace_memory(const ortk_config* cfg, int32_t B, int32_t S, int32_t R, int32_t T, void* ws, int32_t* dtype) {
@@ -874,19 +884,26 @@
     const bool box_early = c.use_side && !cfg->no_box && phase != 2;
     hipEvent_t feats16_done = nullptr;
     const bool f16 = c.use_side && w.feats16 && phase != 2 && (cfg->feat % 64) == 0 && tuning().feats_bf16;
+    const bool w16_valid = cfg->precision && w.w16 && (bt->images_valid & ORTK_IMAGE_W16) != 0;
+    hipEvent_t call_begin = nullptr;
+    if (w16_valid && c.use_side && phase != 2) {
+        call_begin = c.side->take();
+        if (hipEventRecord(call_begin, c.s) != hipSuccess) return ORTK_EINVAL;
+    }
     if (phase != 2) {
         if (f16) {
             TRY(ortk_cast_bf16(bt->att_feats, w.feats16, w.Me * cfg->feat, (ortk_stream)c.side->s));
             TRY(c.side_mark(&feats16_done));
         }
         if (box_early) TRY(queue_box_bias(c, o, bt->boxes, w.logbias, bt->B, bt->S, &box_done));
-        TRY(make_w16(cfg, o, params, w.w16, stream));
+        if (!w16_valid) TRY(make_w16(cfg, o, params, w.w16, stream));
+        const void* t_src = w16_valid ? w.w16 : nullptr;
         if (c.use_side) {
             if (!box_early) TRY(c.fork());
-            TRY(make_w16t(cfg, o, params, w.w16t, (ortk_stream)c.side->s));
+            TRY(make_w16t(cfg, o, params, t_src, w.w16t, (ortk_stream)c.side->s));
             TRY(c.side_mark(nullptr));
         } else {
-            TRY(make_w16t(cfg, o, params, w.w16t, stream));
+            TRY(make_w16t(cfg, o, params, t_src, w.w16t, stream));
         }
     }
     c.ell_f = cfg->sparse_fwd;
@@ -915,9 +932,13 @@
     hipEvent_t pack_done = nullptr;
     if (cs.on && (phase != 2 || repack2)) {
         if (c.use_side && phase != 2 && tuning().feats_bf16) {
-            hipEvent_t w16_ready = c.side->take();
+            hipEvent_t w16_ready = call_begin;
+            if (!w16_ready) {
+                w16_ready = c.side->take();
+                if (hipEventRecord(w16_ready, c.s) != hipSuccess) return ORTK_EINVAL;
+            }
             pack_done = c.side->take();
-            if (hipEventRecord(w16_ready, c.s) != hipSuccess || hipStreamWaitEvent(c.side->s2, w16_ready, 0) != hipSuccess) return ORTK_EINVAL;
+            if (hipStreamWaitEvent(c.side->s2, w16_ready, 0) != hipSuccess) return ORTK_EINVAL;
             TRY(chain_pack_all(w.w16, w.chain_pk, cs.t, c.side->s2));
             if (hipEventRecord(pack_done, c.side->s2) != hipSuccess) return ORTK_EINVAL;
         } else {
@@ -1463,7 +1484,7 @@
     v.push_back({o.gen_w, (int)ortk_align(cfg->vocab, 128), d});
     return v;
 }
-static int make_w16t(const ortk_config* cfg, const Offsets& o, const float* params, void* w16t, ortk_stream stream) {
+static int make_w16t(const ortk_config* cfg, const Offsets& o, const float* params, const void* w16, void* w16t, ortk_stream stream) {
     if (!cfg->precision || !w16t) return 0;
     const std::vector<Blk> v = linear_blocks(cfg, o);
     WBlockTable t; t.n = 0; t.tiles = 0;
@@ -1476,7 +1497,7 @@
         t.tiles += (int32_t)(ortk_cdiv(v[i].N, 64) * ortk_cdiv(v[i].K, 64));
         ++t.n;
     }
-    return cast_bf16_transposed(params, w16t, t, ortk_s(stream));
+    return w16 ? cast_bf16_transposed(w16, ORTK_BF16, w16t, t, ortk_s(stream)) : cast_bf16_transposed(params, ORTK_F32, w16t, t, ortk_s(stream));
 }
 }
 
diff --git a/sparse-image-captioning_amd/csrc/ortk_optim.hip b/sparse-image-captioning_amd/csrc/ortk_optim.hip
--- a/sparse-image-captioning_amd/csrc/ortk_optim.hip
+++ b/sparse-image-captioning_amd/csrc/ortk_optim.hip
@@ -2,35 +2,47 @@
 
 namespace {
 
-template <bool ZERO>
+__device__ __forceinline__ float adam_clip1(float p, float g, float& m, float& v, float step_size, float b1, float b2, float eps, float clip,
+                                            float sqrt_bc2) {
+    const float gc = fminf(fmaxf(g, -clip), clip);
+    m = m + (gc - m) * (1.f - b1);
+    v = v * b2 + gc * gc * (1.f - b2);
+    const float denom = sqrtf(v) / sqrt_bc2 + eps;
+    return p - step_size * (m / denom);
+}
+template <bool ZERO, bool W16>
 __global__ __launch_bounds__(256) void adam_clip_kernel(float* __restrict__ p, float* __restrict__ g, float* __restrict__ m,
-                                                        float* __restrict__ v, int64_t n, float step_size, float b1, float b2,
-                                                        float eps, float clip, float sqrt_bc2) {
+                                                        float* __restrict__ v, __bf16* __restrict__ w16, int64_t n, float step_size, float b1,
+                                                        float b2, float eps, float clip, float sqrt_bc2) {
+    constexpr int NV = W16 ? 2 : 1;
     const int64_t stride = (int64_t)gridDim.x * 256;
-    const int64_t n4 = n >> 2;
-    for (int64_t i = (int64_t)blockIdx.x * 256 + threadIdx.x; i < n4; i += stride) {
-        float4 pp = reinterpret_cast<float4*>(p)[i], gg = reinterpret_cast<const float4*>(g)[i];
-        float4 mm = reinterpret_cast<float4*>(m)[i], vv = reinterpret_cast<float4*>(v)[i];
-        float* P = &pp.x; float* G = &gg.x; float* M = &mm.x; float* V = &vv.x;
-#pragma unroll
-        for (int u = 0; u < 4; ++u) {
-            const float gc = fminf(fmaxf(G[u], -clip), clip);
-            M[u] = M[u] + (gc - M[u]) * (1.f - b1);
-            V[u] = V[u] * b2 + gc * gc * (1.f - b2);
-            const float denom = sqrtf(V[u]) / sqrt_bc2 + eps;
-            P[u] = P[u] - step_size * (M[u] / denom);
+    const int64_t nl = n / (4 * NV);
+    for (int64_t i = (int64_t)blockIdx.x * 256 + threadIdx.x; i < nl; i += stride) {
+        float4 pp[NV], gg[NV], mm[NV], vv[NV];
+#pragma unroll
+        for (int j = 0; j < NV; ++j) {
+            pp[j] = reinterpret_cast<float4*>(p)[NV * i + j]; gg[j] = reinterpret_cast<const float4*>(g)[NV * i + j];
+            mm[j] = reinterpret_cast<float4*>(m)[NV * i + j]; vv[j] = reinterpret_cast<float4*>(v)[NV * i + j];
         }
-        reinterpret_cast<float4*>(p)[i] = pp;
-        reinterpret_cast<float4*>(m)[i] = mm;
-        reinterpret_cast<float4*>(v)[i] = vv;
-        if (ZERO) reinterpret_cast<float4*>(g)[i] = make_float4(0.f, 0.f, 0.f, 0.f);
-    }
-    for (int64_t i = (n4 << 2) + (int64_t)blockIdx.x * 256 + threadIdx.x; i < n; i += stride) {
-        const float gc = fminf(fmaxf(g[i], -clip), clip);
-        const float mi = m[i] + (gc - m[i]) * (1.f - b1);
-        const float vi = v[i] * b2 + gc * gc * (1.f - b2);
-        m[i] = mi; v[i] = vi;
-        p[i] = p[i] - step_size * (mi / (sqrtf(vi) / sqrt_bc2 + eps));
+#pragma unroll
+        for (int j = 0; j < NV; ++j) {
+            float* P = &pp[j].x; float* G = &gg[j].x; float* M = &mm[j].x; float* V = &vv[j].x;
+#pragma unroll
+            for (int u = 0; u < 4; ++u) P[u] = adam_clip1(P[u], G[u], M[u], V[u], step_size, b1, b2, eps, clip, sqrt_bc2);
+            reinterpret_cast<float4*>(p)[NV * i + j] = pp[j];
+            reinterpret_cast<float4*>(m)[NV * i + j] = mm[j];
+            reinterpret_cast<float4*>(v)[NV * i + j] = vv[j];
+            if (ZERO) reinterpret_cast<float4*>(g)[NV * i + j] = make_float4(0.f, 0.f, 0.f, 0.f);
+        }
+        if constexpr (W16)
+            reinterpret_cast<bf16x8*>(w16)[i] = (bf16x8){(__bf16)pp[0].x, (__bf16)pp[0].y, (__bf16)pp[0].z, (__bf16)pp[0].w,
+                                                         (__bf16)pp[1].x, (__bf16)pp[1].y, (__bf16)pp[1].z, (__bf16)pp[1].w};
+    }
+    for (int64_t i = nl * (4 * NV) + (int64_t)blockIdx.x * 256 + threadIdx.x; i < n; i += stride) {
+        float mi = m[i], vi = v[i];
+        const float pi = adam_clip1(p[i], g[i], mi, vi, step_size, b1, b2, eps, clip, sqrt_bc2);
+        m[i] = mi; v[i] = vi; p[i] = pi;
+        if (W16) w16[i] = (__bf16)pi;
         if (ZERO) g[i] = 0.f;
     }
 }
@@ -140,28 +152,35 @@
     return 0;
 }
 
-static int adam_clip_launch(float* p, float* g, float* m, float* v, int64_t n, float lr, float beta1, float beta2, float eps, float clip,
-                            float bc1, float bc2, bool zero, ortk_stream stream) {
+static int adam_clip_launch(float* p, float* g, float* m, float* v, void* w16, int64_t n, float lr, float beta1, float beta2, float eps,
+                            float clip, float bc1, float bc2, bool zero, ortk_stream stream) {
     if (!p || !g || !m || !v || n < 0 || bc1 <= 0.f || bc2 <= 0.f) return ORTK_EINVAL;
     if (n == 0) return 0;
     auto al = [](const void* q) { return (reinterpret_cast<uintptr_t>(q) & 15) == 0; };
-    if (!(al(p) && al(g) && al(m) && al(v))) return ORTK_EINVAL;
+    if (!(al(p) && al(g) && al(m) && al(v) && al(w16))) return ORTK_EINVAL;
     const float step_size = lr / bc1;
     const float sqrt_bc2 = (float)sqrt((double)bc2);
-    if (zero) hipLaunchKernelGGL(adam_clip_kernel<true>, dim3(ew_grid(n / 4 + 1)), dim3(256), 0, ortk_s(stream), p, g, m, v, n, step_size,
-                                 beta1, beta2, eps, clip, sqrt_bc2);
-    else      hipLaunchKernelGGL(adam_clip_kernel<false>, dim3(ew_grid(n / 4 + 1)), dim3(256), 0, ortk_s(stream), p, g, m, v, n, step_size,
-                                 beta1, beta2, eps, clip, sqrt_bc2);
+    __bf16* o = reinterpret_cast<__bf16*>(w16);
+    const dim3 grid(ew_grid(n / (w16 ? 8 : 4) + 1));
+#define ORTK_ADAM(Z, W) hipLaunchKernelGGL((adam_clip_kernel<Z, W>), grid, dim3(256), 0, ortk_s(stream), p, g, m, v, o, n, step_size, beta1, \
+                                           beta2, eps, clip, sqrt_bc2)
+    if (zero) { if (w16) ORTK_ADAM(true, true); else ORTK_ADAM(true, false); }
+    else      { if (w16) ORTK_ADAM(false, true); else ORTK_ADAM(false, false); }
+#undef ORTK_ADAM
     ORTK_CHECK_LAUNCH();
     return 0;
 }
 extern "C" int ortk_adam_clip(float* p, const float* g, float* m, float* v, int64_t n, float lr, float beta1, float beta2,
                               float eps, float clip, float bc1, float bc2, ortk_stream stream) {
-    return adam_clip_launch(p, const_cast<float*>(g), m, v, n, lr, beta1, beta2, eps, clip, bc1, bc2, false, stream);
+    return adam_clip_launch(p, const_cast<float*>(g), m, v, nullptr, n, lr, beta1, beta2, eps, clip, bc1, bc2, false, stream);
 }
 extern "C" int ortk_adam_clip_zero(float* p, float* g, float* m, float* v, int64_t n, float lr, float beta1, float beta2,
                                    float eps, float clip, float bc1, float bc2, ortk_stream stream) {
-    return adam_clip_launch(p, g, m, v, n, lr, beta1, beta2, eps, clip, bc1, bc2, true, stream);
+    return adam_clip_launch(p, g, m, v, nullptr, n, lr, beta1, beta2, eps, clip, bc1, bc2, true, stream);
+}
+extern "C" int ortk_adam_clip_w16(float* p, float* g, float* m, float* v, void* w16, int64_t n, float lr, float beta1, float beta2,
+                                  float eps, float clip, float bc1, float bc2, int32_t zero, ortk_stream stream) {
+    return adam_clip_launch(p, g, m, v, w16, n, lr, beta1, beta2, eps, clip, bc1, bc2, zero != 0, stream);
 }
 
 extern "C" int ortk_mask_apply(const float* w, const float* m, float* w_eff, int64_t n, int32_t mode, uint32_t seed,
diff --git a/sparse-image-captioning_amd/models/relation_transformer.py b/sparse-image-captioning_amd/models/relation_transformer.py
--- a/sparse-image-captioning_amd/models/relation_transformer.py
+++ b/sparse-image-captioning_amd/models/relation_transformer.py
@@ -139,6 +139,7 @@
         self._n_all = lib.ortk_arena_numel_with_buffers(C.byref(self._ccfg))
         self._flat = torch.zeros(self._n_all)
         self._params = {}
+        self._param_version = 0
         self._build_tree()
         self._bind()
         self.reset_parameters()
@@ -202,6 +203,7 @@
                 raise TypeError("the ORT arena is fp32; choose bf16 MFMA with precision='bf16', not .half()/.bfloat16()")
             setattr(self, attr, t)
         self._bind()
+        self.params_changed()
         self._ws_cache = {}
         self._vr_stage = {}
         self._plans = None
@@ -212,11 +214,27 @@
                 par.grad = fn(par.grad)
         return self
 
+    def params_changed(self):
+        self._param_version += 1
+
+    def _params_token(self):
+        ver = self._flat._version
+        for par in self._token_params():
+            ver += par._version
+        return (self._param_version, id(self._flat), ver)
+
+    def _token_params(self):
+        tp = getattr(self, "_token_params_list", None)
+        if tp is None:
+            tp = self._token_params_list = [t[2] for t in self._params.values() if t[2] is not None]
+        return tp
+
     def named_weight_entries(self):
         return [e for e in self._entries if e["kind"] != 2]
 
     @torch.no_grad()
     def reset_parameters(self):
+        self.params_changed()
         for e in self._entries:
             node, leaf, par = self._params[e["name"]]
             name, shape = e["name"], e["shape"]
@@ -252,6 +270,7 @@
         sd = {k: (v.float() if isinstance(v, torch.Tensor) and v.is_floating_point() and v.dtype != torch.float32 else v)
               for k, v in densify_state_dict(state_dict).items()}
         out = super().load_state_dict(sd, strict=strict, **kw)
+        self.params_changed()
         self._plans = None
         return out
 
diff --git a/sparse-image-captioning_amd/training.py b/sparse-image-captioning_amd/training.py
--- a/sparse-image-captioning_amd/training.py
+++ b/sparse-image-captioning_amd/training.py
@@ -1,5 +1,6 @@
 import ctypes as C
 import math
+import weakref
 
 import torch
 import torch.distributed as dist
@@ -65,6 +66,9 @@
         self.keep_grads = bool(keep_grads)
         self.overflow_check_every = 50
         self.check_rollout_status = False
+        self.write_images = True
+        self._img = None
+        self._fwd_img = None
 
     def _batch(self, data, tok_weight, rollouts=False):
         m = self.model
@@ -81,6 +85,7 @@
         nbytes = lib.ortk_train_workspace_bytes(C.byref(m._ccfg), b.B, b.S, b.R, b.T)
         ws = m._workspace(("train", b.B, b.S, b.R, b.T), nbytes, True)
         pptr = m._eff_params_ptr(train, seed)
+        b.images_valid = self._images_valid(b, ws)
         L.check(lib.ortk_forward_phase(C.byref(m._ccfg), pptr, C.byref(b), L.ptr(ws), ws.numel(), None, 0, int(train), seed, 1,
                                        L.stream_ptr()), "ortk_forward_phase(1)")
         dt = C.c_int32(0)
@@ -105,6 +110,7 @@
         nbytes = lib.ortk_train_workspace_bytes(C.byref(m._ccfg), batch.B, batch.S, batch.R, batch.T)
         ws = m._workspace(("train", batch.B, batch.S, batch.R, batch.T), nbytes, True)
         pptr = m._eff_params_ptr(train, seed)
+        batch.images_valid = self._images_valid(batch, ws) if not encoded else 0
         L.check(lib.ortk_forward_phase(C.byref(m._ccfg), pptr, C.byref(batch), L.ptr(ws), ws.numel(), None, 0, int(train), seed,
                                        2 if encoded else 0, L.stream_ptr()), "ortk_forward")
         L.check(lib.ortk_loss(C.byref(m._ccfg), C.byref(batch), L.ptr(ws), ws.numel(), L.ptr(norm), L.ptr(self.loss_dev),
@@ -131,12 +137,43 @@
             return
         parallel.allreduce_arena(self.grads, self.dm if (self.masked and self.train_masks) else None, dtype=self.allreduce_dtype)
 
-    def _adam(self, p, g, m, v, lr, eps, zero=False):
+    def _image_address(self, batch, ws):
+        if not self.write_images or self.masked or not self.model.precision:
+            return None
+        nb = C.c_size_t(0)
+        return L.lib().ortk_train_workspace_image(C.byref(self.model._ccfg), batch.B, batch.S, batch.R, batch.T, L.ptr(ws), 0,
+                                                  C.byref(nb)) or None
+
+    def _images_valid(self, batch, ws):
+        addr = self._image_address(batch, ws)
+        self._fwd_img = None if addr is None else (weakref.ref(ws), addr)
+        img, self._img = self._img, None
+        if addr is None or img is None:
+            return 0
+        ok = img[0]() is ws and img[1] == addr and img[2] == self.model._params_token()
+        return L.IMAGE_W16 if ok else 0
+
+    def _adam(self, p, g, m, v, lr, eps, zero=False, w16=None):
         t = self.step_count
         b1, b2 = self.betas
+        if w16 is not None:
+            L.check(L.lib().ortk_adam_clip_w16(L.ptr(p), L.ptr(g), L.ptr(m), L.ptr(v), w16, p.numel(), lr, b1, b2, eps, self.clip,
+                                               1.0 - b1 ** t, 1.0 - b2 ** t, int(zero), L.stream_ptr()), "ortk_adam_clip_w16")
+            return
         fn = L.lib().ortk_adam_clip_zero if zero else L.lib().ortk_adam_clip
         L.check(fn(L.ptr(p), L.ptr(g), L.ptr(m), L.ptr(v), p.numel(), lr, b1, b2, eps, self.clip,
                    1.0 - b1 ** t, 1.0 - b2 ** t, L.stream_ptr()), "ortk_adam_clip")
+
+    def _image_of_step(self):
+        f = self._fwd_img
+        if f is None or f[0]() is None:
+            return None
+        return f[1]
+
+    def _image_written(self):
+        f, self._fwd_img = self._fwd_img, None
+        self.model.params_changed()
+        self._img = None if f is None else (f[0], f[1], self.model._params_token())
 
     def rate(self):
         return noam_rate(max(self.step_count, 1), self.model.d_model, self.factor, self.warmup)
@@ -284,8 +321,10 @@
             def early():
                 cur = torch.cuda.current_stream()
                 self._opt_stream.wait_stream(cur)
+                w16 = self._image_of_step() if d0 % 8 == 0 else None
                 with torch.cuda.stream(self._opt_stream):
-                    self._adam(m._flat[d0:m._n_train], self.grads[d0:], self.m[d0:], self.v[d0:], lr, self.eps, zero=not self.keep_grads)
+                    self._adam(m._flat[d0:m._n_train], self.grads[d0:], self.m[d0:], self.v[d0:], lr, self.eps, zero=not self.keep_grads,
+                               w16=None if w16 is None else w16 + 2 * d0)
         try:
             seed = self._fwd_bwd(batch, self.norm_dev, train, seed, after_decoder_half=early, encoded=encoded)
         except BaseException:
@@ -295,9 +334,14 @@
         loss = self.loss_dev.clone()
         parallel.reduce_scalar_sum(loss)
         if early is not None:
-            self._adam(m._flat[:d0], self.grads[:d0], self.m[:d0], self.v[:d0], lr, self.eps, zero=not self.keep_grads)
+            w16 = self._image_of_step() if d0 % 8 == 0 else None
+            self._adam(m._flat[:d0], self.grads[:d0], self.m[:d0], self.v[:d0], lr, self.eps, zero=not self.keep_grads, w16=w16)
             torch.cuda.current_stream().wait_stream(self._opt_stream)
             self._grads_clean = not self.keep_grads
+            if w16 is not None:
+                self._image_written()
+            else:
+                m.params_changed()
             return loss
         if getattr(m, "_sparse_train", False) and (self.step_count == 1 or self.step_count % self.overflow_check_every == 0):
             m.check_sparse_overflow()
@@ -316,6 +360,7 @@
                         coef = coef / self.world
             if one_pass:
                 self._masked_tail(0, m._n_train, train, seed, coef, lr)
+                m.params_changed()
                 self._grads_clean = True
                 return loss
             draws = m._draws(train)
@@ -330,8 +375,13 @@
             if self.train_masks and self.mask_active is not None:
                 self.dm.mul_(self.mask_active)
         self._allreduce()
-        self._adam(m._flat[:m._n_train], self.grads, self.m, self.v, lr, self.eps, zero=not self.keep_grads)
+        w16 = self._image_of_step()
+        self._adam(m._flat[:m._n_train], self.grads, self.m, self.v, lr, self.eps, zero=not self.keep_grads, w16=w16)
         self._grads_clean = not self.keep_grads
+        if w16 is not None:
+            self._image_written()
+        else:
+            m.params_changed()
         if self.masked and self.train_masks:
             self._adam(m._mask_flat, self.dm, self.mm, self.mv, self.mask_lr, self.mask_eps)
         return loss
```

Result: slower. 125,300 captions/sec (-1.1%).
